# WHU-USI3DV/LaneMapping

Hardware: AMD Instinct MI355X
Metric: BEV tiles/sec end-to-end (LAS points -> polylines) (higher is better)
Workload: dtype f32; 1 GPU; on-GPU LAS->BEV raster (4,194,304 points/tile resident in HBM) + configs/Proj_polyline_fpn_vit_vertex_2.py, batch=16 per GPU, seeded random weights; lines_per_tile=45, streams=2, hip_graphs=True, points=resident, stream_check=not run (--full runs it), gather_check=n/a (1 rank), raster_check=not run (--full runs it), dist_ranks=1, rccl_ranks=1

## Files before the change

include/lanemap_hip.h:

```cpp
#ifndef LANEMAP_HIP_H
#define LANEMAP_HIP_H
#include <stdint.h>
#ifdef __cplusplus
extern "C" {
#endif

enum { LM_OK = 0, LM_ERR_ARG = 1, LM_ERR_HIP = 2, LM_ERR_NO_DEVICE = 3, LM_ERR_CAPACITY = 4 };
enum { LM_ACT_NONE = 0, LM_ACT_RELU = 1, LM_ACT_GELU = 2 };

int lm_abi_version(void);
const char* lm_last_error(void);
int lm_device_count(void);

int lm_conv2d_nhwc_mfma_f32(void* stream, const float* x, int ldx, const float* wp, int CoutP,
                            const float* scale, const float* shift, const float* res, int ldr, int res_rows,
                            float* y, int ldy, int B, int H, int W, int Cin, int Cout, int KH, int KW,
                            int stride, int pad_h, int pad_w, int dil, int act);
int lm_conv2d_nhwc_mfma_resup_f32(void* stream, const float* x, int ldx, const float* wp, int CoutP, const float* scale,
                                  const float* shift, const float* res_coarse, int ldr, int Hr, int Wr, float* y, int ldy,
                                  int B, int H, int W, int Cin, int Cout, int KH, int KW, int stride, int pad_h, int pad_w,
                                  int dil, int act);

int lm_winograd44_supported(int H, int W, int Cin, int dil);
int lm_winograd44_gn_chunks(int H, int W, int dil);
long lm_winograd44_tiles(int B, int H, int W, int dil);
long lm_winograd44_twin_workspace_bytes(int B, int H, int W, int Cin, int CoutP, int dil);
int lm_conv3x3_winograd44_f32(void* stream, const float* x, int ldx, const float* wu_frag, int CoutP, const float* scale,
                              const float* shift, const float* res, int ldr, float* y, int ldy, int B, int H, int W,
                              int Cin, int Cout, int dil, int act, double* gn_partial);
int lm_conv3x3_winograd44_twin_f32(void* stream, const float* x, int ldx, const float* wu, int CoutP, const float* scale,
                                   const float* shift, const float* res, int ldr, float* y, int ldy, int B, int H, int W,
                                   int Cin, int Cout, int dil, int act, void* workspace, long workspace_bytes);
int lm_wino44_split_fragments(void* stream, const float* frag, float* out, long n_quads);
int lm_conv3x3_winograd44_split_f32(void* stream, const float* x, int ldx, const float* wu_split, int CoutP, const float* scale,
                                    const float* shift, const float* res, int ldr, float* y, int ldy, int B, int H, int W,
                                    int Cin, int Cout, int dil, int act, double* gn_partial, float post);
int lm_conv3x3_winograd44_split_twin_f32(void* stream, const float* x, int ldx, const float* wu, int CoutP, const float* scale,
                                         const float* shift, const float* res, int ldr, float* y, int ldy, int B, int H, int W,
                                         int Cin, int Cout, int dil, int act, void* workspace, long workspace_bytes, float post);

int lm_conv2d_nhwc_mfma_f32_gnstats(void* stream, const float* x, int ldx, const float* wp, int CoutP, const float* shift,
                                    float* y, int ldy, double* gn_partial, int B, int H, int W, int Cin, int Cout,
                                    int KH, int KW, int stride, int pad_h, int pad_w, int dil);
int lm_gn_finalize(void* stream, const double* partial, float* stats, int B, int HW, int C, int nchunk, float eps);
int lm_gn_finalize_split(void* stream, const double* partial, float* stats, int B, int HW, int C, int nchunk, float eps, int split);

int lm_stem_conv7x7_bn_relu(void* stream, const float* x_chw, const float* w_k64, const float* scale,
                            const float* shift, float* y_nhwc, int B, int H, int W);
int lm_stem_conv7x7_bn_relu_u8(void* stream, const unsigned char* x_hwc3, const float* w_k64, const float* scale,
                               const float* shift, float* y_nhwc, int B, int H, int W);
int lm_maxpool3x3s2_nhwc(void* stream, const float* x, float* y, int B, int H, int W, int C);
int lm_conv2d_nhwc_small(void* stream, const float* x, int ldx, const float* w_tc16, const float* scale,
                         const float* shift, float* y, int ldy, int B, int H, int W, int Cin, int Cout,
                         int KH, int KW, int stride, int pad_h, int pad_w, int pre_relu, int act);

int lm_gn_stats(void* stream, const float* x, double* workspace, float* stats, int B, int HW, int C, float eps);
long lm_gn_stats_workspace_bytes(int B, int HW, int C);
int lm_gn_relu_upsample(void* stream, const float* x, const float* stats, const float* gamma, const float* beta,
                        float* y, int B, int Hi, int Wi, int Ho, int Wo, int C, int accumulate);
int lm_gn_relu_upsample_sum(void* stream, int n, const float* const* x, const float* const* stats, const int* Hi, const int* Wi,
                            const int* ldx , const float* gamma, const float* beta,
                            float* y, int B, int Ho, int Wo, int C);
int lm_gn_relu_upsample_sum_conv1x1(void* stream, int n, const float* const* x, const float* const* stats, const int* Hi, const int* Wi,
                                    const int* ldx, const float* gamma, const float* beta, float* y, int B, int Ho, int Wo, int C,
                                    const float* w_c16, const float* bias, int cout, float* y1, int ldy1);
int lm_upsample_bilinear_nhwc(void* stream, const float* x, int ldx, const float* add, int lda, float* y, int ldy,
                              int B, int Hi, int Wi, int Ho, int Wo, int C);
int lm_upsample_bilinear_to_chw(void* stream, const float* x, int ldx, float* y_chw, int B, int Hi, int Wi,
                                int Ho, int Wo, int C);
int lm_layernorm_rows(void* stream, const float* x, const float* gamma, const float* beta, float* y,
                      long rows, int D, float eps);
int lm_unpatchify(void* stream, const float* tokens, float* y_nhwc, int B, int G, int P, int C);
int lm_token_mix_mfma_f32(void* stream, const float* x, const float* wt, int ldw, const float* bias, const float* res, float* y,
                          int B, int M, int K, int N, int act);

int lm_attention_f32(void* stream, const float* qkv, float* out, int B, int N, int heads, int dim_head, float scale);
int lm_attention_masked_f32(void* stream, const float* qkv, float* out, const int* valid, int B, int N, int heads, int dim_head, float scale);

int lm_head_tokens(void* stream, const float* seg, const float* row_nhwc16, float* tok, float seg_bias,
                   int B, int P, int Hr, int Wr, int prop_width, int half_buff);
int lm_head_tokens_window(void* stream, const float* row_nhwc16, float* tok, int B, int P, int Hr, int Wr, int prop_width, int half_buff);
int lm_head_stage2(void* stream, const float* hid, int ldh, int D, const float* w2, const float* b2,
                   float* ext2, float* cls2, float* off2, long M);
int lm_head_proposal_conf(void* stream, const float* tok, const float* wt, const float* bias, float* conf,
                          int BP, int L);

int lm_head_endpoint_tile(void);
int lm_head_endpoint(void* hip_stream, const float* col, int ldc, const float* x_endp, const float* w1p, const float* b1,
                     const float* bn_scale, const float* bn_shift, const float* w2, const float* b2, float* out, int B, int h, int w,
                     int H, int W);

int lm_decode_proposals(void* stream, const float* pconf, const float* ext2, const float* cls2, const float* off2,
                        float* prop_conf, float* v_ext, float* cls_conf, int* cls_idx, double* cls_offset,
                        int B, int P, int R, float exist_thre, int prop_width, int half_buff);
int lm_decode_orient(void* stream, const float* x_nhwc, int ldx, int C, unsigned char* y, long pixels);
int lm_decode_semantic(void* stream, const float* logit_chw3, unsigned char* sem, float* biseg, float* rows,
                       int B, int H, int W, float thre, int raw_mode);
long lm_endp_topk_workspace_bytes(int B);
int lm_endp_topk(void* stream, const float* endp_logit, void* workspace, int* out_idx, float* out_score,
                 int* out_status, int B, int H, int W, int clip, int K);

int lm_pack_segments(void* stream, int n, const void* const* src, const long* bytes, const long* dst_offsets, void* dst);


typedef struct {
    float quat[4];
    float trans[3];
    float bev_img_offset[2];
    float img_reso[2];
    float local_min_ele;
    float ele_reso;
    float inten_lo, inten_hi;
} LmRasterParams;
long lm_bev_raster_workspace_bytes(int B, long max_points_per_tile, int H, int W);
int lm_bev_raster_batch(void* stream, const float* points_xyzi, const long* tile_offsets, const LmRasterParams* params,
                        int B, void* workspace, long workspace_bytes, float* out_chw, unsigned char* out_hwc_u8,
                        int H, int W);
int lm_bev_raster_batch_scaled(void* hip_stream, const float* points_xyzi, const long* tile_offsets, const LmRasterParams* params,
                               int B, void* workspace, long workspace_bytes, float* out_chw, unsigned char* out_hwc_u8,
                               int H, int W, const float* inten_scale);
int lm_tile_ingest_u8(void* stream, const unsigned char* src_hwc, float* dst_chw, int B, int H, int W, int C);

typedef struct {
    double x0, y0, cell;
    int nx, ny;
} LmStripGrid;
int lm_strip_build_grid(const LmRasterParams* params, int T, int H, int W, double z_lo, double z_hi, LmStripGrid* grid,
                        unsigned short* cells, long cells_cap);
long lm_strip_bin_workspace_bytes(long N, int T);
int lm_strip_bin_points(void* hip_stream, const float* points_xyzi, long N, const LmRasterParams* params, int T, int H, int W,
                        double z_lo, double z_hi, void* workspace, long workspace_bytes, long* counts, long* offsets,
                        long* offsets_host, float* binned, long capacity);

long lm_tile_ground_workspace_bytes(int B, int H, int W, int cell_px);
int lm_tile_ground(void* hip_stream, const float* points_xyzi, const long* tile_offsets, const LmRasterParams* params, int B, int H,
                   int W, int cell_px, void* workspace, long workspace_bytes, float* ground, float* ground_min, float* cell_min);
long lm_ground_select_workspace_bytes(long N, int B);
int lm_ground_select(void* hip_stream, const float* points_xyzi, const long* tile_offsets, const LmRasterParams* params, int B, int H,
                     int W, int cell_px, const float* ground, float h_lo, float h_hi, void* workspace, long workspace_bytes,
                     float* points_out, long* out_offsets, long* out_offsets_host);

long lm_tile_intensity_workspace_bytes(int B, int G);
int lm_tile_intensity_window(void* hip_stream, const float* points_xyzi, const long* tile_offsets, const LmRasterParams* params, int B,
                             int H, int W, const int* group, int G, int q_lo_ppm, int q_hi_ppm, void* workspace, long workspace_bytes,
                             int* window, long* count, unsigned* coarse_hist);

long lm_drape_workspace_bytes(long n_vertices, int B, int radius_px);
int lm_drape_vertices(void* hip_stream, const float* points_xyzi, const long* tile_offsets, const LmRasterParams* params, int B, int H,
                      int W, const int* vertices_rc, const long* vertex_offsets, int radius_px, void* workspace, long workspace_bytes,
                      float* z, int* npix, float* pixel_min);

int lm_tile_gap_hist(void* hip_stream, const unsigned char* tiles_hwc_u8, int B, int H, int W, int max_radius_px, unsigned* hist);
int lm_tile_gap_fill(void* hip_stream, const unsigned char* tiles_hwc_u8, int B, int H, int W, const int* radius_px,
                     unsigned char* out_hwc_u8);

int lm_endp_cluster(const int* topk_idx, int n_avail, int Wc, int clip, int k0, int k_step, int k_max, int radius,
                    int min_clusters, int* out_hw, int max_out, int* n_out, int* k_used);
int lm_polyline_assemble(const float* prop_conf, const float* prop_v_ext, const double* cls_offset,
                         const float* bi_seg_rows, const int* endp_hw, int n_endp, int P, int R, float obj_thre,
                         int min_vertices, double* out_lanes, int* endp_keep);
int lm_raster_polylines(const double* lanes, int P, int R, unsigned char* out);
int lm_line8(unsigned char* out, int x1, int y1, int x2, int y2, int colour);
int lm_trace_lines(const double* cols, int n, int R, const float* seg_rows, double* out);
int lm_polyline_backproject(unsigned char* bev_hwc, int H, int W, int C, const double* img_seqs, const int* seq_lens, int L,
                            int Vmax, const double* params13, const double* las_read_offset, double* out);
int lm_polyline_backproject_z(unsigned char* bev_hwc, int H, int W, int C, const double* img_seqs, const int* seq_lens, int L,
                              int Vmax, const double* params13, const double* las_read_offset, double* out,
                              const float* vertex_z, int fit);

long lm_skeletonize_lee_2d(unsigned char* img, int H, int W);

void* lm_merge_create(void);
void lm_merge_destroy(void* merger);
int lm_merge_add_tile(void* merger, const double* points, const int* lens, int n);
long lm_merge_finish(void* merger, long* total_points);
int lm_merge_result(void* merger, double* points, int* lens);
int lm_downsample_seq(const double* seq, int n, double dist_min, double* out);

int lm_softmax_rows(void* stream, float* x, long rows, int cols);
int lm_rowref_select(void* stream, const float* ext, const float* cls, float* mean_out, int* valid, float thr_ext, int* corr,
                     int B, int H, int W, int L);
int lm_rowref_gather(void* stream, const float* x_nhwc8, const int* corr, float* tok, int B, int H, int W, int L);
int lm_rowref_scatter(void* stream, const float* x_nhwc8, const float* tok, const int* corr, const int* valid,
                      float* y_nhwc8, int B, int H, int W, int L);
int lm_rowref_gather_win(void* hip_stream, const float* x_nhwc8, const int* corr, float* tok, int B, int H, int W, int L, int off_grid);
int lm_rowref_scatter_win(void* hip_stream, const float* x_nhwc8, const float* tok, const int* corr, const int* valid,
                          float* y_nhwc8, int B, int H, int W, int L, int off_grid);
int lm_rowref_decode(void* stream, const float* ext2, const float* cls2, unsigned char* conf, unsigned char* cls_map,
                     int* col_idx, int B, int H, int W, int L);

long lm_voxelize_workspace_bytes(long n_points);
long lm_scan_workspace_bytes(long n);
int lm_exclusive_scan_u32(void* stream, const unsigned* in, unsigned* out, long n, void* workspace, long workspace_bytes);
long lm_sort_pairs_workspace_bytes(long n);
int lm_sort_pairs_u32(void* stream, unsigned* keys_io, unsigned* vals_io, long n, int end_bit, void* workspace, long workspace_bytes);
int lm_voxelize_hard(void* stream, const float* points, long n, const float* range_lo_xyz, const float* voxel_size_xyz,
                     const int* grid_xyz, int max_points, int max_voxels, int batch_idx, const int* row_base, int cap_rows,
                     float* feats, int ldf, int* coords, int* row_end, int raster_order, void* workspace,
                     long workspace_bytes);
int lm_sparse_grid_build(void* stream, const int* coords, long n, int* grid, int B, int D, int H, int W);
long lm_sparse_conv_outputs_workspace_bytes(long out_cells);
int lm_sparse_conv_outputs(void* stream, const int* in_coords, long n_in, int B, const int* ksp_zyx9, int Do, int Ho, int Wo,
                           int* out_grid, int* out_coords, int cap_rows, int* out_count, void* workspace, long workspace_bytes);
int lm_sparse_rulebook(void* stream, const int* out_coords, long n_out, const int* in_grid, int B, int D, int H, int W,
                       const int* ksp_zyx9, int* nbr);
int lm_conv_gather_mfma_f32(void* stream, const float* x, int ldx, const int* nbr, int taps, const float* wp, int CoutP,
                            const float* scale, const float* shift, const float* res, int ldr, float* y, int ldy,
                            long M, int Cin, int Cout, int act);
int lm_sparse_to_dense_nhwc(void* stream, const float* feats, int ldf, const int* coords, long n, float* out, int B, int D,
                            int H, int W, int C, int flip_h);
int lm_upsample_bicubic_nhwc(void* stream, const float* x, float* y, int B, int H, int W, int C, int Ho, int Wo);

typedef struct {
    int version_major, version_minor, point_format, record_len;
    long n_points, offset_to_points;
    double scale[3], offset[3], min_xyz[3], max_xyz[3];
} LmLasHeader;
int lm_las_parse_header(const unsigned char* bytes, long len, LmLasHeader* out);
int lm_las_decode_points(void* stream, const unsigned char* records, int record_len, long n, const double* scale,
                         const double* offset, const double* shift, float inten_lo, float inten_hi, int normalise,
                         float* out_xyzi);
enum { LM_LAS_DROP_SYNTHETIC = 1, LM_LAS_DROP_KEYPOINT = 2, LM_LAS_DROP_WITHHELD = 4, LM_LAS_DROP_OVERLAP = 8 };
enum { LM_LAS_RETURNS_ALL = 0, LM_LAS_RETURNS_FIRST = 1, LM_LAS_RETURNS_LAST = 2, LM_LAS_RETURNS_SINGLE = 3 };
typedef struct { unsigned class_mask[8]; unsigned drop_flags; int returns; float z_lo, z_hi; } LmLasSelect;
long lm_las_select_workspace_bytes(long n);
int lm_las_decode_select(void* hip_stream, const unsigned char* records, int record_len, int point_format, long n,
                         const double* scale, const double* offset, const double* shift, float inten_lo, float inten_hi,
                         int normalise, const LmLasSelect* select, void* workspace, long workspace_bytes, float* out_xyzi,
                         long* kept, unsigned long* class_hist);

int lm_png_info(const unsigned char* data, long size, int* H, int* W, int* C);
int lm_png_decode_u8(const unsigned char* data, long size, unsigned char* out_hwc, long out_bytes);
int lm_png_decode_files_u8(const char* const* paths, int n, unsigned char* out_nhwc, int H, int W, int C, int threads);
int lm_zlib_inflate(const unsigned char* data, long size, unsigned char* out, long capacity, long* produced);

long lm_lane_json_text(const double* lane_vertexes, int n_lines, int row_size, int with_pervertex_semantics, char* out, long cap);
int lm_lane_json_write(const double* lane_vertexes, int n_lines, int row_size, int with_pervertex_semantics, const char* path);
int lm_seqs_json_write(const double* seqs, const int* lens, int L, int Vmax, int D, const char* path);

#ifdef __cplusplus
}
#endif
#endif
```

lanemapping_amd/_lib.py:

```python
import ctypes as C
import os

_HERE = os.path.dirname(os.path.abspath(__file__))
LIB_PATH = os.environ.get('LANEMAP_HIP_LIB') or os.path.join(_HERE, 'liblanemap_hip.so')

c_f32p = C.POINTER(C.c_float)
vp, i32, i64, f32 = C.c_void_p, C.c_int, C.c_long, C.c_float


class LmRasterParams(C.Structure):
    _fields_ = [('quat', C.c_float * 4), ('trans', C.c_float * 3), ('bev_img_offset', C.c_float * 2),
                ('img_reso', C.c_float * 2), ('local_min_ele', C.c_float), ('ele_reso', C.c_float),
                ('inten_lo', C.c_float), ('inten_hi', C.c_float)]


class LmLasHeader(C.Structure):
    _fields_ = [('version_major', C.c_int), ('version_minor', C.c_int), ('point_format', C.c_int), ('record_len', C.c_int),
                ('n_points', C.c_long), ('offset_to_points', C.c_long), ('scale', C.c_double * 3), ('offset', C.c_double * 3),
                ('min_xyz', C.c_double * 3), ('max_xyz', C.c_double * 3)]


class LmStripGrid(C.Structure):
    _fields_ = [('x0', C.c_double), ('y0', C.c_double), ('cell', C.c_double), ('nx', C.c_int), ('ny', C.c_int)]


class LmLasSelect(C.Structure):
    _fields_ = [('class_mask', C.c_uint * 8), ('drop_flags', C.c_uint), ('returns', C.c_int), ('z_lo', C.c_float), ('z_hi', C.c_float)]


SIGNATURES = {
    'lm_abi_version': (i32, []),
    'lm_last_error': (C.c_char_p, []),
    'lm_device_count': (i32, []),
    'lm_conv2d_nhwc_mfma_f32': (i32, [vp, vp, i32, vp, i32, vp, vp, vp, i32, i32, vp, i32,
                                      i32, i32, i32, i32, i32, i32, i32, i32, i32, i32, i32, i32]),
    'lm_conv2d_nhwc_mfma_resup_f32': (i32, [vp, vp, i32, vp, i32, vp, vp, vp, i32, i32, i32, vp, i32,
                                            i32, i32, i32, i32, i32, i32, i32, i32, i32, i32, i32, i32]),
    'lm_winograd44_supported': (i32, [i32, i32, i32, i32]),
    'lm_winograd44_gn_chunks': (i32, [i32, i32, i32]),
    'lm_winograd44_tiles': (i64, [i32, i32, i32, i32]),
    'lm_winograd44_twin_workspace_bytes': (i64, [i32, i32, i32, i32, i32, i32]),
    'lm_conv3x3_winograd44_f32': (i32, [vp, vp, i32, vp, i32, vp, vp, vp, i32, vp, i32, i32, i32, i32, i32, i32, i32, i32, vp]),
    'lm_conv3x3_winograd44_twin_f32': (i32, [vp, vp, i32, vp, i32, vp, vp, vp, i32, vp, i32, i32, i32, i32, i32, i32, i32, i32, vp, i64]),
    'lm_wino44_split_fragments': (i32, [vp, vp, vp, i64]),
    'lm_conv3x3_winograd44_split_f32': (i32, [vp, vp, i32, vp, i32, vp, vp, vp, i32, vp, i32, i32, i32, i32, i32, i32, i32, i32, vp, f32]),
    'lm_conv3x3_winograd44_split_twin_f32': (i32, [vp, vp, i32, vp, i32, vp, vp, vp, i32, vp, i32, i32, i32, i32, i32, i32, i32, i32, vp, i64, f32]),
    'lm_conv2d_nhwc_mfma_f32_gnstats': (i32, [vp, vp, i32, vp, i32, vp, vp, i32, vp] + [i32] * 11),
    'lm_gn_finalize': (i32, [vp, vp, vp, i32, i32, i32, i32, f32]),
    'lm_gn_finalize_split': (i32, [vp, vp, vp, i32, i32, i32, i32, f32, i32]),
    'lm_stem_conv7x7_bn_relu': (i32, [vp, vp, vp, vp, vp, vp, i32, i32, i32]),
    'lm_stem_conv7x7_bn_relu_u8': (i32, [vp, vp, vp, vp, vp, vp, i32, i32, i32]),
    'lm_maxpool3x3s2_nhwc': (i32, [vp, vp, vp, i32, i32, i32, i32]),
    'lm_conv2d_nhwc_small': (i32, [vp, vp, i32, vp, vp, vp, vp, i32, i32, i32, i32, i32, i32, i32, i32, i32, i32, i32, i32, i32]),
    'lm_gn_stats': (i32, [vp, vp, vp, vp, i32, i32, i32, f32]),
    'lm_gn_stats_workspace_bytes': (i64, [i32, i32, i32]),
    'lm_gn_relu_upsample': (i32, [vp, vp, vp, vp, vp, vp, i32, i32, i32, i32, i32, i32, i32]),
    'lm_gn_relu_upsample_sum': (i32, [vp, i32, vp, vp, vp, vp, vp, vp, vp, vp, i32, i32, i32, i32]),
    'lm_gn_relu_upsample_sum_conv1x1': (i32, [vp, i32, vp, vp, vp, vp, vp, vp, vp, vp, i32, i32, i32, i32, vp, vp, i32, vp, i32]),
    'lm_upsample_bilinear_nhwc': (i32, [vp, vp, i32, vp, i32, vp, i32, i32, i32, i32, i32, i32, i32]),
    'lm_upsample_bilinear_to_chw': (i32, [vp, vp, i32, vp, i32, i32, i32, i32, i32, i32]),
    'lm_layernorm_rows': (i32, [vp, vp, vp, vp, vp, i64, i32, f32]),
    'lm_token_mix_mfma_f32': (i32, [vp, vp, vp, i32, vp, vp, vp, i32, i32, i32, i32, i32]),
    'lm_unpatchify': (i32, [vp, vp, vp, i32, i32, i32, i32]),
    'lm_attention_f32': (i32, [vp, vp, vp, i32, i32, i32, i32, f32]),
    'lm_attention_masked_f32': (i32, [vp, vp, vp, vp, i32, i32, i32, i32, f32]),
    'lm_head_tokens': (i32, [vp, vp, vp, vp, f32, i32, i32, i32, i32, i32, i32]),
    'lm_head_tokens_window': (i32, [vp, vp, vp, i32, i32, i32, i32, i32, i32]),
    'lm_head_stage2': (i32, [vp, vp, i32, i32, vp, vp, vp, vp, vp, i64]),
    'lm_head_proposal_conf': (i32, [vp, vp, vp, vp, vp, i32, i32]),
    'lm_head_endpoint_tile': (i32, []),
    'lm_head_endpoint': (i32, [vp, vp, i32, vp, vp, vp, vp, vp, vp, vp, vp, i32, i32, i32, i32, i32]),
    'lm_decode_proposals': (i32, [vp, vp, vp, vp, vp, vp, vp, vp, vp, vp, i32, i32, i32, f32, i32, i32]),
    'lm_decode_orient': (i32, [vp, vp, i32, i32, vp, i64]),
    'lm_decode_semantic': (i32, [vp, vp, vp, vp, vp, i32, i32, i32, f32, i32]),
    'lm_endp_topk_workspace_bytes': (i64, [i32]),
    'lm_endp_topk': (i32, [vp, vp, vp, vp, vp, vp, i32, i32, i32, i32, i32]),
    'lm_pack_segments': (i32, [vp, i32, vp, vp, vp, vp]),
    'lm_bev_raster_workspace_bytes': (i64, [i32, i64, i32, i32]),
    'lm_bev_raster_batch': (i32, [vp, vp, C.POINTER(i64), C.POINTER(LmRasterParams), i32, vp, i64, vp, vp, i32, i32]),
    'lm_bev_raster_batch_scaled': (i32, [vp, vp, C.POINTER(i64), C.POINTER(LmRasterParams), i32, vp, i64, vp, vp, i32, i32, c_f32p]),
    'lm_tile_ingest_u8': (i32, [vp, vp, vp, i32, i32, i32, i32]),
    'lm_strip_build_grid': (i32, [C.POINTER(LmRasterParams), i32, i32, i32, C.c_double, C.c_double, C.POINTER(LmStripGrid), vp, i64]),
    'lm_strip_bin_workspace_bytes': (i64, [i64, i32]),
    'lm_strip_bin_points': (i32, [vp, vp, i64, C.POINTER(LmRasterParams), i32, i32, i32, C.c_double, C.c_double, vp, i64, vp, vp,
                                  C.POINTER(i64), vp, i64]),
    'lm_tile_ground_workspace_bytes': (i64, [i32, i32, i32, i32]),
    'lm_tile_ground': (i32, [vp, vp, C.POINTER(i64), C.POINTER(LmRasterParams), i32, i32, i32, i32, vp, i64, vp, vp, vp]),
    'lm_ground_select_workspace_bytes': (i64, [i64, i32]),
    'lm_ground_select': (i32, [vp, vp, C.POINTER(i64), C.POINTER(LmRasterParams), i32, i32, i32, i32, vp, f32, f32, vp, i64, vp, vp,
                               C.POINTER(i64)]),
    'lm_tile_intensity_workspace_bytes': (i64, [i32, i32]),
    'lm_tile_intensity_window': (i32, [vp, vp, C.POINTER(i64), C.POINTER(LmRasterParams), i32, i32, i32, C.POINTER(i32), i32, i32, i32, vp, i64,
                                       vp, vp, vp]),
    'lm_drape_workspace_bytes': (i64, [i64, i32, i32]),
    'lm_drape_vertices': (i32, [vp, vp, C.POINTER(i64), C.POINTER(LmRasterParams), i32, i32, i32, vp, C.POINTER(i64), i32, vp, i64, vp, vp, vp]),
    'lm_tile_gap_hist': (i32, [vp, vp, i32, i32, i32, i32, vp]),
    'lm_tile_gap_fill': (i32, [vp, vp, i32, i32, i32, C.POINTER(i32), vp]),
    'lm_endp_cluster': (i32, [vp, i32, i32, i32, i32, i32, i32, i32, i32, vp, i32, vp, vp]),
    'lm_polyline_assemble': (i32, [vp, vp, vp, vp, vp, i32, i32, i32, f32, i32, vp, vp]),
    'lm_raster_polylines': (i32, [vp, i32, i32, vp]),
    'lm_line8': (i32, [vp, i32, i32, i32, i32, i32]),
    'lm_trace_lines': (i32, [vp, i32, i32, vp, vp]),
    'lm_polyline_backproject': (i32, [vp, i32, i32, i32, vp, vp, i32, i32, vp, vp, vp]),
    'lm_polyline_backproject_z': (i32, [vp, i32, i32, i32, vp, vp, i32, i32, vp, vp, vp, vp, i32]),
    'lm_skeletonize_lee_2d': (i64, [vp, i32, i32]),
    'lm_merge_create': (vp, []),
    'lm_merge_destroy': (None, [vp]),
    'lm_merge_add_tile': (i32, [vp, vp, vp, i32]),
    'lm_merge_finish': (i64, [vp, C.POINTER(i64)]),
    'lm_merge_result': (i32, [vp, vp, vp]),
    'lm_downsample_seq': (i32, [vp, i32, C.c_double, vp]),
    'lm_softmax_rows': (i32, [vp, vp, i64, i32]),
    'lm_rowref_select': (i32, [vp, vp, vp, vp, vp, f32, vp, i32, i32, i32, i32]),
    'lm_rowref_gather': (i32, [vp, vp, vp, vp, i32, i32, i32, i32]),
    'lm_rowref_scatter': (i32, [vp, vp, vp, vp, vp, vp, i32, i32, i32, i32]),
    'lm_rowref_gather_win': (i32, [vp, vp, vp, vp, i32, i32, i32, i32, i32]),
    'lm_rowref_scatter_win': (i32, [vp, vp, vp, vp, vp, vp, i32, i32, i32, i32, i32]),
    'lm_rowref_decode': (i32, [vp, vp, vp, vp, vp, vp, i32, i32, i32, i32]),
    'lm_voxelize_workspace_bytes': (i64, [i64]),
    'lm_scan_workspace_bytes': (i64, [i64]),
    'lm_exclusive_scan_u32': (i32, [vp, vp, vp, i64, vp, i64]),
    'lm_sort_pairs_workspace_bytes': (i64, [i64]),
    'lm_sort_pairs_u32': (i32, [vp, vp, vp, i64, i32, vp, i64]),
    'lm_voxelize_hard': (i32, [vp, vp, i64, c_f32p, c_f32p, C.POINTER(i32), i32, i32, i32, vp, i32, vp, i32, vp, vp, i32, vp, i64]),
    'lm_sparse_grid_build': (i32, [vp, vp, i64, vp, i32, i32, i32, i32]),
    'lm_sparse_conv_outputs_workspace_bytes': (i64, [i64]),
    'lm_sparse_conv_outputs': (i32, [vp, vp, i64, i32, C.POINTER(i32), i32, i32, i32, vp, vp, i32, vp, vp, i64]),
    'lm_sparse_rulebook': (i32, [vp, vp, i64, vp, i32, i32, i32, i32, C.POINTER(i32), vp]),
    'lm_conv_gather_mfma_f32': (i32, [vp, vp, i32, vp, i32, vp, i32, vp, vp, vp, i32, vp, i32, i64, i32, i32, i32]),
    'lm_sparse_to_dense_nhwc': (i32, [vp, vp, i32, vp, i64, vp, i32, i32, i32, i32, i32, i32]),
    'lm_upsample_bicubic_nhwc': (i32, [vp, vp, vp, i32, i32, i32, i32, i32, i32]),
    'lm_las_parse_header': (i32, [vp, i64, C.POINTER(LmLasHeader)]),
    'lm_las_decode_points': (i32, [vp, vp, i32, i64, C.POINTER(C.c_double), C.POINTER(C.c_double), C.POINTER(C.c_double), f32, f32,
                                   i32, vp]),
    'lm_las_select_workspace_bytes': (i64, [i64]),
    'lm_las_decode_select': (i32, [vp, vp, i32, i32, i64, C.POINTER(C.c_double), C.POINTER(C.c_double), C.POINTER(C.c_double), f32, f32,
                                   i32, C.POINTER(LmLasSelect), vp, i64, vp, vp, vp]),
    'lm_png_info': (i32, [vp, i64, C.POINTER(i32), C.POINTER(i32), C.POINTER(i32)]),
    'lm_png_decode_u8': (i32, [vp, i64, vp, i64]),
    'lm_png_decode_files_u8': (i32, [C.POINTER(C.c_char_p), i32, vp, i32, i32, i32, i32]),
    'lm_zlib_inflate': (i32, [vp, i64, vp, i64, C.POINTER(i64)]),
    'lm_lane_json_text': (i64, [vp, i32, i32, i32, vp, i64]),
    'lm_lane_json_write': (i32, [vp, i32, i32, i32, C.c_char_p]),
    'lm_seqs_json_write': (i32, [vp, vp, i32, i32, i32, C.c_char_p]),
}

_lib = None


class LanemapHipError(RuntimeError):
    pass


def lib():
    global _lib
    if _lib is None:
        if not os.path.exists(LIB_PATH):
            raise LanemapHipError(
                f'{LIB_PATH} is missing: the HIP library is the only implementation of this package '
                '(no CPU fallback). Build it with `python -m lanemapping_amd.build`.')
        import torch
        L = C.CDLL(LIB_PATH)
        for name, (res, args) in SIGNATURES.items():
            fn = getattr(L, name)
            fn.restype = res
            fn.argtypes = args
        _lib = L
    return _lib


def check(code):
    if code != 0:
        raise LanemapHipError(f'lanemap_hip error {code}: {lib().lm_last_error().decode()}')
```

lanemapping_amd/csrc/common.h:

```cpp
#pragma once
#include <hip/hip_runtime.h>
#include <cstdarg>
#include <cstdint>
#include <cstdio>

#define LM_API extern "C" __attribute__((visibility("default")))

enum {
    LM_OK = 0,
    LM_ERR_ARG = 1,
    LM_ERR_HIP = 2,
    LM_ERR_NO_DEVICE = 3,
    LM_ERR_CAPACITY = 4
};

void lm_set_error(const char* fmt, ...);
int lm_ensure_dynamic_lds(const void* kernel, size_t bytes);

#define LM_REQUIRE(cond, ...)            \
    do {                                 \
        if (!(cond)) {                   \
            lm_set_error(__VA_ARGS__);   \
            return LM_ERR_ARG;           \
        }                                \
    } while (0)

#define LM_HIP(expr)                                                                  \
    do {                                                                              \
        hipError_t e_ = (expr);                                                       \
        if (e_ != hipSuccess) {                                                       \
            lm_set_error("%s failed: %s (%s:%d)", #expr, hipGetErrorString(e_), __FILE__, __LINE__); \
            return LM_ERR_HIP;                                                        \
        }                                                                             \
    } while (0)

#define LM_LAUNCH_CHECK() LM_HIP(hipGetLastError())

static inline int lm_cdiv(long a, long b) { return (int)((a + b - 1) / b); }
static inline long lm_cdivl(long a, long b) { return (a + b - 1) / b; }
static inline size_t lm_align256(size_t v) { return (v + 255) / 256 * 256; }

enum { LM_ACT_NONE = 0, LM_ACT_RELU = 1, LM_ACT_GELU = 2 };

#ifdef __HIPCC__
__device__ __forceinline__ void lm_bilin_axis_scaled(int o, int in, float scale, int& i0, int& i1, float& w0, float& w1) {
#pragma clang fp contract(off)
    const float src = scale * (float)o;
    i0 = (int)src;
    if (i0 > in - 1) i0 = in - 1;
    i1 = i0 + ((i0 < in - 1) ? 1 : 0);
    w1 = fminf(fmaxf(src - (float)i0, 0.f), 1.f);
    w0 = 1.f - w1;
}
__device__ __forceinline__ void lm_bilin_axis(int o, int in, int out, int& i0, int& i1, float& w0, float& w1) {
#pragma clang fp contract(off)
    const float scale = (out > 1) ? (float)(in - 1) / (float)(out - 1) : 0.f;
    lm_bilin_axis_scaled(o, in, scale, i0, i1, w0, w1);
}
#endif
struct LmFastDiv {
    unsigned d, mul, sh;
};
static inline LmFastDiv lm_fastdiv_make(unsigned d) {
    LmFastDiv f;
    f.d = d;
    f.sh = 0;
    while ((1ull << f.sh) < d) ++f.sh;
    f.mul = (unsigned)((((1ull << f.sh) - d) << 32) / d + 1);
    return f;
}
#ifdef __HIPCC__
__device__ __forceinline__ unsigned lm_fastdiv(unsigned n, const LmFastDiv& f) { return (__umulhi(n, f.mul) + n) >> f.sh; }
__device__ __forceinline__ void lm_gn_affine(float mean, float rstd, float gamma, float beta, float& a, float& g) {
#pragma clang fp contract(off)
    a = rstd * gamma;
    g = __builtin_fmaf(-mean, a, beta);
}
__device__ __forceinline__ float lm_gn_relu(float v, float a, float g) { return fmaxf(__builtin_fmaf(v, a, g), 0.f); }
__device__ __forceinline__ float lm_bilerp(float v00, float v01, float v10, float v11, float wy0, float wy1, float wx0, float wx1) {
#pragma clang fp contract(off)
    const float top = wx0 * v00 + wx1 * v01;
    const float bot = wx0 * v10 + wx1 * v11;
    return wy0 * top + wy1 * bot;
}
#endif
```

lanemapping_amd/csrc/decode.hip:

```cpp
#include "common.h"

#define LM_PACK_MAX_SEGMENTS 8

typedef float f32x4 __attribute__((ext_vector_type(4)));

namespace {

template <int N>
__device__ __forceinline__ int softmax_argmax(const float* in, float* out) {
    float m = in[0];
#pragma unroll
    for (int i = 1; i < N; ++i) m = fmaxf(m, in[i]);
    float s = 0.f;
#pragma unroll
    for (int i = 0; i < N; ++i) {
        out[i] = expf(in[i] - m);
        s += out[i];
    }
    int best = 0;
#pragma unroll
    for (int i = 0; i < N; ++i) {
        out[i] = out[i] / s;
        if (out[i] > out[best]) best = i;
    }
    return best;
}

template <int FW>
__global__ __launch_bounds__(256) void decode_proposals_kernel(
    const float* __restrict__ pconf, const float* __restrict__ ext2, const float* __restrict__ cls2,
    const float* __restrict__ off2, float* __restrict__ prop_conf, float* __restrict__ v_ext,
    float* __restrict__ cls_conf, int* __restrict__ cls_idx, double* __restrict__ cls_offset, int P, int R,
    float exist_thre, int prop_width, int half_buff, long total) {
    const long i = (long)blockIdx.x * 256 + threadIdx.x;
    if (i >= total) return;
    const int h = (int)(i % R);
    const long bp = i / R;
    const int p = (int)(bp % P);
    if (h == 0) {
        float o[2];
        softmax_argmax<2>(pconf + bp * 2, o);
        prop_conf[bp * 2] = o[0];
        prop_conf[bp * 2 + 1] = o[1];
    }
    float e[3];
    softmax_argmax<3>(ext2 + i * 3, e);
    float v = 0.f;
    if (e[1] > e[2] && e[1] > exist_thre) v = 1.f;
    if (e[2] > e[1] && e[2] > exist_thre) v = 2.f;
    v_ext[i] = v;
    float c[FW];
    const int idx = softmax_argmax<FW>(cls2 + i * FW, c);
#pragma unroll
    for (int k = 0; k < FW; ++k) cls_conf[i * FW + k] = c[k];
    cls_idx[i] = idx;
    const float fsum = (float)idx + off2[i * FW + idx];
    double co = (double)fsum;
    if (co > (double)FW) co = (double)FW;
    cls_offset[i] = co + (double)(prop_width * p - half_buff);
}

__global__ __launch_bounds__(256) void decode_orient_kernel(const float* __restrict__ x, int ldx, int C,
                                                            unsigned char* __restrict__ y, long total) {
    const long i = (long)blockIdx.x * 256 + threadIdx.x;
    if (i >= total) return;
    const float* xp = x + i * ldx;
    int best = 0;
    float bv = xp[0];
    for (int c = 1; c < C; ++c) {
        const float v = xp[c];
        if (v > bv) {
            bv = v;
            best = c;
        }
    }
    y[i] = (unsigned char)best;
}

__global__ __launch_bounds__(256) void decode_semantic_kernel(const float* __restrict__ logit, unsigned char* __restrict__ sem,
                                                              float* __restrict__ biseg, float* __restrict__ rows, int H, int W,
                                                              float thre, int raw_mode, long total) {
    const long i = (long)blockIdx.x * 256 + threadIdx.x;
    if (i >= total) return;
    const long HW = (long)H * W;
    const long b = i / HW, r = i - b * HW;
    const float* lp = logit + b * 3 * HW + r;
    const float l0 = lp[0], l1 = lp[HW], l2 = lp[2 * HW];
    float s1, s2;
    if (raw_mode) {
        s1 = l1;
        s2 = l2;
    } else {
        const float m = fmaxf(l0, fmaxf(l1, l2));
        const float e0 = expf(l0 - m), e1 = expf(l1 - m), e2 = expf(l2 - m);
        const float s = (e0 + e1) + e2;
        s1 = e1 / s;
        s2 = e2 / s;
    }
    unsigned char c = 0;
    if (s1 > s2 && s1 > thre) c = 1;
    if (s2 > s1 && s2 > thre) c = 2;
    sem[i] = c;
    if (biseg) {
        const float bs = s1 + s2;
        biseg[i] = bs;
        const int y = (int)(r / W);
        if (rows && (y & 7) == 3) rows[(b * (H / 8) + (y >> 3)) * W + (r - (long)y * W)] = bs;
    }
}

constexpr int NB = 1024;
constexpr int CAP = 4096;
struct TopkParams {
    const float* logit;
    unsigned* hist;
    unsigned* cand_cnt;
    unsigned long long* cand;
    int H, W, clip, K;
    LmFastDiv div_wc;
};

__device__ __forceinline__ unsigned score_key(float logit) {
    const float s = 1.0f / (1.0f + expf(-logit));
    return __float_as_uint(s);
}

__device__ __forceinline__ unsigned level_bin(unsigned key, int level) {
    return level == 0 ? (key >> 20) : (level == 1 ? ((key >> 10) & 1023u) : (key & 1023u));
}

__device__ void pick_bin_block(const unsigned* h, unsigned& need, unsigned& bin, unsigned* tmp) {
    const int t = threadIdx.x;
    unsigned c[4] = {0u, 0u, 0u, 0u}, s = 0;
    if (t < 256) {
        const uint4 v = *reinterpret_cast<const uint4*>(h + 4 * t);
        c[0] = v.x; c[1] = v.y; c[2] = v.z; c[3] = v.w;
        s = v.x + v.y + v.z + v.w;
        tmp[t] = s;
    }
    if (t == 0) {
        tmp[256] = need == 0 ? (unsigned)(NB - 1) : 0u;
        tmp[257] = 0u;
    }
    __syncthreads();
    for (int off = 1; off < 256; off <<= 1) {
        unsigned add = 0;
        if (t + off < 256) add = tmp[t + off];
        __syncthreads();
        if (t < 256) tmp[t] += add;
        __syncthreads();
    }
    if (t < 256 && need > 0) {
        const unsigned incl = tmp[t], above = incl - s;
        if (above < need && incl >= need) {
            unsigned acc = above;
#pragma unroll
            for (int k = 3; k >= 0; --k) {
                if (acc + c[k] >= need) {
                    tmp[256] = (unsigned)(4 * t + k);
                    tmp[257] = need - acc;
                    break;
                }
                acc += c[k];
            }
        }
    }
    __syncthreads();
    bin = tmp[256];
    need = tmp[257];
    __syncthreads();
}

__global__ __launch_bounds__(256) void zero_u32_kernel(unsigned* __restrict__ p, long n) {
    const long i = (long)blockIdx.x * 256 + threadIdx.x;
    if (i < n) p[i] = 0u;
}

template <int LEVEL>
__global__ __launch_bounds__(256) void topk_pass_kernel(TopkParams p) {
    __shared__ unsigned lh[NB];
    __shared__ unsigned pb_tmp[258];
    const int b = blockIdx.y;
    const int Hc = p.H - 2 * p.clip, Wc = p.W - 2 * p.clip;
    const long n = (long)Hc * Wc;
    unsigned* hist = p.hist + (long)b * 3 * NB;
    if (LEVEL < 3)
        for (int i = threadIdx.x; i < NB; i += 256) lh[i] = 0;
    unsigned prefix = 0;
    bool take_ties = false;
    {
        unsigned need = (unsigned)p.K, bin = 0;
#pragma unroll
        for (int lv = 0; lv < LEVEL && lv < 3; ++lv) {
            pick_bin_block(hist + lv * NB, need, bin, pb_tmp);
            prefix |= bin << (20 - 10 * lv);
        }
        if (LEVEL == 3) take_ties = hist[2 * NB + bin] == need;
    }
    __syncthreads();
    const float* lp = p.logit + (long)b * p.H * p.W;
    for (long i = (long)blockIdx.x * 256 + threadIdx.x; i < n; i += (long)gridDim.x * 256) {
        const int y = (int)lm_fastdiv((unsigned)i, p.div_wc), x = (int)((unsigned)i - (unsigned)y * (unsigned)Wc);
        const unsigned key = score_key(lp[(long)(y + p.clip) * p.W + x + p.clip]);
        if (LEVEL == 0) {
            atomicAdd(&lh[key >> 20], 1u);
        } else if (LEVEL == 1) {
            if ((key >> 20) == (prefix >> 20)) atomicAdd(&lh[(key >> 10) & 1023u], 1u);
        } else if (LEVEL == 2) {
            if ((key >> 10) == (prefix >> 10)) atomicAdd(&lh[key & 1023u], 1u);
        } else {
            if (key > prefix || (key == prefix && take_ties)) {
                const unsigned slot = atomicAdd(p.cand_cnt + b, 1u);
                if (slot < CAP) p.cand[(long)b * CAP + slot] = ((unsigned long long)key << 32) | (unsigned)(0xFFFFFFFFu - (unsigned)i);
            }
        }
    }
    if (LEVEL < 3) {
        __syncthreads();
        for (int i = threadIdx.x; i < NB; i += 256)
            if (lh[i]) atomicAdd(&hist[LEVEL * NB + i], lh[i]);
    }
}

__global__ __launch_bounds__(1024) void topk_ties_kernel(TopkParams p) {
    __shared__ unsigned sh[4];
    __shared__ unsigned wave_tot[16];
    const int b = blockIdx.x;
    const unsigned* hist = p.hist + (long)b * 3 * NB;
    __shared__ unsigned pb_tmp[258];
    unsigned need = (unsigned)p.K, bin = 0, T = 0;
#pragma unroll
    for (int lv = 0; lv < 3; ++lv) {
        pick_bin_block(hist + lv * NB, need, bin, pb_tmp);
        T |= bin << (20 - 10 * lv);
    }
    if (threadIdx.x == 0) sh[3] = p.cand_cnt[b];
    __syncthreads();
    const unsigned base = sh[3];
    if (hist[2 * NB + bin] == need || need == 0) return;
    const int Wc = p.W - 2 * p.clip;
    const long n = (long)(p.H - 2 * p.clip) * Wc;
    const float* lp = p.logit + (long)b * p.H * p.W;
    const int lane = threadIdx.x & 63, wave = threadIdx.x >> 6;
    unsigned taken = 0;
    for (long i0 = 0; i0 < n && taken < need; i0 += 1024) {
        const long i = i0 + threadIdx.x;
        bool tie = false;
        if (i < n) {
            const int y = (int)lm_fastdiv((unsigned)i, p.div_wc), x = (int)((unsigned)i - (unsigned)y * (unsigned)Wc);
            tie = score_key(lp[(long)(y + p.clip) * p.W + x + p.clip]) == T;
        }
        const unsigned long long m = __ballot(tie);
        const unsigned before = (unsigned)__popcll(m & ((1ull << lane) - 1ull));
        if (lane == 0) wave_tot[wave] = (unsigned)__popcll(m);
        __syncthreads();
        unsigned off = 0, tot = 0;
        for (int w = 0; w < 16; ++w) {
            if (w < wave) off += wave_tot[w];
            tot += wave_tot[w];
        }
        const unsigned rank = taken + off + before;
        if (tie && rank < need) p.cand[(long)b * CAP + base + rank] = ((unsigned long long)T << 32) | (unsigned)(0xFFFFFFFFu - (unsigned)i);
        taken += tot;
        __syncthreads();
    }
    if (threadIdx.x == 0) p.cand_cnt[b] = base + need;
}

__global__ __launch_bounds__(1024) void topk_sort_kernel(TopkParams p, int* __restrict__ out_idx, float* __restrict__ out_score,
                                                         int* __restrict__ out_status) {
    __shared__ unsigned long long v[CAP];
    const int b = blockIdx.x;
    const unsigned cnt = p.cand_cnt[b];
    const unsigned n = cnt < (unsigned)CAP ? cnt : (unsigned)CAP;
    for (int i = threadIdx.x; i < CAP; i += 1024) v[i] = (unsigned)i < n ? p.cand[(long)b * CAP + i] : 0ull;
    __syncthreads();
    for (int k = 2; k <= CAP; k <<= 1)
        for (int j = k >> 1; j > 0; j >>= 1) {
            for (int i = threadIdx.x; i < CAP; i += 1024) {
                const int l = i ^ j;
                if (l > i) {
                    const unsigned long long a = v[i], c = v[l];
                    const bool desc = (i & k) == 0;
                    if (desc ? (a < c) : (a > c)) {
                        v[i] = c;
                        v[l] = a;
                    }
                }
            }
            __syncthreads();
        }
    for (int i = threadIdx.x; i < p.K; i += 1024) {
        const unsigned long long e = v[i];
        const bool ok = (unsigned)i < n;
        out_idx[(long)b * p.K + i] = ok ? (int)(0xFFFFFFFFu - (unsigned)(e & 0xFFFFFFFFu)) : -1;
        out_score[(long)b * p.K + i] = ok ? __uint_as_float((unsigned)(e >> 32)) : 0.f;
    }
    if (threadIdx.x == 0) out_status[b] = (cnt > (unsigned)CAP) ? 1 : 0;
}


struct PackArgs {
    const void* src[LM_PACK_MAX_SEGMENTS];
    long offs[LM_PACK_MAX_SEGMENTS];
    long words[LM_PACK_MAX_SEGMENTS];
    long first_chunk[LM_PACK_MAX_SEGMENTS + 1];
    int n;
};

__global__ __launch_bounds__(256) void pack_segments_kernel(PackArgs a, unsigned char* __restrict__ dst) {
    const long c = (long)blockIdx.x * 256 + threadIdx.x;
    if (c >= a.first_chunk[a.n]) return;
    int s = 0;
#pragma unroll
    for (int k = 1; k < LM_PACK_MAX_SEGMENTS; ++k) s += (k < a.n && c >= a.first_chunk[k]) ? 1 : 0;
    const long w0 = (c - a.first_chunk[s]) * 4;
    const unsigned* src = static_cast<const unsigned*>(a.src[s]) + w0;
    unsigned* out = reinterpret_cast<unsigned*>(dst + a.offs[s]) + w0;
    const long left = a.words[s] - w0;
    if (left >= 4 && ((reinterpret_cast<unsigned long long>(src) & 15ull) == 0)) {
        *reinterpret_cast<uint4*>(out) = *reinterpret_cast<const uint4*>(src);
    } else {
        for (int e = 0; e < 4 && e < left; ++e) out[e] = src[e];
    }
}

}

LM_API int lm_decode_proposals(void* stream, const float* pconf, const float* ext2, const float* cls2, const float* off2,
                               float* prop_conf, float* v_ext, float* cls_conf, int* cls_idx, double* cls_offset,
                               int B, int P, int R, float exist_thre, int prop_width, int half_buff) {
    LM_REQUIRE(pconf && ext2 && cls2 && off2 && prop_conf && v_ext && cls_conf && cls_idx && cls_offset, "decode_proposals: null pointer");
    const int fw = prop_width + 2 * half_buff;
    LM_REQUIRE(fw == 10 || fw == 12 || fw == 16, "decode_proposals: prop_fea_width must be 10, 12 or 16 (got %d)", fw);
    const long total = (long)B * P * R;
    auto kernel = fw == 10 ? decode_proposals_kernel<10> : fw == 12 ? decode_proposals_kernel<12> : decode_proposals_kernel<16>;
    hipLaunchKernelGGL(kernel, dim3(lm_cdiv(total, 256)), dim3(256), 0, (hipStream_t)stream, pconf, ext2, cls2,
                       off2, prop_conf, v_ext, cls_conf, cls_idx, cls_offset, P, R, exist_thre, prop_width, half_buff, total);
    LM_LAUNCH_CHECK();
    return LM_OK;
}

LM_API int lm_decode_orient(void* stream, const float* x_nhwc, int ldx, int C, unsigned char* y, long pixels) {
    LM_REQUIRE(x_nhwc && y && C >= 1, "decode_orient: bad args");
    hipLaunchKernelGGL(decode_orient_kernel, dim3(lm_cdiv(pixels, 256)), dim3(256), 0, (hipStream_t)stream, x_nhwc, ldx, C, y, pixels);
    LM_LAUNCH_CHECK();
    return LM_OK;
}

LM_API int lm_decode_semantic(void* stream, const float* logit_chw3, unsigned char* sem, float* biseg, float* rows,
                              int B, int H, int W, float thre, int raw_mode) {
    LM_REQUIRE(logit_chw3 && sem, "decode_semantic: null pointer");
    LM_REQUIRE(!rows || H % 8 == 0, "decode_semantic: H must be a multiple of 8 for the row gather");
    const long total = (long)B * H * W;
    hipLaunchKernelGGL(decode_semantic_kernel, dim3(lm_cdiv(total, 256)), dim3(256), 0, (hipStream_t)stream, logit_chw3, sem,
                       biseg, rows, H, W, thre, raw_mode, total);
    LM_LAUNCH_CHECK();
    return LM_OK;
}

LM_API long lm_endp_topk_workspace_bytes(int B) {
    return (long)B * (3 * NB * sizeof(unsigned) + sizeof(unsigned) * 4 + (long)CAP * sizeof(unsigned long long));
}

LM_API int lm_endp_topk(void* stream, const float* endp_logit, void* workspace, int* out_idx, float* out_score,
                        int* out_status, int B, int H, int W, int clip, int K) {
    LM_REQUIRE(endp_logit && workspace && out_idx && out_score && out_status, "endp_topk: null pointer");
    LM_REQUIRE(K >= 1 && K <= CAP / 2 && H > 2 * clip && W > 2 * clip, "endp_topk: bad K=%d or crop", K);
    hipStream_t s = (hipStream_t)stream;
    TopkParams p;
    p.logit = endp_logit;
    char* ws = (char*)workspace;
    p.hist = (unsigned*)ws;
    p.cand_cnt = (unsigned*)(ws + (size_t)B * 3 * NB * sizeof(unsigned));
    p.cand = (unsigned long long*)(ws + (size_t)B * (3 * NB + 4) * sizeof(unsigned));
    p.H = H; p.W = W; p.clip = clip; p.K = K;
    LM_REQUIRE(W > 2 * clip && H > 2 * clip && (long)(H - 2 * clip) * (W - 2 * clip) < (1L << 31), "endp_topk: bad crop (H=%d W=%d clip=%d)", H, W, clip);
    p.div_wc = lm_fastdiv_make((unsigned)(W - 2 * clip));
    const long zero_words = (long)B * (3 * NB + 4);
    hipLaunchKernelGGL(zero_u32_kernel, dim3(lm_cdiv(zero_words, 256)), dim3(256), 0, s, (unsigned*)workspace, zero_words);
    LM_LAUNCH_CHECK();
    dim3 grid(256, B);
    hipLaunchKernelGGL(topk_pass_kernel<0>, grid, dim3(256), 0, s, p);
    LM_LAUNCH_CHECK();
    hipLaunchKernelGGL(topk_pass_kernel<1>, grid, dim3(256), 0, s, p);
    LM_LAUNCH_CHECK();
    hipLaunchKernelGGL(topk_pass_kernel<2>, grid, dim3(256), 0, s, p);
    LM_LAUNCH_CHECK();
    hipLaunchKernelGGL(topk_pass_kernel<3>, grid, dim3(256), 0, s, p);
    LM_LAUNCH_CHECK();
    hipLaunchKernelGGL(topk_ties_kernel, dim3(B), dim3(1024), 0, s, p);
    LM_LAUNCH_CHECK();
    hipLaunchKernelGGL(topk_sort_kernel, dim3(B), dim3(1024), 0, s, p, out_idx, out_score, out_status);
    LM_LAUNCH_CHECK();
    return LM_OK;
}

LM_API int lm_pack_segments(void* stream, int n, const void* const* src, const long* bytes, const long* dst_offsets, void* dst) {
    LM_REQUIRE(n >= 1 && n <= LM_PACK_MAX_SEGMENTS && src && bytes && dst_offsets && dst, "pack_segments: 1..%d segments", LM_PACK_MAX_SEGMENTS);
    PackArgs a;
    a.n = n;
    a.first_chunk[0] = 0;
    for (int s = 0; s < LM_PACK_MAX_SEGMENTS; ++s) {
        const bool on = s < n;
        LM_REQUIRE(!on || (src[s] && bytes[s] >= 0 && bytes[s] % 4 == 0 && dst_offsets[s] % 16 == 0), "pack_segments: segment %d: bytes %% 4, offset %% 16", s);
        a.src[s] = on ? src[s] : nullptr;
        a.offs[s] = on ? dst_offsets[s] : 0;
        a.words[s] = on ? bytes[s] / 4 : 0;
        a.first_chunk[s + 1] = a.first_chunk[s] + (a.words[s] + 3) / 4;
    }
    const long chunks = a.first_chunk[n];
    if (chunks == 0) return LM_OK;
    hipLaunchKernelGGL(pack_segments_kernel, dim3(lm_cdiv(chunks, 256)), dim3(256), 0, (hipStream_t)stream, a, static_cast<unsigned char*>(dst));
    LM_LAUNCH_CHECK();
    return LM_OK;
}
```

lanemapping_amd/csrc/norm_resize.hip:

```cpp
#include "common.h"

typedef float f32x4 __attribute__((ext_vector_type(4)));

namespace {

__device__ __forceinline__ void bilin_axis(int o, int in, int out, int& i0, int& i1, float& w0, float& w1) {
    lm_bilin_axis(o, in, out, i0, i1, w0, w1);
}

constexpr int GN_CHUNK = 512;

__global__ __launch_bounds__(256) void gn_partial_kernel(const float* __restrict__ x, double* __restrict__ part,
                                                         int HW, int C, int nchunk) {
    __shared__ double red[2][256];
    const int b = blockIdx.y, chunk = blockIdx.x;
    const int lanes_p = 256 / C;
    const int c = threadIdx.x % C, pl = threadIdx.x / C;
    const int p0 = chunk * GN_CHUNK;
    const int p1 = min(p0 + GN_CHUNK, HW);
    double s = 0.0, ss = 0.0;
    const float* xb = x + (long)b * HW * C;
    for (int p = p0 + pl; p < p1; p += lanes_p) {
        const double v = (double)xb[(long)p * C + c];
        s += v;
// ... 171 lines not shown
        if ((SAME >> k) & 1) {
#pragma unroll
            for (int e = 0; e < 4; ++e) o[e] = lm_gn_relu(tap[k][0][e], a[e], g[e]);
        } else {
            f32x4 v[4];
#pragma unroll
            for (int q = 0; q < 4; ++q)
#pragma unroll
                for (int e = 0; e < 4; ++e) v[q][e] = lm_gn_relu(tap[k][q][e], a[e], g[e]);
#pragma unroll
            for (int e = 0; e < 4; ++e) o[e] = lm_bilerp(v[0][e], v[1][e], v[2][e], v[3][e], wy0[k], wy1[k], wx0[k], wx1[k]);
        }
        if (k == 0) {
            acc = o;
        } else {
#pragma unroll
            for (int e = 0; e < 4; ++e) acc[e] = acc[e] + o[e];
        }
    }
    if (y) *reinterpret_cast<f32x4*>(y + (long)i * 4) = acc;
    if (Q.w) {
        float part[8];
#pragma unroll
        for (int n = 0; n < 8; ++n) part[n] = 0.f;
#pragma unroll
        for (int e = 0; e < 4; ++e) {
            const f32x4 w0 = *reinterpret_cast<const f32x4*>(wl + (c + e) * 8), w1 = *reinterpret_cast<const f32x4*>(wl + (c + e) * 8 + 4);
#pragma unroll
            for (int n = 0; n < 4; ++n) {
                part[n] = fmaf(acc[e], w0[n], part[n]);
                part[4 + n] = fmaf(acc[e], w1[n], part[4 + n]);
            }
        }
        const int lane = threadIdx.x & 63;
#pragma unroll
        for (int half = 4, mask = 1; half >= 1; half >>= 1, mask <<= 1) {
            const bool upper = (lane & mask) != 0;
#pragma unroll
            for (int jj = 0; jj < half; ++jj) {
                float lo = part[jj], hi = part[jj + half];
                asm volatile("" : "+v"(lo), "+v"(hi));
                const float send = upper ? lo : hi, keep = upper ? hi : lo;
                part[jj] = keep + __shfl_xor(send, mask);
            }
        }
        for (unsigned o = 8; o < c4n; o <<= 1) part[0] += __shfl_xor(part[0], (int)o);
        const unsigned li = (unsigned)c >> 2;
        const int n = 4 * (int)(li & 1) + 2 * (int)((li >> 1) & 1) + (int)((li >> 2) & 1);
        if (li < 8 && n < Q.cout) Q.y1[(long)((b * Ho + oy) * Wo + ox) * Q.ldy1 + n] = part[0] + (Q.bias ? Q.bias[n] : 0.f);
    }
}

constexpr int UT_R = 8, UT_C = 16;

__global__ __launch_bounds__(256) void gn_relu_up_lds_kernel(GnTerm T, const float* __restrict__ gamma, const float* __restrict__ beta,
                                                             float* __restrict__ y, int Ho, int Wo, int C, int SR, int SC) {
    extern __shared__ __attribute__((aligned(16))) float ups[];
    __shared__ int ty0[UT_R], ty1[UT_R], tx0[UT_C], tx1[UT_C];
    __shared__ float twy0[UT_R], twy1[UT_R], twx0[UT_C], twx1[UT_C];
    const int tid = threadIdx.x, c4n = C / 4;
    const int oy0 = blockIdx.y * UT_R, ox0 = blockIdx.x * UT_C, b = blockIdx.z;
    const int ny = min(UT_R, Ho - oy0), nx = min(UT_C, Wo - ox0);
    int sy0, sx0, i1;
    float w0, w1;
    lm_bilin_axis_scaled(oy0, T.Hi, T.sy, sy0, i1, w0, w1);
    lm_bilin_axis_scaled(ox0, T.Wi, T.sx, sx0, i1, w0, w1);
    if (tid < UT_R) {
        int a0, a1;
        lm_bilin_axis_scaled(min(oy0 + tid, Ho - 1), T.Hi, T.sy, a0, a1, w0, w1);
        ty0[tid] = a0 - sy0; ty1[tid] = a1 - sy0; twy0[tid] = w0; twy1[tid] = w1;
    } else if (tid >= 64 && tid < 64 + UT_C) {
        const int t = tid - 64;
        int a0, a1;
        lm_bilin_axis_scaled(min(ox0 + t, Wo - 1), T.Wi, T.sx, a0, a1, w0, w1);
        tx0[t] = a0 - sx0; tx1[t] = a1 - sx0; twx0[t] = w0; twx1[t] = w1;
    }
    const int cq = tid % c4n, pstep = 256 / c4n, p0 = tid / c4n;
    const int c = cq * 4;
    f32x4 a, g;
    {
        const f32x4 gm = *reinterpret_cast<const f32x4*>(gamma + c), bt = *reinterpret_cast<const f32x4*>(beta + c);
        const f32x4* st = reinterpret_cast<const f32x4*>(T.stats + ((long)b * C + c) * 2);
        const f32x4 st0 = st[0], st1 = st[1];
        const float mean[4] = {st0[0], st0[2], st1[0], st1[2]}, rstd[4] = {st0[1], st0[3], st1[1], st1[3]};
#pragma unroll
        for (int e = 0; e < 4; ++e) {
            float ae, ge;
            lm_gn_affine(mean[e], rstd[e], gm[e], bt[e], ae, ge);
            a[e] = ae;
            g[e] = ge;
        }
    }
    const int nsrc = SR * SC;
    const float* xb = T.x + (long)b * T.Hi * T.Wi * T.ld + c;
    constexpr int UNR = 4;
    for (int pb = p0; pb < nsrc; pb += pstep * UNR) {
        f32x4 v[UNR];
#pragma unroll
        for (int u = 0; u < UNR; ++u) {
            const int pp = pb + u * pstep;
            const int r = pp / SC, q = pp - r * SC;
            const int yy = min(sy0 + r, T.Hi - 1), xx = min(sx0 + q, T.Wi - 1);
            if (pp < nsrc) v[u] = *reinterpret_cast<const f32x4*>(xb + ((long)yy * T.Wi + xx) * T.ld);
        }
#pragma unroll
        for (int u = 0; u < UNR; ++u) {
            const int pp = pb + u * pstep;
            if (pp < nsrc) {
                f32x4 o;
#pragma unroll
                for (int e = 0; e < 4; ++e) o[e] = lm_gn_relu(v[u][e], a[e], g[e]);
                *reinterpret_cast<f32x4*>(ups + (long)pp * C + c) = o;
            }
        }
    }
    __syncthreads();
    const long obase = ((long)b * Ho + oy0) * Wo + ox0;
    for (int pp = p0; pp < UT_R * UT_C; pp += pstep) {
        const int r = pp / UT_C, q = pp % UT_C;
        if (r >= ny || q >= nx) continue;
        const float* s0 = ups + (long)(ty0[r] * SC) * C + c;
        const float* s1 = ups + (long)(ty1[r] * SC) * C + c;
        const f32x4 v00 = *reinterpret_cast<const f32x4*>(s0 + tx0[q] * C), v01 = *reinterpret_cast<const f32x4*>(s0 + tx1[q] * C);
        const f32x4 v10 = *reinterpret_cast<const f32x4*>(s1 + tx0[q] * C), v11 = *reinterpret_cast<const f32x4*>(s1 + tx1[q] * C);
        const float wy0 = twy0[r], wy1 = twy1[r], wx0 = twx0[q], wx1 = twx1[q];
        f32x4 o;
#pragma unroll
        for (int e = 0; e < 4; ++e) o[e] = lm_bilerp(v00[e], v01[e], v10[e], v11[e], wy0, wy1, wx0, wx1);
        __builtin_nontemporal_store(o, reinterpret_cast<f32x4*>(y + (obase + (long)r * Wo + q) * C + c));
    }
}

__global__ __launch_bounds__(256) void gn_sum3_lds_kernel(GnSum P, const float* __restrict__ gamma, const float* __restrict__ beta,
                                                          float* __restrict__ y, int Ho, int Wo, int C, int SR, int SC, Proj1x1 Q) {
    extern __shared__ __attribute__((aligned(16))) float ups[];
    __shared__ int ty0[UT_R], ty1[UT_R], tx0[UT_C], tx1[UT_C];
    __shared__ float twy0[UT_R], twy1[UT_R], twx0[UT_C], twx1[UT_C];
    const int tid = threadIdx.x, c4n = C / 4;
    const int oy0 = blockIdx.y * UT_R, ox0 = blockIdx.x * UT_C, b = blockIdx.z;
    const int ny = min(UT_R, Ho - oy0), nx = min(UT_C, Wo - ox0);
    const GnTerm& T0 = P.t[0];
    const GnTerm& T1 = P.t[1];
    const GnTerm& T2 = P.t[2];
    int sy0, sx0, i1;
    float w0, w1;
    lm_bilin_axis_scaled(oy0, T1.Hi, T1.sy, sy0, i1, w0, w1);
    lm_bilin_axis_scaled(ox0, T1.Wi, T1.sx, sx0, i1, w0, w1);
    if (tid < UT_R) {
        int a0, a1;
        lm_bilin_axis_scaled(min(oy0 + tid, Ho - 1), T1.Hi, T1.sy, a0, a1, w0, w1);
        ty0[tid] = a0 - sy0; ty1[tid] = a1 - sy0; twy0[tid] = w0; twy1[tid] = w1;
    } else if (tid >= 64 && tid < 64 + UT_C) {
        const int t = tid - 64;
        int a0, a1;
        lm_bilin_axis_scaled(min(ox0 + t, Wo - 1), T1.Wi, T1.sx, a0, a1, w0, w1);
        tx0[t] = a0 - sx0; tx1[t] = a1 - sx0; twx0[t] = w0; twx1[t] = w1;
    }
    const int cq = tid % c4n, pstep = 256 / c4n, p0 = tid / c4n;
    const int c = cq * 4;
    f32x4 a[3], g[3];
    {
        const f32x4 gm = *reinterpret_cast<const f32x4*>(gamma + c), bt = *reinterpret_cast<const f32x4*>(beta + c);
#pragma unroll
        for (int k = 0; k < 3; ++k) {
            const f32x4* st = reinterpret_cast<const f32x4*>(P.t[k].stats + ((long)b * C + c) * 2);
            const f32x4 st0 = st[0], st1 = st[1];
            const float mean[4] = {st0[0], st0[2], st1[0], st1[2]}, rstd[4] = {st0[1], st0[3], st1[1], st1[3]};
#pragma unroll
            for (int e = 0; e < 4; ++e) {
                float ae, ge;
                lm_gn_affine(mean[e], rstd[e], gm[e], bt[e], ae, ge);
                a[k][e] = ae;
                g[k][e] = ge;
            }
        }
    }
    float pw[4][8];
#pragma unroll
    for (int e = 0; e < 4; ++e)
#pragma unroll
        for (int n = 0; n < 8; ++n) pw[e][n] = n < Q.cout ? Q.w[(c + e) * 16 + n] : 0.f;
    const int nsrc = SR * SC;
    {
        const float* xb = T1.x + (long)b * T1.Hi * T1.Wi * T1.ld + c;
        constexpr int UNR = 4;
        for (int pb = p0; pb < nsrc; pb += pstep * UNR) {
            f32x4 v[UNR];
#pragma unroll
            for (int u = 0; u < UNR; ++u) {
                const int pp = pb + u * pstep;
                const int r = pp / SC, q = pp - r * SC;
                const int yy = min(sy0 + r, T1.Hi - 1), xx = min(sx0 + q, T1.Wi - 1);
                if (pp < nsrc) v[u] = *reinterpret_cast<const f32x4*>(xb + ((long)yy * T1.Wi + xx) * T1.ld);
            }
#pragma unroll
            for (int u = 0; u < UNR; ++u) {
                const int pp = pb + u * pstep;
                if (pp < nsrc) {
                    f32x4 o;
#pragma unroll
                    for (int e = 0; e < 4; ++e) o[e] = lm_gn_relu(v[u][e], a[1][e], g[1][e]);
                    *reinterpret_cast<f32x4*>(ups + (long)pp * C + c) = o;
                }
            }
        }
    }
    __syncthreads();
    const float* x0b = T0.x + (long)b * T0.Hi * T0.Wi * T0.ld + c;
    const float* x2b = T2.x + (long)b * T2.Hi * T2.Wi * T2.ld + c;
    const int lane = tid & 63;
    const unsigned li = (unsigned)cq;
    const int nsel = 4 * (int)(li & 1) + 2 * (int)((li >> 1) & 1) + (int)((li >> 2) & 1);
    const float pbias = (li < 8 && nsel < Q.cout && Q.bias) ? Q.bias[nsel] : 0.f;
    constexpr int UNR2 = 4;
    for (int pb = p0; pb < UT_R * UT_C; pb += pstep * UNR2) {
        f32x4 t0[UNR2], t2[UNR2];
        bool live[UNR2];
        int rr[UNR2], qq[UNR2];
#pragma unroll
        for (int u = 0; u < UNR2; ++u) {
            const int pp = pb + u * pstep;
            rr[u] = pp / UT_C; qq[u] = pp % UT_C;
            live[u] = rr[u] < ny && qq[u] < nx;
            const int oy = min(oy0 + rr[u], Ho - 1), ox = min(ox0 + qq[u], Wo - 1);
            t0[u] = *reinterpret_cast<const f32x4*>(x0b + ((long)oy * T0.Wi + ox) * T0.ld);
            t2[u] = *reinterpret_cast<const f32x4*>(x2b + ((long)oy * T2.Wi + ox) * T2.ld);
        }
#pragma unroll
        for (int u = 0; u < UNR2; ++u) {
            const int r = min(rr[u], UT_R - 1), q = qq[u];
            const float* s0 = ups + (long)(ty0[r] * SC) * C + c;
            const float* s1 = ups + (long)(ty1[r] * SC) * C + c;
            const f32x4 v00 = *reinterpret_cast<const f32x4*>(s0 + tx0[q] * C), v01 = *reinterpret_cast<const f32x4*>(s0 + tx1[q] * C);
            const f32x4 v10 = *reinterpret_cast<const f32x4*>(s1 + tx0[q] * C), v11 = *reinterpret_cast<const f32x4*>(s1 + tx1[q] * C);
            const float wy0 = twy0[r], wy1 = twy1[r], wx0 = twx0[q], wx1 = twx1[q];
            f32x4 acc;
#pragma unroll
            for (int e = 0; e < 4; ++e) {
#pragma clang fp contract(off)
                const float o0 = lm_gn_relu(t0[u][e], a[0][e], g[0][e]);
                const float o1 = lm_bilerp(v00[e], v01[e], v10[e], v11[e], wy0, wy1, wx0, wx1);
                const float o2 = lm_gn_relu(t2[u][e], a[2][e], g[2][e]);
                acc[e] = (o0 + o1) + o2;
            }
            const long opix = ((long)b * Ho + oy0 + rr[u]) * Wo + ox0 + qq[u];
            if (y && live[u]) *reinterpret_cast<f32x4*>(y + opix * C + c) = acc;
            float part[8];
#pragma unroll
            for (int n = 0; n < 8; ++n) part[n] = 0.f;
#pragma unroll
            for (int e = 0; e < 4; ++e)
#pragma unroll
                for (int n = 0; n < 8; ++n) part[n] = fmaf(acc[e], pw[e][n], part[n]);
#pragma unroll
            for (int half = 4, mask = 1; half >= 1; half >>= 1, mask <<= 1) {
                const bool upper = (lane & mask) != 0;
#pragma unroll
                for (int jj = 0; jj < half; ++jj) {
                    float lo = part[jj], hi = part[jj + half];
                    asm volatile("" : "+v"(lo), "+v"(hi));
                    const float send = upper ? lo : hi, keep = upper ? hi : lo;
                    part[jj] = keep + __shfl_xor(send, mask);
                }
            }
            for (unsigned o = 8; o < (unsigned)c4n; o <<= 1) part[0] += __shfl_xor(part[0], (int)o);
            if (live[u] && li < 8 && nsel < Q.cout) Q.y1[opix * Q.ldy1 + nsel] = part[0] + pbias;
        }
    }
}

__global__ __launch_bounds__(256) void upsample_nhwc_kernel(const float* __restrict__ x, int ldx, const float* __restrict__ add, int lda,
                                                            float* __restrict__ y, int ldy, int Hi, int Wi, int Ho, int Wo,
                                                            int C, long total4) {
    const long i = (long)blockIdx.x * 256 + threadIdx.x;
    if (i >= total4) return;
    const int c4n = C / 4;
    const int c = (int)(i % c4n) * 4;
    long t = i / c4n;
    const int ox = (int)(t % Wo);
    t /= Wo;
    const int oy = (int)(t % Ho);
    const int b = (int)(t / Ho);
    int y0, y1, x0, x1;
    float wy0, wy1, wx0, wx1;
    bilin_axis(oy, Hi, Ho, y0, y1, wy0, wy1);
    bilin_axis(ox, Wi, Wo, x0, x1, wx0, wx1);
    const float* xb = x + (long)b * Hi * Wi * ldx + c;
    const f32x4 v00 = *reinterpret_cast<const f32x4*>(xb + ((long)y0 * Wi + x0) * ldx);
    const f32x4 v01 = *reinterpret_cast<const f32x4*>(xb + ((long)y0 * Wi + x1) * ldx);
    const f32x4 v10 = *reinterpret_cast<const f32x4*>(xb + ((long)y1 * Wi + x0) * ldx);
    const f32x4 v11 = *reinterpret_cast<const f32x4*>(xb + ((long)y1 * Wi + x1) * ldx);
    const long opix = ((long)b * Ho + oy) * Wo + ox;
    f32x4 o;
#pragma unroll
    for (int e = 0; e < 4; ++e) o[e] = lm_bilerp(v00[e], v01[e], v10[e], v11[e], wy0, wy1, wx0, wx1);
    if (add) {
        const f32x4 r = *reinterpret_cast<const f32x4*>(add + opix * lda + c);
#pragma unroll
        for (int e = 0; e < 4; ++e) o[e] = o[e] + r[e];
    }
    *reinterpret_cast<f32x4*>(y + opix * ldy + c) = o;
}

__device__ __forceinline__ float upsample_blend(float v00, float v01, float v10, float v11, float wy0, float wy1, float wx0, float wx1) {
    return lm_bilerp(v00, v01, v10, v11, wy0, wy1, wx0, wx1);
}

__global__ __launch_bounds__(256) void upsample_to_chw_kernel(const float* __restrict__ x, int ldx, float* __restrict__ y,
                                                              int Hi, int Wi, int Ho, int Wo, int C, long total) {
    const long i = (long)blockIdx.x * 256 + threadIdx.x;
    if (i >= total) return;
    const int ox = (int)(i % Wo);
    long t = i / Wo;
    const int oy = (int)(t % Ho);
    t /= Ho;
    const int c = (int)(t % C);
    const int b = (int)(t / C);
    int y0, y1, x0, x1;
    float wy0, wy1, wx0, wx1;
    bilin_axis(oy, Hi, Ho, y0, y1, wy0, wy1);
    bilin_axis(ox, Wi, Wo, x0, x1, wx0, wx1);
    const float* xb = x + (long)b * Hi * Wi * ldx + c;
    const float v00 = xb[((long)y0 * Wi + x0) * ldx], v01 = xb[((long)y0 * Wi + x1) * ldx];
    const float v10 = xb[((long)y1 * Wi + x0) * ldx], v11 = xb[((long)y1 * Wi + x1) * ldx];
    y[i] = upsample_blend(v00, v01, v10, v11, wy0, wy1, wx0, wx1);
}

__global__ __launch_bounds__(256) void upsample_to_chw4_kernel(const float* __restrict__ x, int ldx, float* __restrict__ y,
                                                               int Hi, int Wi, int Ho, int Wo, int C, unsigned total4) {
    const unsigned i = blockIdx.x * 256u + threadIdx.x;
    if (i >= total4) return;
    const unsigned wq = (unsigned)Wo / 4;
    const int ox0 = (int)(i % wq) * 4;
    unsigned t = i / wq;
    const int oy = (int)(t % (unsigned)Ho);
    t /= (unsigned)Ho;
    const int c = (int)(t % (unsigned)C);
    const int b = (int)(t / (unsigned)C);
    int y0, y1;
    float wy0, wy1;
    bilin_axis(oy, Hi, Ho, y0, y1, wy0, wy1);
    const float* xb = x + (long)b * Hi * Wi * ldx + c;
    const float* r0 = xb + (long)y0 * Wi * ldx;
    const float* r1 = xb + (long)y1 * Wi * ldx;
    f32x4 o;
#pragma unroll
    for (int k = 0; k < 4; ++k) {
        int x0, x1;
        float wx0, wx1;
        bilin_axis(ox0 + k, Wi, Wo, x0, x1, wx0, wx1);
        const float v00 = r0[(long)x0 * ldx], v01 = r0[(long)x1 * ldx], v10 = r1[(long)x0 * ldx], v11 = r1[(long)x1 * ldx];
        o[k] = upsample_blend(v00, v01, v10, v11, wy0, wy1, wx0, wx1);
    }
    *reinterpret_cast<f32x4*>(y + (long)i * 4) = o;
}

template <int PER>
__global__ __launch_bounds__(256) void layernorm_kernel(const float* __restrict__ x, const float* __restrict__ gamma,
                                                        const float* __restrict__ beta, float* __restrict__ y, long rows,
                                                        float eps) {
    constexpr int D = PER * 64;
    const long row = (long)blockIdx.x * 4 + (threadIdx.x >> 6);
    if (row >= rows) return;
    const int lane = threadIdx.x & 63;
    const float* xr = x + row * D;
    float v[PER];
    float s = 0.f;
#pragma unroll
    for (int k = 0; k < PER; ++k) {
        v[k] = xr[k * 64 + lane];
        s += v[k];
    }
    for (int o = 32; o > 0; o >>= 1) s += __shfl_xor(s, o);
    const float mean = s / (float)D;
    float q = 0.f;
#pragma unroll
    for (int k = 0; k < PER; ++k) {
        const float d = v[k] - mean;
        q += d * d;
    }
    for (int o = 32; o > 0; o >>= 1) q += __shfl_xor(q, o);
    const float rstd = 1.0f / sqrtf(q / (float)D + eps);
    float* yr = y + row * D;
#pragma unroll
    for (int k = 0; k < PER; ++k) {
        const int c = k * 64 + lane;
        yr[c] = (v[k] - mean) * rstd * gamma[c] + beta[c];
    }
}

template <int PER>
__global__ __launch_bounds__(256) void layernorm_masked_kernel(const float* __restrict__ x, const float* __restrict__ gamma,
                                                               const float* __restrict__ beta, float* __restrict__ y, long rows, int D,
                                                               float eps) {
    const long row = (long)blockIdx.x * 4 + (threadIdx.x >> 6);
    if (row >= rows) return;
    const int lane = threadIdx.x & 63;
    const float* xr = x + row * D;
    float v[PER];
    float s = 0.f;
#pragma unroll
    for (int k = 0; k < PER; ++k) {
        const int c = k * 64 + lane;
        v[k] = c < D ? xr[c] : 0.f;
        s += v[k];
    }
    for (int o = 32; o > 0; o >>= 1) s += __shfl_xor(s, o);
    const float mean = s / (float)D;
    float q = 0.f;
#pragma unroll
    for (int k = 0; k < PER; ++k) {
        const float d = k * 64 + lane < D ? v[k] - mean : 0.f;
        q += d * d;
    }
    for (int o = 32; o > 0; o >>= 1) q += __shfl_xor(q, o);
    const float rstd = 1.0f / sqrtf(q / (float)D + eps);
    float* yr = y + row * D;
#pragma unroll
    for (int k = 0; k < PER; ++k) {
        const int c = k * 64 + lane;
        if (c < D) yr[c] = (v[k] - mean) * rstd * gamma[c] + beta[c];
    }
}

__global__ __launch_bounds__(256) void unpatchify_kernel(const float* __restrict__ t, float* __restrict__ y, int G, int P,
                                                         int C, long total) {
    const long i = (long)blockIdx.x * 256 + threadIdx.x;
    if (i >= total) return;
    const int c = (int)(i % C);
    long r = i / C;
    const int xx = (int)(r % (G * P));
    r /= (G * P);
    const int yy = (int)(r % (G * P));
    const int b = (int)(r / (G * P));
    const int gh = yy / P, p1 = yy % P, gw = xx / P, p2 = xx % P;
    y[i] = t[((long)b * G * G + gh * G + gw) * (P * P * C) + (p1 * P + p2) * C + c];
}

}

LM_API int lm_gn_stats(void* stream, const float* x, double* workspace, float* stats, int B, int HW, int C, float eps) {
    LM_REQUIRE(x && workspace && stats, "gn_stats: null pointer");
    LM_REQUIRE(C <= 256 && 256 % C == 0, "gn_stats: C=%d must divide 256", C);
    const int nchunk = lm_cdiv(HW, GN_CHUNK);
    hipLaunchKernelGGL(gn_partial_kernel, dim3(nchunk, B), dim3(256), 0, (hipStream_t)stream, x, workspace, HW, C, nchunk);
    LM_LAUNCH_CHECK();
    hipLaunchKernelGGL(gn_final_kernel, dim3(lm_cdiv(C, 32), B), dim3(256), 0, (hipStream_t)stream, workspace, stats, HW, C, nchunk, eps, 1);
    LM_LAUNCH_CHECK();
    return LM_OK;
}

LM_API int lm_gn_finalize(void* stream, const double* partial, float* stats, int B, int HW, int C, int nchunk, float eps) {
    LM_REQUIRE(partial && stats && nchunk >= 1, "gn_finalize: bad args");
    hipLaunchKernelGGL(gn_final_kernel, dim3(lm_cdiv(C, 32), B), dim3(256), 0, (hipStream_t)stream, partial, stats, HW, C, nchunk, eps, 1);
    LM_LAUNCH_CHECK();
    return LM_OK;
}

LM_API int lm_gn_finalize_split(void* stream, const double* partial, float* stats, int B, int HW, int C, int nchunk, float eps, int split) {
    LM_REQUIRE(partial && stats && nchunk >= 1 && split >= 1 && C % split == 0, "gn_finalize_split: bad args (C=%d split=%d)", C, split);
    hipLaunchKernelGGL(gn_final_kernel, dim3(lm_cdiv(C, 32), B), dim3(256), 0, (hipStream_t)stream, partial, stats, HW, C, nchunk, eps, split);
    LM_LAUNCH_CHECK();
    return LM_OK;
}

LM_API long lm_gn_stats_workspace_bytes(int B, int HW, int C) {
    return (long)B * lm_cdiv(HW, GN_CHUNK) * C * 2 * (long)sizeof(double);
}

LM_API int lm_gn_relu_upsample(void* stream, const float* x, const float* stats, const float* gamma, const float* beta,
                               float* y, int B, int Hi, int Wi, int Ho, int Wo, int C, int accumulate) {
    LM_REQUIRE(x && stats && gamma && beta && y && C % 4 == 0, "gn_relu_upsample: bad args");
    const long total4 = (long)B * Ho * Wo * (C / 4);
    hipLaunchKernelGGL(gn_relu_upsample_kernel, dim3(lm_cdiv(total4, 256)), dim3(256), 0, (hipStream_t)stream,
                       x, stats, gamma, beta, y, Hi, Wi, Ho, Wo, C, accumulate, total4);
    LM_LAUNCH_CHECK();
    return LM_OK;
}

namespace {
int up_block_extent(int in, int out, int tile) {
#pragma clang fp contract(off)
    const float scale = (out > 1) ? (float)(in - 1) / (float)(out - 1) : 0.f;
    auto tap0 = [&](int o) {
        int i0 = (int)(scale * (float)o);
        return i0 > in - 1 ? in - 1 : i0;
    };
    int ext = 1;
    for (int o0 = 0; o0 < out; o0 += tile) {
        const int ol = (o0 + tile - 1 < out ? o0 + tile - 1 : out - 1);
        const int last0 = tap0(ol), last1 = last0 + (last0 < in - 1 ? 1 : 0);
        const int e = last1 - tap0(o0) + 1;
        if (e > ext) ext = e;
    }
    return ext;
}

int launch_gn_sum(void* stream, int n, const float* const* x, const float* const* stats, const int* Hi, const int* Wi, const int* ldx,
                  const float* gamma, const float* beta, float* y, int B, int Ho, int Wo, int C, Proj1x1 Q) {
    LM_REQUIRE(n >= 1 && n <= 3 && x && stats && Hi && Wi && gamma && beta && C > 0 && C % 4 == 0, "gn_relu_upsample_sum: bad args");
    const long total4 = (long)B * Ho * Wo * (C / 4);
    LM_REQUIRE(total4 > 0 && total4 < (1L << 31), "gn_relu_upsample_sum: %ld output quads do not fit 32-bit indices", total4);
    GnSum P;
    P.n = n;
    for (int k = 0; k < 3; ++k) {
        const int q = k < n ? k : 0;
        LM_REQUIRE(x[q] && stats[q] && Hi[q] > 0 && Wi[q] > 0, "gn_relu_upsample_sum: bad term %d", q);
        const int ld = ldx ? ldx[q] : C;
        LM_REQUIRE(ld >= C && ld % 4 == 0, "gn_relu_upsample_sum: bad leading dimension %d of term %d", ld, q);
        LM_REQUIRE((long)Hi[q] * Wi[q] * ld < (1L << 30), "gn_relu_upsample_sum: term %d: an image of %ld elements does not fit 32-bit byte offsets", q,
                   (long)Hi[q] * Wi[q] * ld);
        P.t[k] = GnTerm{x[q], stats[q], Hi[q], Wi[q], ld, Ho > 1 ? (float)(Hi[q] - 1) / (float)(Ho - 1) : 0.f,
                        Wo > 1 ? (float)(Wi[q] - 1) / (float)(Wo - 1) : 0.f};
    }
    const int c4n = C / 4;
    LM_REQUIRE(256 % c4n == 0 || !Q.w, "gn_relu_upsample_sum: the fused 1x1 projection needs C/4 = %d to divide 256", c4n);
    LM_REQUIRE(Ho <= 65535 && B <= 65535, "gn_relu_upsample_sum: grid too large");
    int c4shift = -1;
    for (int sft = 0; sft < 16; ++sft)
        if ((1 << sft) == c4n) c4shift = sft;
    int same = 0;
    for (int k = 0; k < n; ++k)
        if (Hi[k] == Ho && Wi[k] == Wo) same |= 1 << k;
    if (n == 1 && same == 0 && !Q.w && y && 256 % c4n == 0 && Hi[0] > 1 && Wi[0] > 1 && Ho >= 2 * Hi[0] - 1 && Wo >= 2 * Wi[0] - 1) {
        static const bool lds_up = [] { const char* e = getenv("LM_GN_UP_LDS"); return !e || atoi(e) != 0; }();
        const int SR = up_block_extent(Hi[0], Ho, UT_R), SC = up_block_extent(Wi[0], Wo, UT_C);
        const size_t lds = (size_t)SR * SC * C * sizeof(float);
        if (lds_up && lds <= 72 * 1024) {
            if (int e = lm_ensure_dynamic_lds((const void*)gn_relu_up_lds_kernel, lds)) return e;
            hipLaunchKernelGGL(gn_relu_up_lds_kernel, dim3((unsigned)lm_cdiv(Wo, UT_C), (unsigned)lm_cdiv(Ho, UT_R), (unsigned)B), dim3(256), lds,
                               (hipStream_t)stream, P.t[0], gamma, beta, y, Ho, Wo, C, SR, SC);
            LM_LAUNCH_CHECK();
            return LM_OK;
        }
    }
    if (n == 3 && same == 5 && Q.w && c4n >= 8 && c4n <= 64 && (c4n & (c4n - 1)) == 0 && Hi[1] > 1 && Wi[1] > 1 && Ho >= 2 * Hi[1] - 1 &&
        Wo >= 2 * Wi[1] - 1) {
        static const bool lds_sum = [] { const char* e = getenv("LM_GN_SUM_LDS"); return !e || atoi(e) != 0; }();
        const int SR = up_block_extent(Hi[1], Ho, UT_R), SC = up_block_extent(Wi[1], Wo, UT_C);
        const size_t lds = (size_t)SR * SC * C * sizeof(float);
        if (lds_sum && lds <= 64 * 1024) {
            if (int e = lm_ensure_dynamic_lds((const void*)gn_sum3_lds_kernel, lds)) return e;
            hipLaunchKernelGGL(gn_sum3_lds_kernel, dim3((unsigned)lm_cdiv(Wo, UT_C), (unsigned)lm_cdiv(Ho, UT_R), (unsigned)B), dim3(256), lds,
                               (hipStream_t)stream, P, gamma, beta, y, Ho, Wo, C, SR, SC, Q);
            LM_LAUNCH_CHECK();
            return LM_OK;
        }
    }
    const dim3 grid((unsigned)lm_cdiv((long)Wo * c4n, 256), (unsigned)Ho, (unsigned)B);
#define LM_GNS(NN, SS)                                                                                                           \
    case (NN) * 8 + (SS):                                                                                                        \
        hipLaunchKernelGGL((gn_relu_upsample_sum_kernel<NN, SS>), grid, dim3(256), 0, (hipStream_t)stream, P, gamma, beta, y, Ho, Wo, C, \
                           c4shift, Q);                                                                                         \
        break;
    switch (n * 8 + same) {
        LM_GNS(1, 0) LM_GNS(1, 1)
        LM_GNS(2, 0) LM_GNS(2, 1) LM_GNS(2, 2) LM_GNS(2, 3)
        LM_GNS(3, 0) LM_GNS(3, 1) LM_GNS(3, 2) LM_GNS(3, 3) LM_GNS(3, 4) LM_GNS(3, 5) LM_GNS(3, 6) LM_GNS(3, 7)
    }
#undef LM_GNS
    LM_LAUNCH_CHECK();
    return LM_OK;
}
}

LM_API int lm_gn_relu_upsample_sum(void* stream, int n, const float* const* x, const float* const* stats, const int* Hi, const int* Wi,
                                   const int* ldx, const float* gamma, const float* beta, float* y, int B, int Ho, int Wo, int C) {
    LM_REQUIRE(y, "gn_relu_upsample_sum: null output");
    return launch_gn_sum(stream, n, x, stats, Hi, Wi, ldx, gamma, beta, y, B, Ho, Wo, C, Proj1x1{nullptr, nullptr, nullptr, 0, 0});
}

LM_API int lm_gn_relu_upsample_sum_conv1x1(void* stream, int n, const float* const* x, const float* const* stats, const int* Hi,
                                           const int* Wi, const int* ldx, const float* gamma, const float* beta, float* y, int B, int Ho,
                                           int Wo, int C, const float* w_c16, const float* bias, int cout, float* y1, int ldy1) {
    LM_REQUIRE(w_c16 && y1 && cout >= 1 && cout <= 8 && ldy1 >= cout, "gn_relu_upsample_sum_conv1x1: bad projection (cout=%d)", cout);
    const int c4n = C / 4;
    LM_REQUIRE(C % 4 == 0 && c4n >= 8 && c4n <= 64 && (c4n & (c4n - 1)) == 0,
               "gn_relu_upsample_sum_conv1x1: C=%d: C/4 must be a power of two in [8, 64] (one pixel per wave segment)", C);
    return launch_gn_sum(stream, n, x, stats, Hi, Wi, ldx, gamma, beta, y, B, Ho, Wo, C, Proj1x1{w_c16, bias, y1, cout, ldy1});
}

LM_API int lm_upsample_bilinear_nhwc(void* stream, const float* x, int ldx, const float* add, int lda, float* y, int ldy,
                                     int B, int Hi, int Wi, int Ho, int Wo, int C) {
    LM_REQUIRE(x && y && C % 4 == 0 && ldx % 4 == 0 && ldy % 4 == 0 && (!add || lda % 4 == 0), "upsample_nhwc: bad args");
    const long total4 = (long)B * Ho * Wo * (C / 4);
    hipLaunchKernelGGL(upsample_nhwc_kernel, dim3(lm_cdiv(total4, 256)), dim3(256), 0, (hipStream_t)stream,
                       x, ldx, add, lda, y, ldy, Hi, Wi, Ho, Wo, C, total4);
    LM_LAUNCH_CHECK();
    return LM_OK;
}

LM_API int lm_upsample_bilinear_to_chw(void* stream, const float* x, int ldx, float* y, int B, int Hi, int Wi,
                                       int Ho, int Wo, int C) {
    LM_REQUIRE(x && y && C >= 1, "upsample_to_chw: bad args");
    const long total = (long)B * C * Ho * Wo;
    if (Wo % 4 == 0 && total / 4 < (1L << 31) && ((uintptr_t)y & 15) == 0) {
        hipLaunchKernelGGL(upsample_to_chw4_kernel, dim3(lm_cdiv(total / 4, 256)), dim3(256), 0, (hipStream_t)stream,
                           x, ldx, y, Hi, Wi, Ho, Wo, C, (unsigned)(total / 4));
        LM_LAUNCH_CHECK();
        return LM_OK;
    }
    hipLaunchKernelGGL(upsample_to_chw_kernel, dim3(lm_cdiv(total, 256)), dim3(256), 0, (hipStream_t)stream,
                       x, ldx, y, Hi, Wi, Ho, Wo, C, total);
    LM_LAUNCH_CHECK();
    return LM_OK;
}

LM_API int lm_layernorm_rows(void* stream, const float* x, const float* gamma, const float* beta, float* y,
                             long rows, int D, float eps) {
    LM_REQUIRE(x && gamma && beta && y && D >= 32 && D <= 4096 && D % 32 == 0 && D != 768,
               "layernorm: D=%d must be 512 or 1024, or another multiple of 32 in [32, 4096] except 768", D);
    const dim3 grid(lm_cdiv(rows, 4));
    hipStream_t s = (hipStream_t)stream;
    if (D == 512)
        hipLaunchKernelGGL(layernorm_kernel<8>, grid, dim3(256), 0, s, x, gamma, beta, y, rows, eps);
    else if (D == 1024)
        hipLaunchKernelGGL(layernorm_kernel<16>, grid, dim3(256), 0, s, x, gamma, beta, y, rows, eps);
#define LM_LN_MASKED(PER) else if (D <= PER * 64) hipLaunchKernelGGL(layernorm_masked_kernel<PER>, grid, dim3(256), 0, s, x, gamma, beta, y, rows, D, eps);
    LM_LN_MASKED(1) LM_LN_MASKED(2) LM_LN_MASKED(4) LM_LN_MASKED(8) LM_LN_MASKED(16) LM_LN_MASKED(32) LM_LN_MASKED(64)
#undef LM_LN_MASKED
    LM_LAUNCH_CHECK();
    return LM_OK;
}

LM_API int lm_unpatchify(void* stream, const float* tokens, float* y_nhwc, int B, int G, int P, int C) {
    LM_REQUIRE(tokens && y_nhwc, "unpatchify: null pointer");
    const long total = (long)B * G * P * G * P * C;
    hipLaunchKernelGGL(unpatchify_kernel, dim3(lm_cdiv(total, 256)), dim3(256), 0, (hipStream_t)stream, tokens, y_nhwc, G, P, C, total);
    LM_LAUNCH_CHECK();
    return LM_OK;
}
```

lanemapping_amd/net.py:

```python
import torch
import torch.nn as nn

from . import ops, trace
from .registry import NET, build_pcencoder, build_backbone, build_heads


@NET.register_module
class Detector1stage(nn.Module):
    def __init__(self, head_type='seg', loss_type='row_ce', cfg=None):
        super().__init__()
        self.cfg = cfg
        self.conv1 = nn.Conv2d(144, 144, 3, 3)
        self.pcencoder = build_pcencoder(cfg)
        self.backbone = build_backbone(cfg)
        self.heads = build_heads(cfg)
        self.head_type, self.loss_type = head_type, loss_type

    def forward_raw(self, batch):
        fused = hasattr(self.pcencoder, 'fpn') and self.cfg.heads.type == 'ColumnProposal2'
        col = None
        if fused:
            proj = batch['proj']
            B, H, W = (proj.shape[0], proj.shape[1], proj.shape[2]) if proj.dtype == torch.uint8 else (proj.shape[0], proj.shape[2], proj.shape[3])
            col = ops.new_act(B, 16, H // 4, W // 4, proj.device)
            with trace.stage('pcencoder'):
                fea, fea_up, bi_seg, endp_est = self.pcencoder.fpn(proj, fea_up_out=col[:, 8:16])
        else:
            with trace.stage('pcencoder'):
                fea, fea_up, bi_seg, endp_est = self.pcencoder(batch)
        if self.cfg.vit_seg == True:
            with trace.stage('backbone'):
                fea = self.backbone(fea)
        with trace.stage('heads'):
            if self.cfg.heads.type == 'RowSharNotReducRef':
                out = self.heads(fea)
            else:
                out = self.heads(fea, fea_up, endp_est, col=col) if fused else self.heads(fea, fea_up, endp_est)
        out['semantic_seg'] = bi_seg
        out['endp_est'] = endp_est
        return out

    def forward(self, batch, is_get_features=False, stack_local_global_features=False):
        if self.training:
            raise NotImplementedError('lanemapping_amd implements the inference hot path only (call .eval())')
        if is_get_features:
            raise NotImplementedError('is_get_features is not on the hot path')
        output = {}
        with torch.no_grad():
            out = self.forward_raw(batch)
            output.update(self.heads.get_exist_coor_endp_dict(out))
            output['lane_maps'] = self.heads.get_lane_map_numpy_with_label(
                output, batch, is_flip=self.cfg.flip_label, is_img=self.cfg.view, is_get_1_stage_result=False,
                is_gt_avai=self.cfg.is_gt_avai)
            if self.cfg.show_result:
                output['pred_maps'] = self.heads.get_lane_map_on_source_image(output, batch)
        return output


@NET.register_module
class Segmentor(nn.Module):
    def __init__(self, head_type='seg', loss_type='ce', cfg=None):
        super().__init__()
        self.cfg = cfg
        self.pcencoder = build_pcencoder(cfg)
        self.head_type, self.loss_type = head_type, loss_type

    def forward(self, batch):
        if self.training:
            raise NotImplementedError('lanemapping_amd implements the inference hot path only (call .eval())')
        with torch.no_grad():
            _, _, bi_seg, endp_est = self.pcencoder(batch)
            pred = {'seg': bi_seg, 'endp': endp_est}
            return dict(self.pcencoder.infer_validate(pred, seg_thre=self.cfg.seg_thre, endp_thre=self.cfg.endp_thre))
```

lanemapping_amd/ops.py:

```python
import ctypes as C
import math

import torch

from ._lib import lib, check, LmRasterParams, LmStripGrid, LanemapHipError

ACT_NONE, ACT_RELU, ACT_GELU = 0, 1, 2


def _stream():
    return C.c_void_p(torch._C._cuda_getCurrentRawStream(torch._C._cuda_getDevice()))


def _ptr(t):
    if t is None:
        return None
    if not t.is_cuda:
        raise LanemapHipError('lanemapping_amd ops need tensors on an MI355X (HIP) device; no CPU fallback exists')
    if t.device.index != torch._C._cuda_getDevice():
        raise LanemapHipError(f'tensor on cuda:{t.device.index} but the current device is cuda:{torch._C._cuda_getDevice()}: '
                              'call torch.cuda.set_device() (one process drives one GPU)')
    return C.c_void_p(t.data_ptr())


# ... 224 lines not shown
    else:
        launch()
    check(lib().lm_gn_finalize(_stream(), _ptr(part), _ptr(stats), B, Ho * Wo, cout, nchunk, eps))
    return out, stats


def linear_mfma(x2d, wp, n_out, scale=None, shift=None, res=None, res_rows=0, act=ACT_NONE, out=None):
    assert x2d.dim() == 2 and x2d.stride(1) == 1
    M, K = x2d.shape
    if out is None:
        out = torch.empty((M, n_out), device=x2d.device, dtype=torch.float32)
    ldr = res.stride(0) if res is not None else 0
    def launch():
        check(lib().lm_conv2d_nhwc_mfma_f32(_stream(), _ptr(x2d), x2d.stride(0), _ptr(wp), wp.shape[1], _ptr(scale),
                                            _ptr(shift), _ptr(res), ldr, res_rows, _ptr(out), out.stride(0),
                                            1, 1, M, K, n_out, 1, 1, 1, 0, 0, 1, act))
    if _conv_hook is not None:
        _conv_hook(f'gemm M{M} K{K} N{n_out}', 2.0 * M * n_out * K, launch)
    else:
        launch()
    return out


def token_mix(x2d, wt, M, bias, B, res=None, act=ACT_NONE, out=None):
    assert x2d.dim() == 2 and x2d.is_contiguous() and x2d.shape[0] % B == 0
    K, N = x2d.shape[0] // B, x2d.shape[1]
    assert wt.shape[0] >= K and wt.shape[1] >= M and bias.numel() == M
    if out is None:
        out = torch.empty((B * M, N), device=x2d.device, dtype=torch.float32)
    assert out.is_contiguous() and tuple(out.shape) == (B * M, N)
    if res is not None:
        assert res.is_contiguous() and tuple(res.shape) == (B * M, N)
    def launch():
        check(lib().lm_token_mix_mfma_f32(_stream(), _ptr(x2d), _ptr(wt), wt.shape[1], _ptr(bias), _ptr(res), _ptr(out),
                                          B, M, K, N, act))
    if _conv_hook is not None:
        _conv_hook(f'token_mix M{M} K{K} N{N} B{B}', 2.0 * B * M * K * N, launch)
    else:
        launch()
    return out


def conv_small(x, w16, cout, kh=1, kw=1, stride=1, pad=0, scale=None, shift=None, pre_relu=False, act=ACT_NONE, out=None):
    x, ldx = as_nhwc(x)
    B, cin, H, W = x.shape
    ph, pw = (pad, pad) if isinstance(pad, int) else pad
    Ho = (H + 2 * ph - kh) // stride + 1
    Wo = (W + 2 * pw - kw) // stride + 1
    if out is None:
        out = new_act(B, cout, Ho, Wo, x.device)
    out_, ldy = as_nhwc(out)
    assert out_.data_ptr() == out.data_ptr()
    check(lib().lm_conv2d_nhwc_small(_stream(), _ptr(x), ldx, _ptr(w16), _ptr(scale), _ptr(shift), _ptr(out), ldy,
                                     B, H, W, cin, cout, kh, kw, stride, ph, pw, int(pre_relu), act))
    return out


def stem(x, w_k64, scale, shift):
    x = x.contiguous()
    if x.dtype == torch.uint8:
        B, H, W, C_ = x.shape
        assert C_ == 3, 'u8 tiles are [B,H,W,3]'
    else:
        B, _, H, W = x.shape
    Ho, Wo = (H - 1) // 2 + 1, (W - 1) // 2 + 1
    out = new_act(B, 64, Ho, Wo, x.device)
    fn = lib().lm_stem_conv7x7_bn_relu_u8 if x.dtype == torch.uint8 else lib().lm_stem_conv7x7_bn_relu
    check(fn(_stream(), _ptr(x), _ptr(w_k64), _ptr(scale), _ptr(shift), _ptr(out), B, H, W))
    return out


def maxpool3x3s2(x):
    x, ld = as_nhwc(x)
    B, C_, H, W = x.shape
    assert ld == C_
    out = new_act(B, C_, (H - 1) // 2 + 1, (W - 1) // 2 + 1, x.device)
    check(lib().lm_maxpool3x3s2_nhwc(_stream(), _ptr(x), _ptr(out), B, H, W, C_))
    return out


def gn_stats(x, eps=1e-5):
    x, ld = as_nhwc(x)
    B, C_, H, W = x.shape
    assert ld == C_
    ws = torch.empty(lib().lm_gn_stats_workspace_bytes(B, H * W, C_) // 8, device=x.device, dtype=torch.float64)
    stats = torch.empty((B, C_, 2), device=x.device, dtype=torch.float32)
    check(lib().lm_gn_stats(_stream(), _ptr(x), _ptr(ws), _ptr(stats), B, H * W, C_, eps))
    return stats


def gn_relu_upsample(x, stats, gamma, beta, size, out=None, accumulate=False):
    x, ld = as_nhwc(x)
    B, C_, H, W = x.shape
    assert ld == C_
    Ho, Wo = size
    if out is None:
        assert not accumulate
        out = new_act(B, C_, Ho, Wo, x.device)
    check(lib().lm_gn_relu_upsample(_stream(), _ptr(x), _ptr(stats), _ptr(gamma), _ptr(beta), _ptr(out),
                                    B, H, W, Ho, Wo, C_, int(accumulate)))
    return out


def gn_relu_upsample_sum(terms, gamma, beta, size, out=None, proj=None, keep_sum=True):
    n = len(terms)
    xs = [as_nhwc(x) for x, _ in terms]
    B, C_ = xs[0][0].shape[:2]
    for (x, ld) in xs:
        assert ld >= C_ and ld % 4 == 0 and x.shape[0] == B and x.shape[1] == C_
    Ho, Wo = size
    dev = xs[0][0].device
    if out is None and (keep_sum or proj is None):
        out = new_act(B, C_, Ho, Wo, dev)
    vp_arr, i_arr = C.c_void_p * n, C.c_int * n
    head = (_stream(), n, vp_arr(*[_ptr(x) for x, _ in xs]), vp_arr(*[_ptr(st) for _, st in terms]),
            i_arr(*[x.shape[2] for x, _ in xs]), i_arr(*[x.shape[3] for x, _ in xs]), i_arr(*[ld for _, ld in xs]),
            _ptr(gamma), _ptr(beta))
    if proj is None:
        check(lib().lm_gn_relu_upsample_sum(*head, _ptr(out), B, Ho, Wo, C_))
        return out
    w16, bias, cout = proj[:3]
    out1 = proj[3] if len(proj) > 3 and proj[3] is not None else new_act(B, cout, Ho, Wo, dev)
    o1, ldy1 = as_nhwc(out1)
    assert o1.data_ptr() == out1.data_ptr()
    check(lib().lm_gn_relu_upsample_sum_conv1x1(*head, _ptr(out) if keep_sum else None, B, Ho, Wo, C_, _ptr(w16), _ptr(bias), cout,
                                                _ptr(out1), ldy1))
    return (out, out1) if keep_sum else out1


def upsample_nhwc(x, size, add=None, out=None):
    x, ldx = as_nhwc(x)
    B, C_, H, W = x.shape
    Ho, Wo = size
    if out is None and add is None and (Ho, Wo) == (H, W):
        return x
    if out is None:
        out = new_act(B, C_, Ho, Wo, x.device)
    out_, ldy = as_nhwc(out)
    assert out_.data_ptr() == out.data_ptr()
    lda = 0
    if add is not None:
        add, lda = as_nhwc(add)
    check(lib().lm_upsample_bilinear_nhwc(_stream(), _ptr(x), ldx, _ptr(add), lda, _ptr(out), ldy, B, H, W, Ho, Wo, C_))
    return out


def pack_head_endpoint(conv1, bn, conv2):
    s, beta = fold_bn(bn)
    return (conv1.weight.permute(1, 2, 3, 0).float().contiguous(), conv1.bias.float().contiguous(), s, beta,
            conv2.weight[0].float().contiguous(), conv2.bias.float().contiguous())


def head_endpoint_tile():
    return int(lib().lm_head_endpoint_tile())


def head_endpoint(col, x_endp, packed, out=None):
    col_, ldc = as_nhwc(col)
    B, C_, h, w = col_.shape
    assert C_ == 16, 'head_endpoint: col has 16 channels'
    x_endp = x_endp.contiguous()
    assert x_endp.dim() == 4 and x_endp.shape[0] == B and x_endp.shape[1] == 1 and x_endp.dtype == torch.float32
    H, W = x_endp.shape[2:]
    if out is None:
        out = torch.empty((B, 1, H, W), device=col.device, dtype=torch.float32)
    w1p, b1, s, beta, w2, b2 = packed
    assert w1p.numel() == 17 * 36 and w2.numel() == 36
    check(lib().lm_head_endpoint(_stream(), _ptr(col_), ldc, _ptr(x_endp), _ptr(w1p), _ptr(b1), _ptr(s), _ptr(beta), _ptr(w2), _ptr(b2),
                                 _ptr(out), B, h, w, H, W))
    return out


def upsample_to_chw(x, size):
    x, ldx = as_nhwc(x)
    B, C_, H, W = x.shape
    Ho, Wo = size
    out = torch.empty((B, C_, Ho, Wo), device=x.device, dtype=torch.float32)
    check(lib().lm_upsample_bilinear_to_chw(_stream(), _ptr(x), ldx, _ptr(out), B, H, W, Ho, Wo, C_))
    return out


def layernorm(x2d, gamma, beta, eps=1e-5):
    assert x2d.is_contiguous()
    out = torch.empty_like(x2d)
    check(lib().lm_layernorm_rows(_stream(), _ptr(x2d), _ptr(gamma), _ptr(beta), _ptr(out), x2d.shape[0], x2d.shape[1], eps))
    return out


def unpatchify(tokens, B, G, P, C_):
    out = new_act(B, C_, G * P, G * P, tokens.device)
    check(lib().lm_unpatchify(_stream(), _ptr(tokens.contiguous()), _ptr(out), B, G, P, C_))
    return out


def attention(qkv, B, N, heads, dim_head, scale, valid=None):
    assert qkv.is_contiguous()
    out = torch.empty((B * N, heads * dim_head), device=qkv.device, dtype=torch.float32)
    if valid is None:
        check(lib().lm_attention_f32(_stream(), _ptr(qkv), _ptr(out), B, N, heads, dim_head, float(scale)))
    else:
        assert valid.dtype == torch.int32 and valid.is_contiguous() and tuple(valid.shape) == (B, N)
        check(lib().lm_attention_masked_f32(_stream(), _ptr(qkv), _ptr(out), _ptr(valid), B, N, heads, dim_head, float(scale)))
    return out


def head_tokens(seg, row, P, prop_width, half_buff, seg_bias):
    row, ld = as_nhwc(row)
    B, C_, Hr, Wr = row.shape
    assert C_ == 16 and ld == 16
    tok = torch.empty((B * P * Hr, 16 * (prop_width + 2 * half_buff)), device=row.device, dtype=torch.float32)
    if seg is None:
        check(lib().lm_head_tokens_window(_stream(), _ptr(row), _ptr(tok), B, P, Hr, Wr, prop_width, half_buff))
        return tok
    seg = seg.reshape(B, 2 * Hr, 2 * Wr).contiguous()
    check(lib().lm_head_tokens(_stream(), _ptr(seg), _ptr(row), _ptr(tok), float(seg_bias), B, P, Hr, Wr, prop_width, half_buff))
    return tok


def head_stage2(hid, D, w2, b2, B, P, R, w_small=None):
    M = hid.shape[0]
    FW = (w2.shape[0] - 3) // 2
    assert w2.shape == (3 + 2 * FW, D) and b2.numel() == 3 + 2 * FW and hid.shape[1] >= 3 * D and hid.stride(1) == 1
    ext2 = torch.empty((B, P, R, 3), device=hid.device, dtype=torch.float32)
    cls2 = torch.empty((B, P, R, FW), device=hid.device, dtype=torch.float32)
    off2 = torch.empty((B, P, R, FW), device=hid.device, dtype=torch.float32)
    if FW == 10:
        check(lib().lm_head_stage2(_stream(), _ptr(hid), hid.stride(0), D, _ptr(w2), _ptr(b2), _ptr(ext2), _ptr(cls2), _ptr(off2), M))
        return ext2, cls2, off2
    if w_small is None:
        raise ValueError(f'head_stage2: prop_fea_width {FW} runs through lm_conv2d_nhwc_small and needs the pack_small weights')
    bounds = (0, 3, 3 + FW, 3 + 2 * FW)
    for br, (y, w16) in enumerate(zip((ext2, cls2, off2), w_small)):
        n = bounds[br + 1] - bounds[br]
        assert tuple(w16.shape) == (1, D, 16)
        x = hid[:, br * D:(br + 1) * D]
        shift = b2[bounds[br]:bounds[br + 1]]
        check(lib().lm_conv2d_nhwc_small(_stream(), _ptr(x), hid.stride(0), _ptr(w16), None, _ptr(shift), _ptr(y), n,
                                         1, 1, M, D, n, 1, 1, 1, 0, 0, 0, ACT_NONE))
    return ext2, cls2, off2


def head_proposal_conf(tok, wt, bias, B, P):
    L = tok.numel() // (B * P)
    conf = torch.empty((B, P, 2), device=tok.device, dtype=torch.float32)
    check(lib().lm_head_proposal_conf(_stream(), _ptr(tok), _ptr(wt), _ptr(bias), _ptr(conf), B * P, L))
    return conf


def pack_readback(tensors, block=None):
    offs, sizes, off = [], [], 0
    for t in tensors:
        assert t.is_contiguous()
        nb = t.numel() * t.element_size()
        assert nb % 4 == 0, 'lm_pack_segments copies 4-byte words'
        off = (off + 255) // 256 * 256
        offs.append(off); sizes.append(nb)
        off += nb
    if block is None or block.numel() < off or block.device != tensors[0].device:
        block = torch.empty(max(off, 1), device=tensors[0].device, dtype=torch.uint8)
    n = len(tensors)
    src = (C.c_void_p * n)(*[t.data_ptr() for t in tensors])
    nby = (C.c_long * n)(*sizes)
    dof = (C.c_long * n)(*offs)
    check(lib().lm_pack_segments(_stream(), n, src, nby, dof, _ptr(block)))
    return block, list(zip(offs, sizes))


def decode_proposals(pconf, ext2, cls2, off2, exist_thre, prop_width, half_buff):
    B, P, R, FW = cls2.shape
    assert FW == prop_width + 2 * half_buff and off2.shape[-1] == FW, 'cls2 / offset2 are prop_fea_width wide'
    dev = cls2.device
    prop_conf = torch.empty((B, P, 2), device=dev, dtype=torch.float32)
    v_ext = torch.empty((B, P, R), device=dev, dtype=torch.float32)
    cls_conf = torch.empty((B, P, R, FW), device=dev, dtype=torch.float32)
    cls_idx = torch.empty((B, P, R), device=dev, dtype=torch.int32)
    cls_offset = torch.empty((B, P, R), device=dev, dtype=torch.float64)
    check(lib().lm_decode_proposals(_stream(), _ptr(pconf.contiguous()), _ptr(ext2.contiguous()), _ptr(cls2.contiguous()),
                                    _ptr(off2.contiguous()), _ptr(prop_conf), _ptr(v_ext), _ptr(cls_conf), _ptr(cls_idx),
                                    _ptr(cls_offset), B, P, R, float(exist_thre), prop_width, half_buff))
    return prop_conf, v_ext, cls_conf, cls_idx, cls_offset


def decode_orient(orient_logits):
    x, ld = as_nhwc(orient_logits)
    B, C_, H, W = x.shape
    out = torch.empty((B, H, W), device=x.device, dtype=torch.uint8)
    check(lib().lm_decode_orient(_stream(), _ptr(x), ld, C_, _ptr(out), B * H * W))
    return out


def decode_semantic(logits_chw, thre, raw_mode=False, want_biseg=True):
    x = logits_chw.contiguous()
    B, C_, H, W = x.shape
    assert C_ == 3
    sem = torch.empty((B, H, W), device=x.device, dtype=torch.uint8)
    biseg = rows = None
    if want_biseg:
        biseg = torch.empty((B, H, W), device=x.device, dtype=torch.float32)
        rows = torch.empty((B, H // 8, W), device=x.device, dtype=torch.float32)
    check(lib().lm_decode_semantic(_stream(), _ptr(x), _ptr(sem), _ptr(biseg), _ptr(rows), B, H, W, float(thre), int(raw_mode)))
    return sem, biseg, rows


def endp_topk(endp_logits, K=512, clip=20):
    x = endp_logits.contiguous()
    B, C_, H, W = x.shape
    assert C_ == 1
    ws = torch.empty(lib().lm_endp_topk_workspace_bytes(B), device=x.device, dtype=torch.uint8)
    idx = torch.empty((B, K), device=x.device, dtype=torch.int32)
    score = torch.empty((B, K), device=x.device, dtype=torch.float32)
    status = torch.empty((B,), device=x.device, dtype=torch.int32)
    check(lib().lm_endp_topk(_stream(), _ptr(x), _ptr(ws), _ptr(idx), _ptr(score), _ptr(status), B, H, W, clip, K))
    return idx, score, status


def make_raster_params(quat=(1, 0, 0, 0), trans=(0, 0, 0), bev_img_offset=(0, 0), img_reso=(0.05, 0.05),
                       local_min_ele=0.0, ele_reso=0.05, inten_lo=800.0, inten_hi=33000.0):
    p = LmRasterParams()
    p.quat[:] = [float(v) for v in quat]
    p.trans[:] = [float(v) for v in trans]
    p.bev_img_offset[:] = [float(v) for v in bev_img_offset]
    p.img_reso[:] = [float(v) for v in img_reso]
    p.local_min_ele, p.ele_reso, p.inten_lo, p.inten_hi = float(local_min_ele), float(ele_reso), float(inten_lo), float(inten_hi)
    return p


_raster_ws = {}


def _workspace(points, need):
    key = (points.device, _stream().value)
    ws = _raster_ws.get(key)
    if ws is None or ws.numel() < need:
        ws = _raster_ws[key] = torch.empty(need, device=points.device, dtype=torch.uint8)
    return ws


def _tile_range_args(who, points, tile_offsets, params):
    if not points.is_cuda:
        _ptr(points)
    assert points.dim() == 2 and points.shape[1] == 4 and points.is_contiguous() and points.dtype == torch.float32
    B = len(params)
    if len(tile_offsets) != B + 1:
        raise ValueError(f'{who}: {len(tile_offsets)} tile_offsets for {B} tiles (B + 1 are needed)')
    offs = (C.c_long * (B + 1))(*[int(o) for o in tile_offsets])
    if B and offs[B] > points.shape[0]:
        raise ValueError(f'{who}: tile_offsets end at {offs[B]}, points has {points.shape[0]} rows')
    return B, offs, (LmRasterParams * B)(*params)


def bev_raster_batch(points, tile_offsets, params, H=1152, W=1152, out=None, want_u8=False, u8_only=False, out_u8=None, inten_scale=None):
    assert points.dim() == 2 and points.shape[1] == 4 and points.is_contiguous() and points.dtype == torch.float32
    B = len(params)
    assert len(tile_offsets) == B + 1
    offs = (C.c_long * (B + 1))(*[int(o) for o in tile_offsets])
    par = (LmRasterParams * B)(*params)
    cap = max([offs[b + 1] - offs[b] for b in range(B)] + [0])
    ws = _workspace(points, lib().lm_bev_raster_workspace_bytes(B, cap, H, W))
    want_u8 = want_u8 or u8_only or out_u8 is not None
    if out is None and not u8_only:
        out = torch.empty((B, 3, H, W), device=points.device, dtype=torch.float32)
    u8 = None
    if want_u8:
        u8 = out_u8 if out_u8 is not None else torch.empty((B, H, W, 3), device=points.device, dtype=torch.uint8)
        assert u8.dtype == torch.uint8 and u8.is_contiguous() and tuple(u8.shape) == (B, H, W, 3)
    if inten_scale is None:
        check(lib().lm_bev_raster_batch(_stream(), _ptr(points) if points.numel() else None, offs, par, B, _ptr(ws), ws.numel(),
                                        None if u8_only else _ptr(out), _ptr(u8), H, W))
    else:
        if len(inten_scale) != B:
            raise ValueError(f'bev_raster_batch: {len(inten_scale)} inten_scale entries for {B} tiles')
        scale = (C.c_float * B)(*[0.0 if v is None else float(v) for v in inten_scale])
        check(lib().lm_bev_raster_batch_scaled(_stream(), _ptr(points) if points.numel() else None, offs, par, B, _ptr(ws), ws.numel(),
                                               None if u8_only else _ptr(out), _ptr(u8), H, W, scale))
    if u8_only:
        return u8
    return (out, u8) if want_u8 else out


def bev_raster(points, params, H=1152, W=1152, want_u8=False):
    r = bev_raster_batch(points, [0, points.shape[0]], [params], H, W, want_u8=want_u8)
    return (r[0][0], r[1][0]) if want_u8 else r[0]


def strip_grid(params, H=1152, W=1152, z_range=None):
    import numpy as np
    T = len(params)
    par = (LmRasterParams * T)(*params)
    z_lo, z_hi = (float(z_range[0]), float(z_range[1])) if z_range is not None else (-math.inf, math.inf)
    g = LmStripGrid()
    check(lib().lm_strip_build_grid(par, T, H, W, z_lo, z_hi, C.byref(g), None, 0))
    cells = np.empty((g.ny, g.nx, 8), dtype=np.uint16)
    check(lib().lm_strip_build_grid(par, T, H, W, z_lo, z_hi, C.byref(g), C.c_void_p(cells.ctypes.data), g.nx * g.ny))
    return {'x0': g.x0, 'y0': g.y0, 'cell': g.cell, 'nx': g.nx, 'ny': g.ny}, cells


def _tilted(p):
    return p.quat[1] != 0.0 or p.quat[2] != 0.0


def strip_bin_points(points, params, H=1152, W=1152, z_range=None, capacity=None):
    if not points.is_cuda:
        _ptr(points)
    assert points.dim() == 2 and points.shape[1] == 4 and points.is_contiguous() and points.dtype == torch.float32
    T, N = len(params), points.shape[0]
    par = (LmRasterParams * T)(*params)
    if z_range is None and N and any(_tilted(p) for p in params):
        z = points[:, 2]
        z = z[torch.isfinite(z)]
        z_range = (float(z.min()), float(z.max())) if z.numel() else (0.0, 0.0)
    z_lo, z_hi = (float(z_range[0]), float(z_range[1])) if z_range is not None else (-math.inf, math.inf)
    if not (math.isfinite(z_lo) and math.isfinite(z_hi)) and any(_tilted(p) for p in params):
        if N:
            raise ValueError('strip_bin_points: tilted tiles need a finite z_range (or None: it is then taken from the points)')
        z_lo, z_hi = 0.0, 0.0
    need = lib().lm_strip_bin_workspace_bytes(N, T)
    if need <= 0:
        raise LanemapHipError(f'strip_bin_points: {T} tiles / {N} points are not supported (1 to 4096 tiles)')
    ws = _workspace(points, need)
    meta = torch.empty(2 * T + 1, device=points.device, dtype=torch.int64)
    offs = (C.c_long * (T + 1))()
    cap = int(capacity) if capacity is not None else N + N // 4
    binned = None
    for attempt in range(2):
        del binned
        binned = torch.empty((cap, 4), device=points.device, dtype=torch.float32)
        rc = lib().lm_strip_bin_points(_stream(), _ptr(points) if N else None, N, par, T, H, W, z_lo, z_hi, _ptr(ws), ws.numel(),
                                       C.c_void_p(meta.data_ptr()), C.c_void_p(meta.data_ptr() + 8 * T), offs, _ptr(binned) if cap else None, cap)
        if rc == 4 and attempt == 0 and capacity is None:
            cap = int(offs[T])
            continue
        check(rc)
        break
    return binned[:offs[T]], [int(o) for o in offs]


def tile_ground(points, tile_offsets, params, H=1152, W=1152, cell_px=32, want_cell_min=False):
    B, offs, par = _tile_range_args('tile_ground', points, tile_offsets, params)
    H, W, cell_px = int(H), int(W), int(cell_px)
    need = lib().lm_tile_ground_workspace_bytes(B, H, W, cell_px)
    Gy, Gx = (-(-H // cell_px), -(-W // cell_px)) if cell_px > 0 else (0, 0)
    ws = _workspace(points, max(need, 16))
    ground = torch.empty((B, Gy, Gx), device=points.device, dtype=torch.float32)
    gmin = torch.empty((B,), device=points.device, dtype=torch.float32)
    cmin = torch.empty_like(ground) if want_cell_min else None
    check(lib().lm_tile_ground(_stream(), _ptr(points) if points.numel() else None, offs, par, B, H, W, cell_px, _ptr(ws), ws.numel() if need else 0,
                               _ptr(ground), _ptr(gmin), _ptr(cmin)))
    return (ground, gmin, cmin) if want_cell_min else (ground, gmin)


def ground_select(points, tile_offsets, params, ground, H=1152, W=1152, cell_px=32, h_range=(-math.inf, math.inf)):
    B, offs, par = _tile_range_args('ground_select', points, tile_offsets, params)
    H, W, cell_px = int(H), int(W), int(cell_px)
    Gy, Gx = (-(-H // cell_px), -(-W // cell_px)) if cell_px > 0 else (0, 0)
    if tuple(ground.shape) != (B, Gy, Gx) or ground.dtype != torch.float32 or not ground.is_contiguous() or ground.device != points.device:
        raise ValueError(f'ground_select: ground must be a contiguous [{B},{Gy},{Gx}] float32 tensor on {points.device} (tile_ground\'s output)')
    N = int(offs[B] - offs[0]) if B else 0
    need = lib().lm_ground_select_workspace_bytes(max(N, 0), B)
    ws = _workspace(points, max(need, 16))
    out = torch.empty((max(N, 0), 4), device=points.device, dtype=torch.float32)
    doffs = torch.empty((B + 1,), device=points.device, dtype=torch.int64)
    hoffs = (C.c_long * (B + 1))()
    check(lib().lm_ground_select(_stream(), _ptr(points) if points.numel() else None, offs, par, B, H, W, cell_px, _ptr(ground),
                                 float(h_range[0]), float(h_range[1]), _ptr(ws), ws.numel() if need else 0, _ptr(out) if N > 0 else None,
                                 C.c_void_p(doffs.data_ptr()), hoffs))
    return out[:hoffs[B]], [int(o) for o in hoffs]


def tile_intensity_window(points, tile_offsets, params, H=1152, W=1152, percentiles=(1.0, 99.9), group=None, want_hist=False):
    B, offs, par = _tile_range_args('tile_intensity_window', points, tile_offsets, params)
    H, W = int(H), int(W)
    if group is None:
        G, grp = B, None
    else:
        if len(group) != B:
            raise ValueError(f'tile_intensity_window: {len(group)} group entries for {B} tiles')
        ids = [int(g) for g in group]
        if any(not 0 <= g < B for g in ids):
            bad = next(b for b, g in enumerate(ids) if not 0 <= g < B)
            raise ValueError(f'tile_intensity_window: group[{bad}]={ids[bad]} is outside 0..B-1={B - 1} (G = max(group) + 1 <= B)')
        grp = (C.c_int * B)(*ids)
        G = max(ids + [0]) + 1
    q_lo, q_hi = (int(round(float(p) * 1e4)) for p in percentiles)
    need = lib().lm_tile_intensity_workspace_bytes(B, G)
    ws = _workspace(points, max(need, 16))
    window = torch.empty((max(G, 0), 2), device=points.device, dtype=torch.int32)
    count = torch.empty((max(G, 0),), device=points.device, dtype=torch.int64)
    hist = torch.empty((max(G, 0), 4096), device=points.device, dtype=torch.int32) if want_hist else None
    check(lib().lm_tile_intensity_window(_stream(), _ptr(points) if points.numel() else None, offs, par, B, H, W, grp, G, q_lo, q_hi,
                                         _ptr(ws), ws.numel() if need else 0, _ptr(window), _ptr(count), _ptr(hist)))
    return (window, count, hist) if want_hist else (window, count)


def drape_vertices(points, tile_offsets, params, vertices, vertex_offsets, H=1152, W=1152, radius_px=4, want_pixel_min=False):
    import numpy as np
    B, offs, par = _tile_range_args('drape_vertices', points, tile_offsets, params)
    H, W, R = int(H), int(W), int(radius_px)
    vert = np.ascontiguousarray(np.asarray(vertices, dtype=np.int32).reshape(-1, 2))
    if len(vertex_offsets) != B + 1:
        raise ValueError(f'drape_vertices: {len(vertex_offsets)} vertex_offsets for {B} tiles (B + 1 are needed)')
    voffs = (C.c_long * (B + 1))(*[int(o) for o in vertex_offsets])
    if voffs[B] != vert.shape[0]:
        raise ValueError(f'drape_vertices: vertex_offsets end at {voffs[B]}, vertices has {vert.shape[0]} rows')
    V, D = vert.shape[0], 2 * max(R, 0) + 1
    need = lib().lm_drape_workspace_bytes(V, B, R)
    ws = _workspace(points, max(need, 16))
    z = torch.empty((V,), device=points.device, dtype=torch.float32)
    npix = torch.empty((V,), device=points.device, dtype=torch.int32)
    pmin = torch.empty((V, D, D), device=points.device, dtype=torch.float32) if want_pixel_min else None
    check(lib().lm_drape_vertices(_stream(), _ptr(points) if points.numel() else None, offs, par, B, H, W, C.c_void_p(vert.ctypes.data), voffs, R,
                                  _ptr(ws), ws.numel() if need else 0, _ptr(z), _ptr(npix), _ptr(pmin)))
    return (z, npix, pmin) if want_pixel_min else (z, npix)


def _gap_args(who, u8):
    if not u8.is_cuda:
        _ptr(u8)
    if u8.dtype != torch.uint8 or u8.dim() != 4 or u8.shape[3] != 3 or not u8.is_contiguous():
        raise ValueError(f'{who}: tiles must be a contiguous uint8 tensor [B,H,W,3], not {u8.dtype} {tuple(u8.shape)}'
                         + ('' if u8.is_contiguous() else ' (not contiguous)'))
    return int(u8.shape[0]), int(u8.shape[1]), int(u8.shape[2])


def tile_gap_hist(u8, max_radius_px=4):
    B, H, W = _gap_args('tile_gap_hist', u8)
    R = int(max_radius_px)
    hist = torch.empty((B, max(R, 0) + 2), device=u8.device, dtype=torch.int32)
    check(lib().lm_tile_gap_hist(_stream(), _ptr(u8), B, H, W, R, _ptr(hist)))
    return hist


def tile_gap_fill(u8, radius_px):
    B, H, W = _gap_args('tile_gap_fill', u8)
    radii = [int(r) for r in radius_px] if hasattr(radius_px, '__len__') else [int(radius_px)] * B
    if len(radii) != B:
        raise ValueError(f'tile_gap_fill: {len(radii)} radius_px entries for {B} tiles')
    out = torch.empty_like(u8)
    check(lib().lm_tile_gap_fill(_stream(), _ptr(u8), B, H, W, (C.c_int * B)(*radii), _ptr(out)))
    return out


def tile_ingest(u8_hwc):
    x = u8_hwc.contiguous()
    B, H, W, C_ = x.shape
    out = torch.empty((B, 3, H, W), device=x.device, dtype=torch.float32)
    check(lib().lm_tile_ingest_u8(_stream(), _ptr(x), _ptr(out), B, H, W, C_))
    return out


_vox_ws = {}


def exclusive_scan_u32(x, out=None):
    x = x.contiguous()
    assert x.dim() == 1 and x.dtype in (torch.int32, torch.uint32)
    out = torch.empty_like(x) if out is None else out
    n = x.numel()
    ws = torch.empty((lib().lm_scan_workspace_bytes(n),), device=x.device, dtype=torch.uint8)
    check(lib().lm_exclusive_scan_u32(_stream(), _ptr(x), _ptr(out), n, _ptr(ws), ws.numel()))
    return out


def sort_pairs_u32_(keys, vals, end_bit=32):
    assert keys.dim() == 1 and keys.shape == vals.shape and keys.is_contiguous() and vals.is_contiguous()
    assert keys.dtype in (torch.int32, torch.uint32) and vals.dtype in (torch.int32, torch.uint32)
    n = keys.numel()
    ws = torch.empty((lib().lm_sort_pairs_workspace_bytes(n),), device=keys.device, dtype=torch.uint8)
    check(lib().lm_sort_pairs_u32(_stream(), _ptr(keys), _ptr(vals), n, int(end_bit), _ptr(ws), ws.numel()))
    return keys, vals


def voxelize_batch(points, range_lo, voxel_size, grid_xyz, max_points, max_voxels, ldf=16, raster_order=False):
    dev = points[0].device
    B = len(points)
    cells = int(grid_xyz[0]) * int(grid_xyz[1]) * int(grid_xyz[2])
    caps = [min(int(p.shape[0]), int(max_voxels), cells) for p in points]
    cap = max(1, sum(caps))
    feats = torch.empty((cap, ldf), device=dev, dtype=torch.float32)
    coords = torch.empty((cap, 4), device=dev, dtype=torch.int32)
    ends = torch.zeros((B,), device=dev, dtype=torch.int32)
    nmax = max(int(p.shape[0]) for p in points)
    need = lib().lm_voxelize_workspace_bytes(nmax)
    key = (dev.index, _stream().value)
    ws = _vox_ws.get(key)
    if ws is None or ws.numel() < need:
        ws = torch.empty((need,), device=dev, dtype=torch.uint8)
        _vox_ws[key] = ws
    lo = (C.c_float * 3)(*[float(v) for v in range_lo])
    vs = (C.c_float * 3)(*[float(v) for v in voxel_size])
    g = (C.c_int * 3)(*[int(v) for v in grid_xyz])
    for b, p in enumerate(points):
        if not p.is_cuda:
            raise LanemapHipError('voxelize_batch needs device tensors; no CPU fallback exists')
        p = p.contiguous().float()
        assert p.dim() == 2 and p.shape[1] == 4
        base = C.c_void_p(ends[b - 1:b].data_ptr()) if b > 0 else None
        check(lib().lm_voxelize_hard(_stream(), _ptr(p) if p.shape[0] else None, p.shape[0], lo, vs, g, int(max_points),
                                     int(max_voxels), b, base, cap, _ptr(feats), ldf, _ptr(coords),
                                     C.c_void_p(ends[b:b + 1].data_ptr()), int(raster_order), _ptr(ws), ws.numel()))
    row_ends = [int(v) for v in ends.cpu()]
    V = row_ends[-1]
    return feats[:V], coords[:V], row_ends


def _ksp(kernel, stride, padding):
    return (C.c_int * 9)(*[int(v) for v in (*kernel, *stride, *padding)])


def sparse_grid(coords, B, shape):
    D, H, W = shape
    grid = torch.empty((B, D, H, W), device=coords.device, dtype=torch.int32)
    check(lib().lm_sparse_grid_build(_stream(), _ptr(coords), coords.shape[0], _ptr(grid), B, D, H, W))
    return grid


# ... 83 lines not shown
```

lanemapping_amd/pcencoder.py:

```python
import os

import torch
import torch.nn as nn

from . import ops, trace
from .registry import PCENCODER
from .packing import PackedModule

_LAYERS = {'resnet18': [2, 2, 2, 2], 'resnet34': [3, 4, 6, 3]}
MERGE_BRANCH_CONVS = os.environ.get('LANEMAP_MERGE_BRANCH_CONVS', '1') != '0'
WINO_F44 = os.environ.get('LANEMAP_WINO_F44', '1') != '0'
WINO_F44_MIN_CIN = int(os.environ.get('LANEMAP_WINO_F44_MIN_CIN', '64'))
WINO_SPLIT = os.environ.get('LANEMAP_WINO_SPLIT', '0') != '0'


def _frag44(w):
    if WINO_SPLIT:
        return ops.pack_wino44_fragments_split(ops.pack_wino44(w))
    return ops.pack_wino44_fragments(ops.pack_wino44(w))


def _f44_ok(conv):
    return WINO_F44 and conv.kernel_size == (3, 3) and conv.stride == (1, 1) and conv.in_channels >= WINO_F44_MIN_CIN and conv.in_channels % 16 == 0


class _ResBlock(nn.Module):

    def __init__(self, cin, cout, stride, dilation, with_down):
        super().__init__()
        self.conv1 = nn.Conv2d(cin, cout, 3, stride, dilation, dilation, bias=False)
        self.bn1 = nn.BatchNorm2d(cout)
        self.conv2 = nn.Conv2d(cout, cout, 3, 1, dilation, dilation, bias=False)
        self.bn2 = nn.BatchNorm2d(cout)
        self.downsample = nn.Sequential(nn.Conv2d(cin, cout, 1, stride, bias=False), nn.BatchNorm2d(cout)) if with_down else None
        self.stride, self.dilation = stride, dilation


def _stage(state, planes, blocks, stride, dilate):
    prev_dil = state[1]
    if dilate:
        state[1] *= stride
        stride = 1
    layers = [_ResBlock(state[0], planes, stride, prev_dil, stride != 1 or state[0] != planes)]
    state[0] = planes
    for _ in range(1, blocks):
        layers.append(_ResBlock(planes, planes, 1, state[1], False))
    return nn.Sequential(*layers)


class _BottomUp(nn.Module):

    def __init__(self, layers, dil, in_channels):
        super().__init__()
        self.conv1 = nn.Conv2d(3, 64, 7, 2, 3, bias=False)
        self.bn1 = nn.BatchNorm2d(64)
        st = [64, 1]
        self.layer1 = _stage(st, in_channels[0], layers[0], 1, False)
        self.layer2 = _stage(st, in_channels[1], layers[1], 2, dil[0])
        if in_channels[2] > 0:
            self.layer3 = _stage(st, in_channels[2], layers[2], 2, dil[1])
        if in_channels[3] > 0:
            self.layer4 = _stage(st, in_channels[3], layers[3], 2, dil[2])


class FPNEncoder(PackedModule):
    def __init__(self, resnet='resnet34', pretrained=False, replace_stride_with_dilation=(False, True, False),
                 out_conv=True, in_channels=(64, 128, 256, -1), cfg=None):
        super().__init__()
        if resnet not in _LAYERS:
            raise NotImplementedError(f'{resnet}: only BasicBlock ResNets are on the hot path')
        if in_channels[2] <= 0 or in_channels[3] > 0:
            raise NotImplementedError('hot path covers in_channels=[c1,c2,c3,-1] (all BASELINE configs)')
        dil = list(replace_stride_with_dilation)
        if len(dil) != 3:
            raise ValueError(f'replace_stride_with_dilation should be None or a 3-element tuple, got {dil}')
        layers = _LAYERS[resnet]
        self.cfg = cfg
        self.in_channels = list(in_channels)
        self.model_buttomup = _BottomUp(layers, dil, in_channels)
        self.conv1 = nn.Conv2d(3, 64, 7, 2, 3, bias=False)
        self.bn1 = nn.BatchNorm2d(64)
        st = [64, 1]
        self.layer1 = _stage(st, in_channels[0], layers[0], 1, False)
        self.layer2 = _stage(st, in_channels[1], layers[1], 2, dil[0])
        self.layer3 = _stage(st, in_channels[2], layers[2], 2, dil[1])
        c = st[0]
        self.out = nn.Conv2d(c, cfg.featuremap_out_channel, 1, bias=False) if out_conv else None
        self.toplayer = nn.Conv2d(c, 256, 1)
        self.smooth1 = nn.Conv2d(c, c, 3, 1, 1)
        self.smooth2 = nn.Conv2d(c, c, 3, 1, 1)
        self.smooth3 = nn.Conv2d(c, c, 3, 1, 1)
        self.latlayer1 = nn.Conv2d(in_channels[1], c, 1)
        self.latlayer2 = nn.Conv2d(in_channels[0], c, 1)
        self.semantic_branch = nn.Conv2d(c, c // 2, 3, 1, 1)
        self.semantic_branch2 = nn.Conv2d(c, c // 2, 3, 1, 1)
        self.conv2 = nn.Conv2d(c, c, 3, 1, 1)
        self.conv3 = nn.Conv2d(c, c, 3, 1, 1)
        self.feature_layer = nn.Conv2d(c // 2, 8, 1)
        self.output_layer_binary_seg = nn.Conv2d(8, 3, 1)
        self.output_layer_endp = nn.Conv2d(c // 2, 1, 1)
        self.gn11 = nn.GroupNorm(c // 2, c // 2)
        self.gn12 = nn.GroupNorm(c, c)
        self.gn21 = nn.GroupNorm(c // 2, c // 2)
        self.gn22 = nn.GroupNorm(c, c)

    def _pack(self):
        P = {}
        P['stem_w'] = self.conv1.weight.permute(2, 3, 1, 0).contiguous().float()
        P['stem_s'], P['stem_b'] = ops.fold_bn(self.bn1)
        for lname in ('layer1', 'layer2', 'layer3'):
            for i, blk in enumerate(getattr(self, lname)):
                k = f'{lname}.{i}'
                P[k + '.w1'] = ops.pack_mfma(blk.conv1.weight)
                P[k + '.s1'], P[k + '.b1'] = ops.fold_bn(blk.bn1)
                P[k + '.w2'] = ops.pack_mfma(blk.conv2.weight)
                P[k + '.s2'], P[k + '.b2'] = ops.fold_bn(blk.bn2)
                for q, conv in (('.w1q', blk.conv1), ('.w2q', blk.conv2)):
                    if _f44_ok(conv):
                        P[k + q] = _frag44(conv.weight)
                if blk.downsample is not None:
                    P[k + '.wd'] = ops.pack_mfma(blk.downsample[0].weight)
                    P[k + '.sd'], P[k + '.bd'] = ops.fold_bn(blk.downsample[1])
        for name in ('toplayer', 'smooth1', 'smooth2', 'smooth3', 'latlayer1', 'latlayer2', 'semantic_branch',
                     'semantic_branch2', 'conv2', 'conv3'):
            m = getattr(self, name)
            P[name + '.w'] = ops.pack_mfma(m.weight)
            P[name + '.b'] = m.bias.float().contiguous()
            if _f44_ok(m):
                P[name + '.wq'] = _frag44(m.weight)
        a, b2 = self.semantic_branch, self.semantic_branch2
        if (MERGE_BRANCH_CONVS and 'semantic_branch.wq' in P and 'semantic_branch2.wq' in P and a.out_channels == b2.out_channels
                and self.gn11.eps == self.gn21.eps):
            P['semantic_branch_ab.wq'] = _frag44(torch.cat([a.weight, b2.weight], dim=0))
            P['semantic_branch_ab.b'] = torch.cat([a.bias, b2.bias]).float().contiguous()
            if ('conv2.wq' in P and 'conv3.wq' in P and self.conv2.out_channels == self.conv3.out_channels
                    and self.gn12.eps == self.gn22.eps):
                P['conv23.wq'] = _frag44(torch.cat([self.conv2.weight, self.conv3.weight], dim=0))
                P['conv23.b'] = torch.cat([self.conv2.bias, self.conv3.bias]).float().contiguous()
        if self.out is not None:
            P['out.w'] = ops.pack_mfma(self.out.weight)
        for name in ('feature_layer', 'output_layer_binary_seg', 'output_layer_endp'):
            m = getattr(self, name)
            P[name + '.w'] = ops.pack_small(m.weight)
            P[name + '.b'] = m.bias.float().contiguous()
        for name in ('gn11', 'gn12', 'gn21', 'gn22'):
            m = getattr(self, name)
            P[name + '.g'], P[name + '.b'] = m.weight.float().contiguous(), m.bias.float().contiguous()
        return P

    @staticmethod
    def _c3(x, P, wkey, cout, stride, dil, **epi):
        if (wkey + 'q') in P and stride == 1 and ops.wino44_supported(x.shape[2], x.shape[3], x.shape[1], dil):
            return ops.conv_wino44(x, P[wkey + 'q'], cout, dil, **epi)
        return ops.conv_mfma(x, P[wkey], cout, 3, 3, stride, dil, dil, **epi)

    def _block(self, x, P, key, blk):
        cout = blk.conv1.out_channels
        y = self._c3(x, P, key + '.w1', cout, blk.stride, blk.dilation, scale=P[key + '.s1'], shift=P[key + '.b1'], act=ops.ACT_RELU)
        if blk.downsample is not None:
            x = ops.conv_mfma(x, P[key + '.wd'], cout, 1, 1, blk.stride, 0, 1, scale=P[key + '.sd'], shift=P[key + '.bd'])
        return self._c3(y, P, key + '.w2', cout, 1, blk.dilation, scale=P[key + '.s2'], shift=P[key + '.b2'], res=x, act=ops.ACT_RELU)

    def _conv3(self, x, P, name, cout):
        return self._c3(x, P, name + '.w', cout, 1, 1, shift=P[name + '.b'])

    def _conv_stats(self, P, src, conv, cout, gn):
        eps = getattr(self, gn).eps
        if (conv + '.wq') in P and ops.wino44_supported(src.shape[2], src.shape[3], src.shape[1], 1):
            return ops.conv_wino44(src, P[conv + '.wq'], cout, 1, shift=P[conv + '.b'], gn_eps=eps)
        if (src.shape[2] * src.shape[3]) % 128 == 0:
            return ops.conv_mfma_gnstats(src, P[conv + '.w'], cout, 3, 3, 1, 1, 1, P[conv + '.b'], eps)
        t = self._conv3(src, P, conv, cout)
        return t, ops.gn_stats(t, eps)

    def _semantic(self, P, p2, p3, p4, conv_a, gn_a, conv_b, gn_b, proj, pre=None, pre_a4=None):
        h, w = p2.shape[2:]
        c_half = self.semantic_branch.out_channels
        t, st = pre_a4 if pre_a4 is not None else self._conv_stats(P, p4, conv_a, p4.shape[1], gn_a)
        s4 = ops.gn_relu_upsample_sum([(t, st)], P[gn_a + '.g'], P[gn_a + '.b'], (h, w))
        terms = [pre[0] if pre is not None and pre[0] is not None else self._conv_stats(P, p2, conv_b, c_half, gn_b),
                 pre[1] if pre is not None and pre[1] is not None else self._conv_stats(P, p3, conv_b, c_half, gn_b)]
        terms.append(self._conv_stats(P, s4, conv_b, c_half, gn_b))
        return ops.gn_relu_upsample_sum(terms, P[gn_b + '.g'], P[gn_b + '.b'], (h, w), proj=proj, keep_sum=False)

    def forward(self, x, fea_up_out=None):
        from . import torch_ops
        if self.out is None:
            return self._forward_impl(x, fea_up_out)
        if fea_up_out is None:
            B, H, W = (x.shape[0], x.shape[1], x.shape[2]) if x.dtype == torch.uint8 else (x.shape[0], x.shape[2], x.shape[3])
            fea_up_out = ops.new_act(B, 8, (H + 3) // 4, (W + 3) // 4, x.device)
        fea, bi_seg, endp = torch_ops.fpn_encoder(x, fea_up_out, torch_ops.stage_weights(self), torch_ops.stage_name(self))
        return fea, fea_up_out, bi_seg, endp

    def _forward_impl(self, x, fea_up_out=None):
        P = self.packed()
        if x.dtype == torch.uint8:
            B, H, W, _ = x.shape
        else:
            B, _, H, W = x.shape
        with trace.stage('fpn.stem'):
            c1 = ops.maxpool3x3s2(ops.stem(x, P['stem_w'], P['stem_s'], P['stem_b']))
        feats = []
        t = c1
        for lname in ('layer1', 'layer2', 'layer3'):
            with trace.stage('fpn.' + lname):
                for i, blk in enumerate(getattr(self, lname)):
                    t = self._block(t, P, f'{lname}.{i}', blk)
            feats.append(t)
        c2, c3, c4 = feats
        trace.push('fpn.topdown')
        fea = ops.conv_mfma(c4, P['out.w'], self.out.out_channels) if self.out is not None else None
        p4 = ops.conv_mfma(c4, P['toplayer.w'], 256, shift=P['toplayer.b'])
        def lateral(c, name, coarse):
            if tuple(coarse.shape[2:]) == tuple(c.shape[2:]):
                return ops.conv_mfma(c, P[name + '.w'], 256, shift=P[name + '.b'], res=coarse)
            return ops.conv_mfma(c, P[name + '.w'], 256, shift=P[name + '.b'], res_up=coarse)

        p3 = lateral(c3, 'latlayer1', p4)
        p2 = lateral(c2, 'latlayer2', p3)
        del c1, c2, c3, c4, feats, t
        p4 = self._conv3(p4, P, 'smooth1', 256)
        p3 = self._conv3(p3, P, 'smooth2', 256)
        p2 = self._conv3(p2, P, 'smooth3', 256)
        trace.pop()
        trace.push('fpn.semantic')
        pre_a, pre_b = [None, None], [None, None]
        if 'semantic_branch_ab.wq' in P:
            ch = self.semantic_branch.out_channels
            for i, src in enumerate((p2, p3)):
                if ops.wino44_supported(src.shape[2], src.shape[3], src.shape[1], 1):
                    t, st = ops.conv_wino44(src, P['semantic_branch_ab.wq'], 2 * ch, 1, shift=P['semantic_branch_ab.b'],
                                            gn_eps=self.gn11.eps, gn_split=2)
                    pre_a[i], pre_b[i] = (t[:, :ch], st[0]), (t[:, ch:], st[1])
        a4 = b4 = None
        if 'conv23.wq' in P and ops.wino44_supported(p4.shape[2], p4.shape[3], p4.shape[1], 1):
            c4o = self.conv2.out_channels
            t, st = ops.conv_wino44(p4, P['conv23.wq'], 2 * c4o, 1, shift=P['conv23.b'], gn_eps=self.gn12.eps, gn_split=2)
            a4, b4 = (t[:, :c4o], st[0]), (t[:, c4o:], st[1])
        fea_up = self._semantic(P, p2, p3, p4, 'conv2', 'gn12', 'semantic_branch', 'gn11',
                                (P['feature_layer.w'], P['feature_layer.b'], 8, fea_up_out), pre_a, a4)
        seg288 = ops.conv_small(fea_up, P['output_layer_binary_seg.w'], 3, shift=P['output_layer_binary_seg.b'], pre_relu=True)
        bi_seg = ops.upsample_to_chw(seg288, (H, W))
        endp288 = self._semantic(P, p2, p3, p4, 'conv3', 'gn22', 'semantic_branch2', 'gn21',
                                 (P['output_layer_endp.w'], P['output_layer_endp.b'], 1, None), pre_b, b4)
        endp = ops.upsample_to_chw(endp288, (H, W))
        trace.pop()
        return fea, fea_up, bi_seg, endp


@PCENCODER.register_module
class PostProjector2(nn.Module):
    def __init__(self, resnet='resnet50', pretrained=False, replace_stride_with_dilation=[False, True, False],
                 out_conv=True, in_channels=[64, 128, 256, -1], cfg=None):
        super().__init__()
        self.cfg = cfg
        self.fpn = FPNEncoder(resnet=resnet, pretrained=pretrained, replace_stride_with_dilation=replace_stride_with_dilation,
                              out_conv=out_conv, in_channels=in_channels, cfg=cfg)

    def forward(self, sample):
        return self.fpn(sample['proj'])

    def infer_validate(self, preds, seg_thre=None, endp_thre=None, display=None):
        from .decode import segmentor_decode
        return segmentor_decode(preds['seg'], preds['endp'], seg_thre)
```

lanemapping_amd/pipeline.py:

```python
import collections
import os
import threading
import time
from concurrent.futures import ThreadPoolExecutor

import numpy as np
import torch

from . import decode, hostpost, ops, torch_ops, trace
from ._lib import LanemapHipError


class TilePipeline:
    def __init__(self, net, host_threads=8, use_graph=None, with_decode_endp=False):
        self.with_decode_endp = bool(with_decode_endp)
        self.use_graph = (os.environ.get('LANEMAP_GRAPHS', '0') != '0') if use_graph is None else bool(use_graph)
        self._graphs = collections.OrderedDict()
        self.net = net
        self.cfg = net.cfg
        self.rowref = net.cfg.heads.type == 'RowSharNotReducRef'
        if net.cfg.heads.type not in ('ColumnProposal2', 'RowSharNotReducRef'):
            raise NotImplementedError(f'TilePipeline has no decode / polyline tail for heads.type={net.cfg.heads.type!r}')
        self.pool = ThreadPoolExecutor(max_workers=host_threads)
        self._pending = None
        self._slots, self._slot_next = [], 0
        self.host_seconds = 0.0
        self.host_tiles = 0
        self._stats_lock = threading.Lock()

    HOST_SLOTS = 3

    def _host_slot(self, nbytes):
        if not self._slots:
            self._slots = [{'block': None, 'futs': []} for _ in range(self.HOST_SLOTS)]
        slot = self._slots[self._slot_next]
        self._slot_next = (self._slot_next + 1) % self.HOST_SLOTS
        assert self._pending is None or self._pending[4] is not slot, 'pinned staging ring too short for the pipeline depth'
        if slot['futs']:
            from concurrent.futures import wait
            wait(slot['futs'])
        slot['futs'] = []
        if slot['block'] is None or slot['block'].numel() < nbytes:
            slot['block'] = torch.empty(max(nbytes, 1), dtype=torch.uint8, pin_memory=True)
        return slot

    def _gpu_stage(self, proj):
        if self.use_graph and torch.is_tensor(proj):
            (block, layout), keep, crop = self._replay(proj)
        else:
            (block, layout), keep, crop = self._device_part(proj)
        total = block.numel()
        slot = self._host_slot(total)
        hb = slot['block']
        hb[:total].copy_(block, non_blocking=True)
        host = {k: hb[o:o + nb].view(dt).view(shape) for k, o, nb, dt, shape in layout}
        ev = torch.cuda.Event()
        ev.record()
        return host, ev, (keep, block), crop, slot

    def _pack(self, dev):
        names = list(dev)
        if len(names) == 1 and dev[names[0]].is_contiguous():
            t = dev[names[0]]
            return t.view(-1).view(torch.uint8), [(names[0], 0, t.numel() * t.element_size(), t.dtype, tuple(t.shape))]
        ts = [dev[k].contiguous() for k in names]
        block, segs = ops.pack_readback(ts)
        end = max(o + nb for o, nb in segs)
        return block[:end], [(k, o, nb, t.dtype, tuple(t.shape)) for k, t, (o, nb) in zip(names, ts, segs)]

    MAX_GRAPHS = 4

    def _weights_key(self):
        from .packing import PackedModule
        mods = self.__dict__.get('_packed_mods')
        if mods is None:
            mods = self.__dict__['_packed_mods'] = [m for m in self.net.modules() if isinstance(m, PackedModule)]
        return tuple(m.param_key() for m in mods)

    def clear_graphs(self):
        self._graphs.clear()

    def _replay(self, proj):
        key = (tuple(proj.shape), proj.dtype, proj.device)
        wkey = self._weights_key()
        ent = self._graphs.get(key)
        if ent is not None and ent[3] != wkey:
            del self._graphs[key]
            ent = None
        if ent is None:
            static_in = torch.empty_like(proj)
            static_in.copy_(proj)
            self._device_part(static_in)
            torch.cuda.synchronize()
            graph = torch.cuda.CUDAGraph()
            with torch.cuda.graph(graph, stream=torch.cuda.Stream(device=proj.device)):
                out = self._device_part(static_in)
            ent = (graph, static_in, out, wkey)
            self._graphs[key] = ent
            while len(self._graphs) > self.MAX_GRAPHS:
                self._graphs.popitem(last=False)
        self._graphs.move_to_end(key)
        graph, static_in, out, _ = ent
        static_in.copy_(proj, non_blocking=True)
        graph.replay()
        return out

    def _device_part(self, proj):
        heads, cfg = self.net.heads, self.cfg
        batch = proj if isinstance(proj, dict) else ({'points': list(proj)} if isinstance(proj, (list, tuple)) else {'proj': proj})
        raw = self.net.forward_raw(batch)
        if self.rowref:
            dev = {'col': heads.decode_columns(raw)}
            keep = (raw, dev)
            crop = 0
        else:
            trace.push('decode')
            prop_conf, v_ext, cls_conf, cls_idx, cls_offset = torch_ops.decode_proposals(
                raw['proposal_conf'], raw['ext2'], raw['cls2'], raw['offset2'], float(cfg.exist_thre), heads.prop_width, heads.prop_half_buff)
            orient = torch_ops.decode_orient(raw['orient'])
            sem, biseg, rows = torch_ops.decode_semantic(raw['semantic_seg'], float(cfg.coor_thre))
            endp = heads.endp_logits(raw)
            idx, score, status = torch_ops.endp_topk(endp, decode.TOPK, decode.CLIP)
            trace.pop()
            dev = {'prop_conf': prop_conf, 'v_ext': v_ext, 'cls_offset': cls_offset, 'rows': rows, 'idx': idx, 'status': status}
            keep = (raw, sem, biseg, orient, cls_conf, cls_idx, dev)
            crop = endp.shape[-1]
        return self._pack(dev), keep, crop

    def _tile_task(self, host, b, crop_w):
        t0 = time.perf_counter()
        if self.rowref:
            heads = self.net.heads
            cols = heads.lines_from_columns(host['col'][b].numpy(), heads.row_size)
            lanes = np.full((72, 144, 2), -1.0)
            lanes[:, :, 1] = 0.0
            lanes[:cols.shape[0], :, 0] = cols
            lanes[:cols.shape[0], :, 1] = (cols > 0).astype(np.float64)
            kept = pts = np.zeros((0, 2), dtype=np.int32)
        else:
            pts, _ = hostpost.cluster_endpoints(host['idx'][b].numpy(), crop_w=crop_w, clip=decode.CLIP,
                                                k0=self.net.heads.num_cls * 2 * 10, k_max=500)
            lanes, kept = hostpost.assemble_polylines(host['prop_conf'][b].numpy(), host['v_ext'][b].numpy(),
                                                      host['cls_offset'][b].numpy(), host['rows'][b].numpy(), pts,
                                                      self.cfg.proposal_obj_thre)
            if lanes.shape[0] < 72:
                pad = np.full((72 - lanes.shape[0],) + lanes.shape[1:], -1.0)
                pad[:, :, 1] = 0.0
                lanes = np.concatenate([lanes, pad])
        dt = time.perf_counter() - t0
        with self._stats_lock:
            self.host_seconds += dt
            self.host_tiles += 1
        return (lanes, kept, pts) if self.with_decode_endp else (lanes, kept)

    def _finish(self, pending):
        host, ev, keep, W, slot = pending
        ev.synchronize()
        if not self.rowref and int(host['status'].max()) != 0:
            raise LanemapHipError('endpoint top-K candidate overflow')
        B = next(iter(host.values())).shape[0]
        futs = [self.pool.submit(self._tile_task, host, b, W - 2 * decode.CLIP) for b in range(B)]
        slot['futs'] = futs
        return futs

    def submit(self, proj):
        with torch.no_grad():
            new = self._gpu_stage(proj)
        futs = self._finish(self._pending) if self._pending is not None else []
        self._pending = new
        return futs

    def flush(self):
        futs = self._finish(self._pending) if self._pending is not None else []
        self._pending = None
        return futs

    def run_batch(self, proj):
        assert self._pending is None
        self.submit(proj)
        return [f.result() for f in self.flush()]
```

lanemapping_amd/torch_ops.py:

```python
import itertools
import weakref
from typing import List, Optional, Tuple

import numpy as np
import torch
from torch import Tensor

from . import ops as _ops

_STAGES = weakref.WeakValueDictionary()
_STAGE_COUNTER = itertools.count()


def stage_name(module):
    n = module.__dict__.get('_lanemap_stage_name')
    if n is None:
        n = module.__dict__['_lanemap_stage_name'] = f'{type(module).__name__}#{next(_STAGE_COUNTER)}'
    _STAGES[n] = module
    return n


def stage_weights(module):
    return [d[n] for d, n in module._slots() if d[n] is not None]


class _with_weights:

    def __init__(self, spec, weights):
        m = _STAGES.get(spec)
        if m is None:
            raise RuntimeError(f'lanemap_hip: no live stage module registered as {spec!r}')
        slots = [(d, n) for d, n in m._slots() if d[n] is not None]
        if len(slots) != len(weights):
            raise RuntimeError(f'lanemap_hip: stage {spec} has {len(slots)} weight tensors, the op was handed {len(weights)}')
        self.m, self.swap = m, [(d, n, d[n], w) for (d, n), w in zip(slots, weights) if d[n] is not w]
        for d, n, own, w in self.swap:
            if own.shape != w.shape or own.dtype != w.dtype:
                raise RuntimeError(f'lanemap_hip: stage {spec}: weight {n} is {tuple(w.shape)} {w.dtype}, expected {tuple(own.shape)} {own.dtype}')

    def __enter__(self):
        for d, n, own, w in self.swap:
            d[n] = w if not isinstance(own, torch.nn.Parameter) or isinstance(w, torch.nn.Parameter) else torch.nn.Parameter(w, requires_grad=False)
        return self.m

    def __exit__(self, *exc):
        for d, n, own, w in self.swap:
            d[n] = own
        return False


def _stage(spec):
    m = _STAGES.get(spec)
    if m is None:
        raise RuntimeError(f'lanemap_hip: no live stage module registered as {spec!r}')
    return m


def _fake_act(like, B, C, H, W, dtype=torch.float32):
    return like.new_empty((B, H, W, C), dtype=dtype).permute(0, 3, 1, 2)


def _out_hw(H, W, kh, kw, stride, pad, dil):
    return (H + 2 * pad - dil * (kh - 1) - 1) // stride + 1, (W + 2 * pad - dil * (kw - 1) - 1) // stride + 1


def _define(name, fn, fake, mutates=(), device='cuda'):
    op = torch.library.custom_op(f'lanemap_hip::{name}', fn, mutates_args=mutates, device_types=device)
    op.register_fake(fake)
    return op


def _conv2d_mfma(x: Tensor, w_packed: Tensor, cout: int, kh: int, kw: int, stride: int, pad: int, dil: int,
                 scale: Optional[Tensor], shift: Optional[Tensor], res: Optional[Tensor], act: int) -> Tensor:
    return _ops.conv_mfma(x, w_packed, cout, kh, kw, stride, pad, dil, scale=scale, shift=shift, res=res, act=act)


def _conv2d_mfma_fake(x, w_packed, cout, kh, kw, stride, pad, dil, scale, shift, res, act):
    Ho, Wo = _out_hw(x.shape[2], x.shape[3], kh, kw, stride, pad, dil)
    return _fake_act(x, x.shape[0], cout, Ho, Wo)


def _conv3x3_winograd44(x: Tensor, wu_frag: Tensor, cout: int, dil: int, scale: Optional[Tensor], shift: Optional[Tensor],
                        res: Optional[Tensor], act: int) -> Tensor:
    return _ops.conv_wino44(x, wu_frag, cout, dil, scale=scale, shift=shift, res=res, act=act)


def _conv3x3_fake(x, w, cout, dil, scale, shift, res, act):
    return _fake_act(x, x.shape[0], cout, x.shape[2], x.shape[3])


def _stem(x: Tensor, w_k64: Tensor, scale: Tensor, shift: Tensor) -> Tensor:
    return _ops.stem(x, w_k64, scale, shift)


def _stem_fake(x, w_k64, scale, shift):
    B, H, W = (x.shape[0], x.shape[1], x.shape[2]) if x.dtype == torch.uint8 else (x.shape[0], x.shape[2], x.shape[3])
    return _fake_act(x, B, 64, (H - 1) // 2 + 1, (W - 1) // 2 + 1)


def _maxpool(x: Tensor) -> Tensor:
    return _ops.maxpool3x3s2(x)


def _maxpool_fake(x):
    return _fake_act(x, x.shape[0], x.shape[1], (x.shape[2] - 1) // 2 + 1, (x.shape[3] - 1) // 2 + 1)


def _gn_stats(x: Tensor, eps: float) -> Tensor:
    return _ops.gn_stats(x, eps)


def _gn_stats_fake(x, eps):
    return x.new_empty((x.shape[0], x.shape[1], 2))


def _gn_relu_upsample(x: Tensor, stats: Tensor, gamma: Tensor, beta: Tensor, Ho: int, Wo: int) -> Tensor:
    return _ops.gn_relu_upsample(x, stats, gamma, beta, (Ho, Wo))


def _upsample_bilinear(x: Tensor, Ho: int, Wo: int) -> Tensor:
    y = _ops.upsample_nhwc(x, (Ho, Wo))
    return y.clone() if y.data_ptr() == x.data_ptr() else y


def _resize_fake(x, *a):
    return _fake_act(x, x.shape[0], x.shape[1], a[-2], a[-1])


def _layernorm_rows(x: Tensor, gamma: Tensor, beta: Tensor, eps: float) -> Tensor:
    return _ops.layernorm(x, gamma, beta, eps)


def _attention(qkv: Tensor, B: int, N: int, heads: int, dim_head: int, scale: float) -> Tensor:
    return _ops.attention(qkv, B, N, heads, dim_head, scale)


def _linear_mfma(x: Tensor, w_packed: Tensor, n_out: int, scale: Optional[Tensor], shift: Optional[Tensor], res: Optional[Tensor],
                 res_rows: int, act: int) -> Tensor:
    return _ops.linear_mfma(x, w_packed, n_out, scale=scale, shift=shift, res=res, res_rows=res_rows, act=act)


def _token_mix(x: Tensor, wt: Tensor, M: int, bias: Tensor, B: int, res: Optional[Tensor], act: int) -> Tensor:
    return _ops.token_mix(x, wt, M, bias, B, res=res, act=act)


def _tile_ingest(u8_hwc: Tensor) -> Tensor:
    return _ops.tile_ingest(u8_hwc)


def _decode_proposals(pconf: Tensor, ext2: Tensor, cls2: Tensor, off2: Tensor, exist_thre: float, prop_width: int,
                      half_buff: int) -> Tuple[Tensor, Tensor, Tensor, Tensor, Tensor]:
    return _ops.decode_proposals(pconf, ext2, cls2, off2, exist_thre, prop_width, half_buff)


def _decode_proposals_fake(pconf, ext2, cls2, off2, exist_thre, prop_width, half_buff):
    B, P, R, FW = cls2.shape
    return (cls2.new_empty((B, P, 2)), cls2.new_empty((B, P, R)), cls2.new_empty((B, P, R, FW)),
            cls2.new_empty((B, P, R), dtype=torch.int32), cls2.new_empty((B, P, R), dtype=torch.float64))


def _decode_semantic(logits: Tensor, thre: float) -> Tuple[Tensor, Tensor, Tensor]:
    return _ops.decode_semantic(logits, thre)


def _decode_semantic_fake(logits, thre):
    B, _, H, W = logits.shape
    return logits.new_empty((B, H, W), dtype=torch.uint8), logits.new_empty((B, H, W)), logits.new_empty((B, H // 8, W))


def _decode_orient(orient_logits: Tensor) -> Tensor:
    return _ops.decode_orient(orient_logits)


def _endp_topk(endp_logits: Tensor, K: int, clip: int) -> Tuple[Tensor, Tensor, Tensor]:
    return _ops.endp_topk(endp_logits, K=K, clip=clip)


def _endp_topk_fake(endp_logits, K, clip):
    B = endp_logits.shape[0]
    return (endp_logits.new_empty((B, K), dtype=torch.int32), endp_logits.new_empty((B, K)), endp_logits.new_empty((B,), dtype=torch.int32))


conv2d_mfma = _define('conv2d_mfma', _conv2d_mfma, _conv2d_mfma_fake)
conv3x3_winograd44 = _define('conv3x3_winograd44', _conv3x3_winograd44, _conv3x3_fake)
stem_conv7x7 = _define('stem_conv7x7', _stem, _stem_fake)
maxpool3x3s2 = _define('maxpool3x3s2', _maxpool, _maxpool_fake)
gn_stats = _define('gn_stats', _gn_stats, _gn_stats_fake)
gn_relu_upsample = _define('gn_relu_upsample', _gn_relu_upsample, lambda x, stats, gamma, beta, Ho, Wo: _resize_fake(x, Ho, Wo))
upsample_bilinear = _define('upsample_bilinear', _upsample_bilinear, lambda x, Ho, Wo: _resize_fake(x, Ho, Wo))
layernorm_rows = _define('layernorm_rows', _layernorm_rows, lambda x, gamma, beta, eps: torch.empty_like(x))
attention = _define('attention', _attention, lambda qkv, B, N, heads, dim_head, scale: qkv.new_empty((B * N, heads * dim_head)))
linear_mfma = _define('linear_mfma', _linear_mfma,
                      lambda x, w_packed, n_out, scale, shift, res, res_rows, act: x.new_empty((x.shape[0], n_out)))
token_mix = _define('token_mix', _token_mix, lambda x, wt, M, bias, B, res, act: x.new_empty((B * M, x.shape[1])))
tile_ingest = _define('tile_ingest', _tile_ingest,
                      lambda u8: u8.new_empty((u8.shape[0], 3, u8.shape[1], u8.shape[2]), dtype=torch.float32))
decode_proposals = _define('decode_proposals', _decode_proposals, _decode_proposals_fake)
decode_semantic = _define('decode_semantic', _decode_semantic, _decode_semantic_fake)
decode_orient = _define('decode_orient', _decode_orient,
                        lambda o: o.new_empty((o.shape[0], o.shape[2], o.shape[3]), dtype=torch.uint8))
endp_topk = _define('endp_topk', _endp_topk, _endp_topk_fake)


def _bev_raster(points: Tensor, tile_offsets: List[int], params: Tensor, H: int, W: int) -> Tensor:
    p = params.detach().cpu().float().numpy()
    pars = [_ops.make_raster_params(quat=r[0:4], trans=r[4:7], bev_img_offset=r[7:9], img_reso=r[9:11], local_min_ele=r[11],
                                    ele_reso=r[12], inten_lo=r[13], inten_hi=r[14]) for r in p]
    return _ops.bev_raster_batch(points, tile_offsets, pars, H, W, u8_only=True)


bev_raster = _define('bev_raster', _bev_raster,
                     lambda points, tile_offsets, params, H, W: points.new_empty((len(tile_offsets) - 1, H, W, 3), dtype=torch.uint8))


def _params_list(params):
    p = params.detach().cpu().float().numpy()
    return [_ops.make_raster_params(quat=r[0:4], trans=r[4:7], bev_img_offset=r[7:9], img_reso=r[9:11], local_min_ele=r[11],
                                    ele_reso=r[12], inten_lo=r[13], inten_hi=r[14]) for r in p]


def _tile_ground(points: Tensor, tile_offsets: List[int], params: Tensor, H: int, W: int, cell_px: int) -> Tuple[Tensor, Tensor]:
    return _ops.tile_ground(points, tile_offsets, _params_list(params), H, W, cell_px)


def _tile_ground_fake(points, tile_offsets, params, H, W, cell_px):
    B = len(tile_offsets) - 1
    return points.new_empty((B, -(-H // cell_px), -(-W // cell_px))), points.new_empty((B,))


tile_ground = _define('tile_ground', _tile_ground, _tile_ground_fake)


def _ground_select(points: Tensor, tile_offsets: List[int], params: Tensor, ground: Tensor, H: int, W: int, cell_px: int, h_lo: float,
                   h_hi: float) -> Tuple[Tensor, Tensor]:
    out, offs = _ops.ground_select(points, tile_offsets, _params_list(params), ground, H, W, cell_px, (h_lo, h_hi))
    return out, torch.tensor(offs, dtype=torch.int64, device=points.device)


def _ground_select_fake(points, tile_offsets, params, ground, H, W, cell_px, h_lo, h_hi):
    n = torch.library.get_ctx().new_dynamic_size()
    return points.new_empty((n, 4)), points.new_empty((len(tile_offsets),), dtype=torch.int64)


ground_select = _define('ground_select', _ground_select, _ground_select_fake)


def _tile_intensity_window(points: Tensor, tile_offsets: List[int], params: Tensor, H: int, W: int, p_lo: float, p_hi: float,
                           group: Optional[List[int]]) -> Tuple[Tensor, Tensor]:
    return _ops.tile_intensity_window(points, tile_offsets, _params_list(params), H, W, (p_lo, p_hi), group)


def _tile_intensity_window_fake(points, tile_offsets, params, H, W, p_lo, p_hi, group):
    G = len(tile_offsets) - 1 if group is None else max(list(group) + [0]) + 1
    return points.new_empty((G, 2), dtype=torch.int32), points.new_empty((G,), dtype=torch.int64)


tile_intensity_window = _define('tile_intensity_window', _tile_intensity_window, _tile_intensity_window_fake)


def _bev_raster_scaled(points: Tensor, tile_offsets: List[int], params: Tensor, H: int, W: int) -> Tensor:
    scale = [float(v) for v in params.detach().cpu().float()[:, 15]]
    return _ops.bev_raster_batch(points, tile_offsets, _params_list(params), H, W, u8_only=True, inten_scale=scale)


bev_raster_scaled = _define('bev_raster_scaled', _bev_raster_scaled,
                            lambda points, tile_offsets, params, H, W: points.new_empty((len(tile_offsets) - 1, H, W, 3), dtype=torch.uint8))


def raster_params_tensor(params):
    rows = [[*p.quat, *p.trans, *p.bev_img_offset, *p.img_reso, p.local_min_ele, p.ele_reso, p.inten_lo, p.inten_hi] for p in params]
    return torch.tensor(rows, dtype=torch.float32)


def _fpn_encoder(proj: Tensor, fea_up_out: Tensor, weights: List[Tensor], stage: str) -> Tuple[Tensor, Tensor, Tensor]:
    with _with_weights(stage, weights) as m:
        fea, _, bi_seg, endp = m._forward_impl(proj, fea_up_out)
    return fea, bi_seg, endp


def _fpn_encoder_fake(proj, fea_up_out, weights, stage):
    B, H, W = (proj.shape[0], proj.shape[1], proj.shape[2]) if proj.dtype == torch.uint8 else (proj.shape[0], proj.shape[2], proj.shape[3])
    m = _stage(stage)
    cf = m.out.out_channels if m.out is not None else 256
    return (_fake_act(proj, B, cf, H // 8, W // 8), proj.new_empty((B, 3, H, W), dtype=torch.float32),
            proj.new_empty((B, 1, H, W), dtype=torch.float32))


fpn_encoder = _define('fpn_encoder', _fpn_encoder, _fpn_encoder_fake, mutates=('fea_up_out',))


def _vit_backbone(fea: Tensor, weights: List[Tensor], stage: str) -> Tensor:
    with _with_weights(stage, weights) as m:
        return m._forward_impl(fea)


def _vit_backbone_fake(fea, weights, stage):
    m = _stage(stage)
    c = m.shared_mlp.out_channels if m.is_with_shared_mlp else m.out_c
    return _fake_act(fea, fea.shape[0], c, m.grid * m.patch, m.grid * m.patch)


vit_backbone = _define('vit_backbone', _vit_backbone, _vit_backbone_fake)


def _mixer_backbone(fea: Tensor, weights: List[Tensor], stage: str) -> Tensor:
    with _with_weights(stage, weights) as m:
        return m._forward_impl(fea)


def _mixer_backbone_fake(fea, weights, stage):
    m = _stage(stage)
    return _fake_act(fea, fea.shape[0], m.output_channels, m.grid * m.patch, m.grid * m.patch)


mixer_backbone = _define('mixer_backbone', _mixer_backbone, _mixer_backbone_fake)


def _colprop_head(x: Tensor, col: Tensor, weights: List[Tensor], stage: str) -> Tuple[Tensor, Tensor, Tensor, Tensor, Tensor]:
    with _with_weights(stage, weights) as m:
        o = m._forward_impl(x, None, None, col=col)
    return o['proposal_conf'], o['ext2'], o['cls2'], o['offset2'], o['orient']


def _colprop_head_fake(x, col, weights, stage):
    m = _stage(stage)
    B, R, P, FW = x.shape[0], x.shape[2], m.num_prop, m.prop_fea_width
    return (x.new_empty((B, P, 2)), x.new_empty((B, P, R, 3)), x.new_empty((B, P, R, FW)), x.new_empty((B, P, R, FW)),
            _fake_act(x, B, m.num_orients, x.shape[2], x.shape[3]))


colprop_head = _define('colprop_head', _colprop_head, _colprop_head_fake, mutates=('col',))


def _colprop_endpoint(col: Tensor, x_endp: Tensor, weights: List[Tensor], stage: str) -> Tensor:
    with _with_weights(stage, weights) as m:
        return m._endpoint_impl(col, x_endp)


def _colprop_endpoint_fake(col, x_endp, weights, stage):
    return x_endp.new_empty((x_endp.shape[0], 1, x_endp.shape[2], x_endp.shape[3]), dtype=torch.float32)


colprop_endpoint = _define('colprop_endpoint', _colprop_endpoint, _colprop_endpoint_fake)


def _endp_cluster(topk_idx: Tensor, crop_w: int, clip: int, k0: int, k_max: int) -> Tensor:
    from . import hostpost
    pts, _ = hostpost.cluster_endpoints(topk_idx.numpy(), crop_w=crop_w, clip=clip, k0=k0, k_max=k_max)
    return torch.from_numpy(pts.astype(np.int32).reshape(-1, 2))


def _endp_cluster_fake(topk_idx, crop_w, clip, k0, k_max):
    n = torch.library.get_ctx().new_dynamic_size()
    return topk_idx.new_empty((n, 2), dtype=torch.int32)


endp_cluster = _define('endp_cluster', _endp_cluster, _endp_cluster_fake, device='cpu')


def _polyline_assemble(prop_conf: Tensor, prop_v_ext: Tensor, cls_offset: Tensor, bi_seg_rows: Tensor, endp_hw: Tensor,
                       obj_thre: float) -> Tuple[Tensor, Tensor]:
    from . import hostpost
    lanes, kept = hostpost.assemble_polylines(prop_conf.numpy(), prop_v_ext.numpy(), cls_offset.numpy(), bi_seg_rows.numpy(),
                                              endp_hw.numpy(), obj_thre)
    return torch.from_numpy(lanes), torch.from_numpy(np.ascontiguousarray(kept, dtype=np.int32).reshape(-1, 2))


def _polyline_assemble_fake(prop_conf, prop_v_ext, cls_offset, bi_seg_rows, endp_hw, obj_thre):
    n = torch.library.get_ctx().new_dynamic_size()
    P, R = prop_v_ext.shape
    return prop_conf.new_empty((P, R, 2), dtype=torch.float64), endp_hw.new_empty((n, 2), dtype=torch.int32)


polyline_assemble = _define('polyline_assemble', _polyline_assemble, _polyline_assemble_fake, device='cpu')

OP_NAMES = ['conv2d_mfma', 'conv3x3_winograd44', 'stem_conv7x7', 'maxpool3x3s2', 'gn_stats', 'gn_relu_upsample',
            'upsample_bilinear', 'layernorm_rows', 'attention', 'linear_mfma', 'token_mix', 'tile_ingest', 'decode_proposals', 'decode_semantic',
            'decode_orient', 'endp_topk', 'bev_raster', 'bev_raster_scaled', 'tile_ground', 'ground_select', 'tile_intensity_window', 'fpn_encoder', 'vit_backbone', 'mixer_backbone', 'colprop_head', 'colprop_endpoint', 'endp_cluster', 'polyline_assemble']
```

Before: 397.1 tiles/s.

## Decode semantic rows and endpoint top-k directly from low-res logits

```diff
diff --git a/include/lanemap_hip.h b/include/lanemap_hip.h
--- a/include/lanemap_hip.h
+++ b/include/lanemap_hip.h
@@ -99,6 +99,10 @@
 long lm_endp_topk_workspace_bytes(int B);
 int lm_endp_topk(void* stream, const float* endp_logit, void* workspace, int* out_idx, float* out_score,
                  int* out_status, int B, int H, int W, int clip, int K);
+int lm_decode_rows_lowres(void* hip_stream, const float* logit_lo, int ldx, float* rows, int B, int Hi, int Wi, int Ho, int Wo,
+                          int raw_mode);
+int lm_endp_topk_lowres(void* hip_stream, const float* endp_lo, int ldx, void* workspace, int* out_idx, float* out_score,
+                        int* out_status, int B, int Hi, int Wi, int H, int W, int clip, int K);
 
 int lm_pack_segments(void* stream, int n, const void* const* src, const long* bytes, const long* dst_offsets, void* dst);
 
diff --git a/lanemapping_amd/_lib.py b/lanemapping_amd/_lib.py
--- a/lanemapping_amd/_lib.py
+++ b/lanemapping_amd/_lib.py
@@ -75,6 +75,8 @@
     'lm_decode_semantic': (i32, [vp, vp, vp, vp, vp, i32, i32, i32, f32, i32]),
     'lm_endp_topk_workspace_bytes': (i64, [i32]),
     'lm_endp_topk': (i32, [vp, vp, vp, vp, vp, vp, i32, i32, i32, i32, i32]),
+    'lm_decode_rows_lowres': (i32, [vp, vp, i32, vp, i32, i32, i32, i32, i32, i32]),
+    'lm_endp_topk_lowres': (i32, [vp, vp, i32, vp, vp, vp, vp, i32, i32, i32, i32, i32, i32, i32]),
     'lm_pack_segments': (i32, [vp, i32, vp, vp, vp, vp]),
     'lm_bev_raster_workspace_bytes': (i64, [i32, i64, i32, i32]),
     'lm_bev_raster_batch': (i32, [vp, vp, C.POINTER(i64), C.POINTER(LmRasterParams), i32, vp, i64, vp, vp, i32, i32]),
diff --git a/lanemapping_amd/csrc/common.h b/lanemapping_amd/csrc/common.h
--- a/lanemapping_amd/csrc/common.h
+++ b/lanemapping_amd/csrc/common.h
@@ -83,4 +83,18 @@
     const float bot = wx0 * v10 + wx1 * v11;
     return wy0 * top + wy1 * bot;
 }
+__device__ __forceinline__ float lm_upsample_px(const float* __restrict__ r0, const float* __restrict__ r1, int ldx, int ox, int Wi, int Wo,
+                                                float wy0, float wy1) {
+    int x0, x1;
+    float wx0, wx1;
+    lm_bilin_axis(ox, Wi, Wo, x0, x1, wx0, wx1);
+    const float v00 = r0[(long)x0 * ldx], v01 = r0[(long)x1 * ldx], v10 = r1[(long)x0 * ldx], v11 = r1[(long)x1 * ldx];
+    return lm_bilerp(v00, v01, v10, v11, wy0, wy1, wx0, wx1);
+}
+__device__ __forceinline__ float lm_upsample_at(const float* __restrict__ xb, int ldx, int Hi, int Wi, int Ho, int Wo, int oy, int ox) {
+    int y0, y1;
+    float wy0, wy1;
+    lm_bilin_axis(oy, Hi, Ho, y0, y1, wy0, wy1);
+    return lm_upsample_px(xb + (long)y0 * Wi * ldx, xb + (long)y1 * Wi * ldx, ldx, ox, Wi, Wo, wy0, wy1);
+}
 #endif
diff --git a/lanemapping_amd/csrc/decode.hip b/lanemapping_amd/csrc/decode.hip
--- a/lanemapping_amd/csrc/decode.hip
+++ b/lanemapping_amd/csrc/decode.hip
@@ -77,6 +77,19 @@
     y[i] = (unsigned char)best;
 }
 
+__device__ __forceinline__ void semantic_scores(float l0, float l1, float l2, int raw_mode, float& s1, float& s2) {
+    if (raw_mode) {
+        s1 = l1;
+        s2 = l2;
+    } else {
+        const float m = fmaxf(l0, fmaxf(l1, l2));
+        const float e0 = expf(l0 - m), e1 = expf(l1 - m), e2 = expf(l2 - m);
+        const float s = (e0 + e1) + e2;
+        s1 = e1 / s;
+        s2 = e2 / s;
+    }
+}
+
 __global__ __launch_bounds__(256) void decode_semantic_kernel(const float* __restrict__ logit, unsigned char* __restrict__ sem,
                                                               float* __restrict__ biseg, float* __restrict__ rows, int H, int W,
                                                               float thre, int raw_mode, long total) {
@@ -87,16 +100,7 @@
     const float* lp = logit + b * 3 * HW + r;
     const float l0 = lp[0], l1 = lp[HW], l2 = lp[2 * HW];
     float s1, s2;
-    if (raw_mode) {
-        s1 = l1;
-        s2 = l2;
-    } else {
-        const float m = fmaxf(l0, fmaxf(l1, l2));
-        const float e0 = expf(l0 - m), e1 = expf(l1 - m), e2 = expf(l2 - m);
-        const float s = (e0 + e1) + e2;
-        s1 = e1 / s;
-        s2 = e2 / s;
-    }
+    semantic_scores(l0, l1, l2, raw_mode, s1, s2);
     unsigned char c = 0;
     if (s1 > s2 && s1 > thre) c = 1;
     if (s2 > s1 && s2 > thre) c = 2;
@@ -109,10 +113,29 @@
     }
 }
 
+__global__ __launch_bounds__(256) void decode_rows_lowres_kernel(const float* __restrict__ x, int ldx, float* __restrict__ rows, int Hi, int Wi,
+                                                                 int Ho, int Wo, int raw_mode, unsigned total) {
+    const unsigned i = blockIdx.x * 256u + threadIdx.x;
+    if (i >= total) return;
+    const unsigned Hr = (unsigned)Ho / 8;
+    const int ox = (int)(i % (unsigned)Wo);
+    const unsigned t = i / (unsigned)Wo;
+    const int oy = (int)(t % Hr) * 8 + 3;
+    const int b = (int)(t / Hr);
+    const float* xb = x + (long)b * Hi * Wi * ldx;
+    const float l0 = lm_upsample_at(xb, ldx, Hi, Wi, Ho, Wo, oy, ox);
+    const float l1 = lm_upsample_at(xb + 1, ldx, Hi, Wi, Ho, Wo, oy, ox);
+    const float l2 = lm_upsample_at(xb + 2, ldx, Hi, Wi, Ho, Wo, oy, ox);
+    float s1, s2;
+    semantic_scores(l0, l1, l2, raw_mode, s1, s2);
+    rows[i] = s1 + s2;
+}
+
 constexpr int NB = 1024;
 constexpr int CAP = 4096;
 struct TopkParams {
     const float* logit;
+    int ldx, Hi, Wi;
     unsigned* hist;
     unsigned* cand_cnt;
     unsigned long long* cand;
@@ -123,6 +146,16 @@
 __device__ __forceinline__ unsigned score_key(float logit) {
     const float s = 1.0f / (1.0f + expf(-logit));
     return __float_as_uint(s);
+}
+
+template <bool LOWRES>
+__device__ __forceinline__ const float* topk_tile(const TopkParams& p, int b) {
+    return LOWRES ? p.logit + (long)b * p.Hi * p.Wi * p.ldx : p.logit + (long)b * p.H * p.W;
+}
+template <bool LOWRES>
+__device__ __forceinline__ float topk_logit(const TopkParams& p, const float* __restrict__ lp, int y, int x) {
+    if constexpr (LOWRES) return lm_upsample_at(lp, p.ldx, p.Hi, p.Wi, p.H, p.W, y + p.clip, x + p.clip);
+    else return lp[(long)(y + p.clip) * p.W + x + p.clip];
 }
 
 __device__ __forceinline__ unsigned level_bin(unsigned key, int level) {
@@ -176,7 +209,7 @@
     if (i < n) p[i] = 0u;
 }
 
-template <int LEVEL>
+template <int LEVEL, bool LOWRES>
 __global__ __launch_bounds__(256) void topk_pass_kernel(TopkParams p) {
     __shared__ unsigned lh[NB];
     __shared__ unsigned pb_tmp[258];
@@ -198,10 +231,10 @@
         if (LEVEL == 3) take_ties = hist[2 * NB + bin] == need;
     }
     __syncthreads();
-    const float* lp = p.logit + (long)b * p.H * p.W;
+    const float* lp = topk_tile<LOWRES>(p, b);
     for (long i = (long)blockIdx.x * 256 + threadIdx.x; i < n; i += (long)gridDim.x * 256) {
         const int y = (int)lm_fastdiv((unsigned)i, p.div_wc), x = (int)((unsigned)i - (unsigned)y * (unsigned)Wc);
-        const unsigned key = score_key(lp[(long)(y + p.clip) * p.W + x + p.clip]);
+        const unsigned key = score_key(topk_logit<LOWRES>(p, lp, y, x));
         if (LEVEL == 0) {
             atomicAdd(&lh[key >> 20], 1u);
         } else if (LEVEL == 1) {
@@ -222,6 +255,7 @@
     }
 }
 
+template <bool LOWRES>
 __global__ __launch_bounds__(1024) void topk_ties_kernel(TopkParams p) {
     __shared__ unsigned sh[4];
     __shared__ unsigned wave_tot[16];
@@ -240,7 +274,7 @@
     if (hist[2 * NB + bin] == need || need == 0) return;
     const int Wc = p.W - 2 * p.clip;
     const long n = (long)(p.H - 2 * p.clip) * Wc;
-    const float* lp = p.logit + (long)b * p.H * p.W;
+    const float* lp = topk_tile<LOWRES>(p, b);
     const int lane = threadIdx.x & 63, wave = threadIdx.x >> 6;
     unsigned taken = 0;
     for (long i0 = 0; i0 < n && taken < need; i0 += 1024) {
@@ -248,7 +282,7 @@
         bool tie = false;
         if (i < n) {
             const int y = (int)lm_fastdiv((unsigned)i, p.div_wc), x = (int)((unsigned)i - (unsigned)y * (unsigned)Wc);
-            tie = score_key(lp[(long)(y + p.clip) * p.W + x + p.clip]) == T;
+            tie = score_key(topk_logit<LOWRES>(p, lp, y, x)) == T;
         }
         const unsigned long long m = __ballot(tie);
         const unsigned before = (unsigned)__popcll(m & ((1ull << lane) - 1ull));
@@ -359,17 +393,26 @@
     return LM_OK;
 }
 
+LM_API int lm_decode_rows_lowres(void* hip_stream, const float* logit_lo, int ldx, float* rows, int B, int Hi, int Wi, int Ho, int Wo,
+                                 int raw_mode) {
+    LM_REQUIRE(logit_lo && rows, "decode_rows_lowres: null pointer");
+    LM_REQUIRE(B >= 1 && Hi >= 1 && Wi >= 1 && ldx >= 3 && Ho >= 8 && Wo >= 1 && Ho % 8 == 0, "decode_rows_lowres: bad shape (Hi=%d Wi=%d ldx=%d Ho=%d Wo=%d; Ho a multiple of 8, ldx >= 3)", Hi, Wi, ldx, Ho, Wo);
+    const long total = (long)B * (Ho / 8) * Wo;
+    LM_REQUIRE(total < (1L << 31) && (long)B * Hi * Wi * ldx < (1L << 40), "decode_rows_lowres: too large");
+    hipLaunchKernelGGL(decode_rows_lowres_kernel, dim3(lm_cdiv(total, 256)), dim3(256), 0, (hipStream_t)hip_stream, logit_lo, ldx, rows,
+                       Hi, Wi, Ho, Wo, raw_mode, (unsigned)total);
+    LM_LAUNCH_CHECK();
+    return LM_OK;
+}
+
 LM_API long lm_endp_topk_workspace_bytes(int B) {
     return (long)B * (3 * NB * sizeof(unsigned) + sizeof(unsigned) * 4 + (long)CAP * sizeof(unsigned long long));
 }
 
-LM_API int lm_endp_topk(void* stream, const float* endp_logit, void* workspace, int* out_idx, float* out_score,
-                        int* out_status, int B, int H, int W, int clip, int K) {
-    LM_REQUIRE(endp_logit && workspace && out_idx && out_score && out_status, "endp_topk: null pointer");
+template <bool LOWRES>
+static int topk_launch(hipStream_t s, TopkParams p, void* workspace, int* out_idx, float* out_score, int* out_status, int B, int H, int W,
+                       int clip, int K) {
     LM_REQUIRE(K >= 1 && K <= CAP / 2 && H > 2 * clip && W > 2 * clip, "endp_topk: bad K=%d or crop", K);
-    hipStream_t s = (hipStream_t)stream;
-    TopkParams p;
-    p.logit = endp_logit;
     char* ws = (char*)workspace;
     p.hist = (unsigned*)ws;
     p.cand_cnt = (unsigned*)(ws + (size_t)B * 3 * NB * sizeof(unsigned));
@@ -381,19 +424,38 @@
     hipLaunchKernelGGL(zero_u32_kernel, dim3(lm_cdiv(zero_words, 256)), dim3(256), 0, s, (unsigned*)workspace, zero_words);
     LM_LAUNCH_CHECK();
     dim3 grid(256, B);
-    hipLaunchKernelGGL(topk_pass_kernel<0>, grid, dim3(256), 0, s, p);
-    LM_LAUNCH_CHECK();
-    hipLaunchKernelGGL(topk_pass_kernel<1>, grid, dim3(256), 0, s, p);
-    LM_LAUNCH_CHECK();
-    hipLaunchKernelGGL(topk_pass_kernel<2>, grid, dim3(256), 0, s, p);
-    LM_LAUNCH_CHECK();
-    hipLaunchKernelGGL(topk_pass_kernel<3>, grid, dim3(256), 0, s, p);
-    LM_LAUNCH_CHECK();
-    hipLaunchKernelGGL(topk_ties_kernel, dim3(B), dim3(1024), 0, s, p);
+    hipLaunchKernelGGL((topk_pass_kernel<0, LOWRES>), grid, dim3(256), 0, s, p);
+    LM_LAUNCH_CHECK();
+    hipLaunchKernelGGL((topk_pass_kernel<1, LOWRES>), grid, dim3(256), 0, s, p);
+    LM_LAUNCH_CHECK();
+    hipLaunchKernelGGL((topk_pass_kernel<2, LOWRES>), grid, dim3(256), 0, s, p);
+    LM_LAUNCH_CHECK();
+    hipLaunchKernelGGL((topk_pass_kernel<3, LOWRES>), grid, dim3(256), 0, s, p);
+    LM_LAUNCH_CHECK();
+    hipLaunchKernelGGL(topk_ties_kernel<LOWRES>, dim3(B), dim3(1024), 0, s, p);
     LM_LAUNCH_CHECK();
     hipLaunchKernelGGL(topk_sort_kernel, dim3(B), dim3(1024), 0, s, p, out_idx, out_score, out_status);
     LM_LAUNCH_CHECK();
     return LM_OK;
+}
+
+LM_API int lm_endp_topk(void* stream, const float* endp_logit, void* workspace, int* out_idx, float* out_score,
+                        int* out_status, int B, int H, int W, int clip, int K) {
+    LM_REQUIRE(endp_logit && workspace && out_idx && out_score && out_status, "endp_topk: null pointer");
+    TopkParams p;
+    p.logit = endp_logit;
+    p.ldx = 1; p.Hi = H; p.Wi = W;
+    return topk_launch<false>((hipStream_t)stream, p, workspace, out_idx, out_score, out_status, B, H, W, clip, K);
+}
+
+LM_API int lm_endp_topk_lowres(void* hip_stream, const float* endp_lo, int ldx, void* workspace, int* out_idx, float* out_score,
+                               int* out_status, int B, int Hi, int Wi, int H, int W, int clip, int K) {
+    LM_REQUIRE(endp_lo && workspace && out_idx && out_score && out_status, "endp_topk_lowres: null pointer");
+    LM_REQUIRE(B >= 1 && Hi >= 1 && Wi >= 1 && ldx >= 1 && (long)B * Hi * Wi * ldx < (1L << 40), "endp_topk_lowres: bad source (B=%d Hi=%d Wi=%d ldx=%d)", B, Hi, Wi, ldx);
+    TopkParams p;
+    p.logit = endp_lo;
+    p.ldx = ldx; p.Hi = Hi; p.Wi = Wi;
+    return topk_launch<true>((hipStream_t)hip_stream, p, workspace, out_idx, out_score, out_status, B, H, W, clip, K);
 }
 
 LM_API int lm_pack_segments(void* stream, int n, const void* const* src, const long* bytes, const long* dst_offsets, void* dst) {
diff --git a/lanemapping_amd/csrc/norm_resize.hip b/lanemapping_amd/csrc/norm_resize.hip
--- a/lanemapping_amd/csrc/norm_resize.hip
+++ b/lanemapping_amd/csrc/norm_resize.hip
@@ -497,9 +497,6 @@
     *reinterpret_cast<f32x4*>(y + opix * ldy + c) = o;
 }
 
-__device__ __forceinline__ float upsample_blend(float v00, float v01, float v10, float v11, float wy0, float wy1, float wx0, float wx1) {
-    return lm_bilerp(v00, v01, v10, v11, wy0, wy1, wx0, wx1);
-}
 
 __global__ __launch_bounds__(256) void upsample_to_chw_kernel(const float* __restrict__ x, int ldx, float* __restrict__ y,
                                                               int Hi, int Wi, int Ho, int Wo, int C, long total) {
@@ -511,14 +508,7 @@
     t /= Ho;
     const int c = (int)(t % C);
     const int b = (int)(t / C);
-    int y0, y1, x0, x1;
-    float wy0, wy1, wx0, wx1;
-    bilin_axis(oy, Hi, Ho, y0, y1, wy0, wy1);
-    bilin_axis(ox, Wi, Wo, x0, x1, wx0, wx1);
-    const float* xb = x + (long)b * Hi * Wi * ldx + c;
-    const float v00 = xb[((long)y0 * Wi + x0) * ldx], v01 = xb[((long)y0 * Wi + x1) * ldx];
-    const float v10 = xb[((long)y1 * Wi + x0) * ldx], v11 = xb[((long)y1 * Wi + x1) * ldx];
-    y[i] = upsample_blend(v00, v01, v10, v11, wy0, wy1, wx0, wx1);
+    y[i] = lm_upsample_at(x + (long)b * Hi * Wi * ldx + c, ldx, Hi, Wi, Ho, Wo, oy, ox);
 }
 
 __global__ __launch_bounds__(256) void upsample_to_chw4_kernel(const float* __restrict__ x, int ldx, float* __restrict__ y,
@@ -540,13 +530,7 @@
     const float* r1 = xb + (long)y1 * Wi * ldx;
     f32x4 o;
 #pragma unroll
-    for (int k = 0; k < 4; ++k) {
-        int x0, x1;
-        float wx0, wx1;
-        bilin_axis(ox0 + k, Wi, Wo, x0, x1, wx0, wx1);
-        const float v00 = r0[(long)x0 * ldx], v01 = r0[(long)x1 * ldx], v10 = r1[(long)x0 * ldx], v11 = r1[(long)x1 * ldx];
-        o[k] = upsample_blend(v00, v01, v10, v11, wy0, wy1, wx0, wx1);
-    }
+    for (int k = 0; k < 4; ++k) o[k] = lm_upsample_px(r0, r1, ldx, ox0 + k, Wi, Wo, wy0, wy1);
     *reinterpret_cast<f32x4*>(y + (long)i * 4) = o;
 }
 
diff --git a/lanemapping_amd/net.py b/lanemapping_amd/net.py
--- a/lanemapping_amd/net.py
+++ b/lanemapping_amd/net.py
@@ -16,15 +16,16 @@
         self.heads = build_heads(cfg)
         self.head_type, self.loss_type = head_type, loss_type
 
-    def forward_raw(self, batch):
+    def forward_raw(self, batch, decode_lowres=False):
         fused = hasattr(self.pcencoder, 'fpn') and self.cfg.heads.type == 'ColumnProposal2'
+        lowres = bool(decode_lowres) and fused and not self.heads.endpoint_mode()
         col = None
         if fused:
             proj = batch['proj']
             B, H, W = (proj.shape[0], proj.shape[1], proj.shape[2]) if proj.dtype == torch.uint8 else (proj.shape[0], proj.shape[2], proj.shape[3])
             col = ops.new_act(B, 16, H // 4, W // 4, proj.device)
             with trace.stage('pcencoder'):
-                fea, fea_up, bi_seg, endp_est = self.pcencoder.fpn(proj, fea_up_out=col[:, 8:16])
+                fea, fea_up, bi_seg, endp_est = self.pcencoder.fpn(proj, fea_up_out=col[:, 8:16], lowres=lowres)
         else:
             with trace.stage('pcencoder'):
                 fea, fea_up, bi_seg, endp_est = self.pcencoder(batch)
@@ -36,6 +37,9 @@
                 out = self.heads(fea)
             else:
                 out = self.heads(fea, fea_up, endp_est, col=col) if fused else self.heads(fea, fea_up, endp_est)
+        if lowres:
+            out['semantic_seg_lowres'], out['endp_est_lowres'], out['decode_size'] = bi_seg, endp_est, (H, W)
+            return out
         out['semantic_seg'] = bi_seg
         out['endp_est'] = endp_est
         return out
diff --git a/lanemapping_amd/ops.py b/lanemapping_amd/ops.py
--- a/lanemapping_amd/ops.py
+++ b/lanemapping_amd/ops.py
@@ -550,15 +550,42 @@
     return sem, biseg, rows
 
 
+def endp_topk_workspace(B, device):
+    return torch.empty(lib().lm_endp_topk_workspace_bytes(B), device=device, dtype=torch.uint8)
+
+
 def endp_topk(endp_logits, K=512, clip=20):
     x = endp_logits.contiguous()
     B, C_, H, W = x.shape
     assert C_ == 1
-    ws = torch.empty(lib().lm_endp_topk_workspace_bytes(B), device=x.device, dtype=torch.uint8)
+    ws = endp_topk_workspace(B, x.device)
     idx = torch.empty((B, K), device=x.device, dtype=torch.int32)
     score = torch.empty((B, K), device=x.device, dtype=torch.float32)
     status = torch.empty((B,), device=x.device, dtype=torch.int32)
     check(lib().lm_endp_topk(_stream(), _ptr(x), _ptr(ws), _ptr(idx), _ptr(score), _ptr(status), B, H, W, clip, K))
+    return idx, score, status
+
+
+def decode_rows_lowres(logits_lo, size, raw_mode=False):
+    x, ldx = as_nhwc(logits_lo)
+    B, C_, h, w = x.shape
+    H, W = size
+    assert C_ == 3 and ldx >= 3
+    rows = torch.empty((B, H // 8, W), device=x.device, dtype=torch.float32)
+    check(lib().lm_decode_rows_lowres(_stream(), _ptr(x), ldx, _ptr(rows), B, h, w, H, W, int(raw_mode)))
+    return rows
+
+
+def endp_topk_lowres(endp_lo, size, K=512, clip=20):
+    x, ldx = as_nhwc(endp_lo)
+    B, C_, h, w = x.shape
+    H, W = size
+    assert C_ == 1
+    ws = endp_topk_workspace(B, x.device)
+    idx = torch.empty((B, K), device=x.device, dtype=torch.int32)
+    score = torch.empty((B, K), device=x.device, dtype=torch.float32)
+    status = torch.empty((B,), device=x.device, dtype=torch.int32)
+    check(lib().lm_endp_topk_lowres(_stream(), _ptr(x), ldx, _ptr(ws), _ptr(idx), _ptr(score), _ptr(status), B, h, w, H, W, clip, K))
     return idx, score, status
 
 
diff --git a/lanemapping_amd/pcencoder.py b/lanemapping_amd/pcencoder.py
--- a/lanemapping_amd/pcencoder.py
+++ b/lanemapping_amd/pcencoder.py
@@ -183,17 +183,17 @@
         terms.append(self._conv_stats(P, s4, conv_b, c_half, gn_b))
         return ops.gn_relu_upsample_sum(terms, P[gn_b + '.g'], P[gn_b + '.b'], (h, w), proj=proj, keep_sum=False)
 
-    def forward(self, x, fea_up_out=None):
+    def forward(self, x, fea_up_out=None, lowres=False):
         from . import torch_ops
         if self.out is None:
-            return self._forward_impl(x, fea_up_out)
+            return self._forward_impl(x, fea_up_out, lowres)
         if fea_up_out is None:
             B, H, W = (x.shape[0], x.shape[1], x.shape[2]) if x.dtype == torch.uint8 else (x.shape[0], x.shape[2], x.shape[3])
             fea_up_out = ops.new_act(B, 8, (H + 3) // 4, (W + 3) // 4, x.device)
-        fea, bi_seg, endp = torch_ops.fpn_encoder(x, fea_up_out, torch_ops.stage_weights(self), torch_ops.stage_name(self))
+        fea, bi_seg, endp = torch_ops.fpn_encoder(x, fea_up_out, torch_ops.stage_weights(self), torch_ops.stage_name(self), bool(lowres))
         return fea, fea_up_out, bi_seg, endp
 
-    def _forward_impl(self, x, fea_up_out=None):
+    def _forward_impl(self, x, fea_up_out=None, lowres=False):
         P = self.packed()
         if x.dtype == torch.uint8:
             B, H, W, _ = x.shape
@@ -241,10 +241,10 @@
         fea_up = self._semantic(P, p2, p3, p4, 'conv2', 'gn12', 'semantic_branch', 'gn11',
                                 (P['feature_layer.w'], P['feature_layer.b'], 8, fea_up_out), pre_a, a4)
         seg288 = ops.conv_small(fea_up, P['output_layer_binary_seg.w'], 3, shift=P['output_layer_binary_seg.b'], pre_relu=True)
-        bi_seg = ops.upsample_to_chw(seg288, (H, W))
+        bi_seg = seg288 if lowres else ops.upsample_to_chw(seg288, (H, W))
         endp288 = self._semantic(P, p2, p3, p4, 'conv3', 'gn22', 'semantic_branch2', 'gn21',
                                  (P['output_layer_endp.w'], P['output_layer_endp.b'], 1, None), pre_b, b4)
-        endp = ops.upsample_to_chw(endp288, (H, W))
+        endp = endp288 if lowres else ops.upsample_to_chw(endp288, (H, W))
         trace.pop()
         return fea, fea_up, bi_seg, endp
 
diff --git a/lanemapping_amd/pipeline.py b/lanemapping_amd/pipeline.py
--- a/lanemapping_amd/pipeline.py
+++ b/lanemapping_amd/pipeline.py
@@ -15,6 +15,7 @@
     def __init__(self, net, host_threads=8, use_graph=None, with_decode_endp=False):
         self.with_decode_endp = bool(with_decode_endp)
         self.use_graph = (os.environ.get('LANEMAP_GRAPHS', '0') != '0') if use_graph is None else bool(use_graph)
+        self.decode_lowres = os.environ.get('LANEMAP_DECODE_LOWRES', '1') != '0'
         self._graphs = collections.OrderedDict()
         self.net = net
         self.cfg = net.cfg
@@ -108,7 +109,7 @@
     def _device_part(self, proj):
         heads, cfg = self.net.heads, self.cfg
         batch = proj if isinstance(proj, dict) else ({'points': list(proj)} if isinstance(proj, (list, tuple)) else {'proj': proj})
-        raw = self.net.forward_raw(batch)
+        raw = self.net.forward_raw(batch, decode_lowres=True) if self.decode_lowres and not self.rowref else self.net.forward_raw(batch)
         if self.rowref:
             dev = {'col': heads.decode_columns(raw)}
             keep = (raw, dev)
@@ -117,14 +118,22 @@
             trace.push('decode')
             prop_conf, v_ext, cls_conf, cls_idx, cls_offset = torch_ops.decode_proposals(
                 raw['proposal_conf'], raw['ext2'], raw['cls2'], raw['offset2'], float(cfg.exist_thre), heads.prop_width, heads.prop_half_buff)
-            orient = torch_ops.decode_orient(raw['orient'])
-            sem, biseg, rows = torch_ops.decode_semantic(raw['semantic_seg'], float(cfg.coor_thre))
-            endp = heads.endp_logits(raw)
-            idx, score, status = torch_ops.endp_topk(endp, decode.TOPK, decode.CLIP)
+            if 'semantic_seg_lowres' in raw:
+                H, W = raw['decode_size']
+                rows = torch_ops.decode_rows_lowres(raw['semantic_seg_lowres'], H, W)
+                idx, score, status = torch_ops.endp_topk_lowres(raw['endp_est_lowres'], H, W, decode.TOPK, decode.CLIP)
+                keep = (raw, score, cls_conf, cls_idx)
+                crop = W
+            else:
+                orient = torch_ops.decode_orient(raw['orient'])
+                sem, biseg, rows = torch_ops.decode_semantic(raw['semantic_seg'], float(cfg.coor_thre))
+                endp = heads.endp_logits(raw)
+                idx, score, status = torch_ops.endp_topk(endp, decode.TOPK, decode.CLIP)
+                keep = (raw, sem, biseg, orient, score, cls_conf, cls_idx)
+                crop = endp.shape[-1]
             trace.pop()
             dev = {'prop_conf': prop_conf, 'v_ext': v_ext, 'cls_offset': cls_offset, 'rows': rows, 'idx': idx, 'status': status}
-            keep = (raw, sem, biseg, orient, cls_conf, cls_idx, dev)
-            crop = endp.shape[-1]
+            keep = keep + (dev,)
         return self._pack(dev), keep, crop
 
     def _tile_task(self, host, b, crop_w):
diff --git a/lanemapping_amd/torch_ops.py b/lanemapping_amd/torch_ops.py
--- a/lanemapping_amd/torch_ops.py
+++ b/lanemapping_amd/torch_ops.py
@@ -179,6 +179,14 @@
 def _endp_topk_fake(endp_logits, K, clip):
     B = endp_logits.shape[0]
     return (endp_logits.new_empty((B, K), dtype=torch.int32), endp_logits.new_empty((B, K)), endp_logits.new_empty((B,), dtype=torch.int32))
+
+
+def _decode_rows_lowres(logits_lo: Tensor, H: int, W: int) -> Tensor:
+    return _ops.decode_rows_lowres(logits_lo, (H, W))
+
+
+def _endp_topk_lowres(endp_lo: Tensor, H: int, W: int, K: int, clip: int) -> Tuple[Tensor, Tensor, Tensor]:
+    return _ops.endp_topk_lowres(endp_lo, (H, W), K=K, clip=clip)
 
 
 conv2d_mfma = _define('conv2d_mfma', _conv2d_mfma, _conv2d_mfma_fake)
@@ -200,6 +208,9 @@
 decode_orient = _define('decode_orient', _decode_orient,
                         lambda o: o.new_empty((o.shape[0], o.shape[2], o.shape[3]), dtype=torch.uint8))
 endp_topk = _define('endp_topk', _endp_topk, _endp_topk_fake)
+decode_rows_lowres = _define('decode_rows_lowres', _decode_rows_lowres,
+                             lambda logits_lo, H, W: logits_lo.new_empty((logits_lo.shape[0], H // 8, W), dtype=torch.float32))
+endp_topk_lowres = _define('endp_topk_lowres', _endp_topk_lowres, lambda endp_lo, H, W, K, clip: _endp_topk_fake(endp_lo, K, clip))
 
 
 def _bev_raster(points: Tensor, tile_offsets: List[int], params: Tensor, H: int, W: int) -> Tensor:
@@ -272,16 +283,19 @@
     return torch.tensor(rows, dtype=torch.float32)
 
 
-def _fpn_encoder(proj: Tensor, fea_up_out: Tensor, weights: List[Tensor], stage: str) -> Tuple[Tensor, Tensor, Tensor]:
-    with _with_weights(stage, weights) as m:
-        fea, _, bi_seg, endp = m._forward_impl(proj, fea_up_out)
+def _fpn_encoder(proj: Tensor, fea_up_out: Tensor, weights: List[Tensor], stage: str, lowres: bool = False) -> Tuple[Tensor, Tensor, Tensor]:
+    with _with_weights(stage, weights) as m:
+        fea, _, bi_seg, endp = m._forward_impl(proj, fea_up_out, lowres)
     return fea, bi_seg, endp
 
 
-def _fpn_encoder_fake(proj, fea_up_out, weights, stage):
+def _fpn_encoder_fake(proj, fea_up_out, weights, stage, lowres=False):
     B, H, W = (proj.shape[0], proj.shape[1], proj.shape[2]) if proj.dtype == torch.uint8 else (proj.shape[0], proj.shape[2], proj.shape[3])
     m = _stage(stage)
     cf = m.out.out_channels if m.out is not None else 256
+    if lowres:
+        h, w = (H + 3) // 4, (W + 3) // 4
+        return _fake_act(proj, B, cf, H // 8, W // 8), _fake_act(proj, B, 3, h, w), _fake_act(proj, B, 1, h, w)
     return (_fake_act(proj, B, cf, H // 8, W // 8), proj.new_empty((B, 3, H, W), dtype=torch.float32),
             proj.new_empty((B, 1, H, W), dtype=torch.float32))
 
@@ -376,4 +390,4 @@
 
 OP_NAMES = ['conv2d_mfma', 'conv3x3_winograd44', 'stem_conv7x7', 'maxpool3x3s2', 'gn_stats', 'gn_relu_upsample',
             'upsample_bilinear', 'layernorm_rows', 'attention', 'linear_mfma', 'token_mix', 'tile_ingest', 'decode_proposals', 'decode_semantic',
-            'decode_orient', 'endp_topk', 'bev_raster', 'bev_raster_scaled', 'tile_ground', 'ground_select', 'tile_intensity_window', 'fpn_encoder', 'vit_backbone', 'mixer_backbone', 'colprop_head', 'colprop_endpoint', 'endp_cluster', 'polyline_assemble']
+            'decode_orient', 'endp_topk', 'decode_rows_lowres', 'endp_topk_lowres', 'bev_raster', 'bev_raster_scaled', 'tile_ground', 'ground_select', 'tile_intensity_window', 'fpn_encoder', 'vit_backbone', 'mixer_backbone', 'colprop_head', 'colprop_endpoint', 'endp_cluster', 'polyline_assemble']
```

After: 399.5 tiles/s, median of 2. No clear change (+0.6%).
